# trungnt13/odin-ai

Measured on AMD Instinct MI355X. Metric: VAE train images/sec, higher is better.
Workload: dtype f32; 1 GPU; dsprites_betavae_b256; global_batch=256, per_gpu_batch=256, parallelism=dp1, graph=True

## Files before the change

### include/odin_hip.h

```cpp
#ifndef ODIN_HIP_H
#define ODIN_HIP_H

#include <stddef.h>
#include <stdint.h>

#ifdef __cplusplus
extern "C" {
#endif

enum { ODIN_LINEAR = 0, ODIN_ELU = 1, ODIN_RELU = 2 };

typedef struct odin_conv_desc {
  int B, H, W, Cin;
  int OH, OW, Cout;
  int KH, KW, stride;
  int pad_t, pad_l;
  int act;
  int center;
  uint32_t* dy_amax;
  uint32_t* dx_amax;
  const uint32_t* x_amax;
  uint32_t* y_amax;
} odin_conv_desc;

int odin_version(void);
const char* odin_debug_last_path(void);
uint32_t odin_crc32c(uint32_t crc, const void* data, size_t n);
const char* odin_last_error(void);
int odin_max_slab_rows(void);
int odin_conv2d_dgrad_keeps_range(const odin_conv_desc* d, int aux_act);
int odin_deconv2d_dgrad_keeps_range(const odin_conv_desc* d, int aux_act);
int odin_bernoulli_tail_keeps_range(int is_deconv, const odin_conv_desc* d, int C1);
#define ODIN_RANGE_WORDS 2048
int odin_range_reset(uint32_t* words, int n, void* stream);
int odin_absmax(const float* t, size_t n, uint32_t* word, void* stream);
int odin_debug_stream_probe(const float* a, const float* b, float* out, size_t n, int variant, int blocks,
                            void* stream);
int odin_debug_absmax_fallbacks(void);

int odin_conv2d_fwd(const float* x, const float* w, const float* bias, float* y,
                    const odin_conv_desc* d, void* stream);
int odin_conv2d_dgrad(const float* dy, const float* w, const float* aux, int aux_act, float* dx,
                      float* colsum_slab, int* slab_rows_out, const odin_conv_desc* d,
                      void* stream);
int odin_conv2d_wgrad(const float* x, const float* dy, float* slab, int* slab_rows_out,
                      const odin_conv_desc* d, void* stream);

int odin_deconv2d_fwd(const float* x, const float* w, const float* bias, float* y,
                      const odin_conv_desc* d, void* stream);
int odin_deconv2d_dgrad(const float* dy, const float* w, const float* aux, int aux_act,
                        float* dx, float* colsum_slab, int* slab_rows_out,
                        const odin_conv_desc* d, void* stream);
int odin_deconv2d_wgrad(const float* x, const float* dy, float* slab, int* slab_rows_out,
                        const odin_conv_desc* d, void* stream);

int odin_conv2d_bwd(const float* x, const float* dy, const float* w, const float* aux, int aux_act, float* dx,
                    float* colsum_slab, int* colsum_rows_out, float* wslab, int* wslab_rows_out,
                    const odin_conv_desc* d, void* stream);
int odin_deconv2d_bwd(const float* x, const float* dy, const float* w, const float* aux, int aux_act, float* dx,
                      float* colsum_slab, int* colsum_rows_out, float* wslab, int* wslab_rows_out,
                      const odin_conv_desc* d, void* stream);
int odin_conv2d_dgrad_first(const float* dy, const float* w, const float* aux, int aux_act, float* dx,
                            float* colsum_slab, int* colsum_rows_out, const odin_conv_desc* d, const float* x0,
                            float* wslab0, int* wslab0_rows_out, const odin_conv_desc* d0, void* stream);
int odin_dense_bwd(const float* x, const float* dy, const float* w, const float* aux, int aux_act, float* dx,
                   float* colsum_slab, int* colsum_rows_out, float* wslab, int* wslab_rows_out, int B, int K,
                   int N, int want_wgrad, int want_dgrad, const uint32_t* dy_amax, uint32_t* dx_amax, void* stream);
int odin_conv2d_reads_x_range(const odin_conv_desc* d);
int odin_deconv2d_reads_x_range(const odin_conv_desc* d);
int odin_dense_reads_x_range(int B, int K, int N);
int odin_dense_fwd_ranged(const float* x, const float* w, const float* bias, float* y, int B, int K, int N, int act,
                          const uint32_t* x_amax, uint32_t* y_amax, void* stream);
int odin_dense_bwd_ranged(const float* x, const float* dy, const float* w, const float* aux, int aux_act, float* dx,
                          float* colsum_slab, int* colsum_rows_out, float* wslab, int* wslab_rows_out, int B, int K,
                          int N, int want_wgrad, int want_dgrad, const uint32_t* dy_amax, uint32_t* dx_amax,
                          const uint32_t* x_amax, void* stream);
int odin_dense_dgrad_keeps_range(int B, int K, int N);

int odin_bernoulli_tail_fwd_bwd(int is_deconv, const float* x, const float* w, const float* bias,
                                const float* w1, const float* b1, const float* target,
                                float* logits, float* g_out, float* llk_part, int* n_part_out,
                                float* tail_slab, int* slab_rows_out, const float* scale,
                                const odin_conv_desc* d, int C1, void* stream);

int odin_dense_fwd(const float* x, const float* w, const float* bias, float* y, int B, int K,
                   int N, int act, void* stream);
int odin_dense_dgrad(const float* dy, const float* w, const float* aux, int aux_act, float* dx,
                     float* colsum_slab, int* slab_rows_out, int B, int K, int N, void* stream);
int odin_dense_wgrad(const float* x, const float* dy, float* slab, int* slab_rows_out, int B,
                     int K, int N, void* stream);

typedef struct odin_reduce_job {
  const float* src;
  float* dst;
  int n;
  int rows;
  int stride;
  int pad_;
} odin_reduce_job;
int odin_slab_reduce(const odin_reduce_job* jobs, int n_jobs, void* stream);

int odin_latent_fwd(const float* p, const float* eps, float* z, float* kl, float* fbmask, int B,
                    int D, int analytic, float free_bits, const float* capacity, void* stream);
int odin_latent_bwd(const float* p, const float* eps, const float* z, const float* dz,
                    const float* dz_extra, const float* fbmask, const float* klw,
                    const float* dloc_x, const float* dscale_x, float* dp, int B, int D,
                    int analytic, void* stream);

int odin_latent_block_rows(int B, int P, int D, int N0);
int odin_latent_block_fwd(const float* h, const float* wl, const float* bl, const float* eps_in,
                          float* eps_out, uint64_t seed, const int32_t* step_dev, float* p, float* z,
                          float* kl, float* fbmask, const float* w0, const float* b0, float* y0, int B,
                          int P, int D, int N0, int act0, int analytic, float free_bits,
                          const float* capacity, void* stream);
int odin_latent_block_bwd(const float* g0, const float* w0, const float* z, const float* p,
                          const float* eps, const float* fbmask, const float* klw, const float* dz_extra,
                          const float* dloc_x, const float* dscale_x, const float* wl, const float* h,
                          int h_act, float* dz, float* dp, float* dh, float* slab0, float* slabl, int B,
                          int P, int D, int N0, int analytic, uint32_t* dh_amax, void* stream);

typedef struct odin_neck_args {
  int B, P, D, C0;
  int act2, act3, act4, act0, act1;
  int analytic;
  float free_bits;
  uint64_t seed;
  const int32_t* step_dev;
  const float* x;
  const uint32_t* x_amax;
  const float *w3, *b3;
  float* y3;
  const float *w4, *b4;
  float* y4;
  const float *wl, *bl;
  const float* eps_in;
  float* eps;
  float *p, *z, *kl, *fbmask;
  const float* capacity;
  const float *w0, *b0;
  float* y0;
  const float *w1, *b1;
  float* y1;
  uint32_t* y1_amax;
  const float* dy1;
  const float* klw;
  const float *dz_extra, *dloc_x, *dscale_x;
  float *dz, *dp;
  float* dh4;
  float* dy3;
  float* dx;
  uint32_t *dh4_amax, *dy3_amax, *dx_amax;
  float* slab1;
  float* slab0;
  float* slabl;
} odin_neck_args;
void odin_wgrad_pair_begin(void);
int odin_wgrad_pair_end(void);
int odin_neck_rows(int B, int P, int D, int C0);
int odin_neck_fwd(const odin_neck_args* a, void* stream);
int odin_neck_bwd(const odin_neck_args* a, void* stream);

int odin_disc_head_rows(int B, int K);
int odin_disc_head_fwd_bwd(const float* h, const float* w, const float* bias, float* logit, int mode,
                           const float* dlogit_in, float* dlogit_out, float* out, int aux_act, float* dh,
                           uint32_t* dh_amax, float* wslab, int* rows_out, void* workspace, int B, int K, void* stream);

int odin_elbo_bernoulli_fwd_bwd(const float* logits, const float* x, float* llk_part,
                                float* dlogits, const float* scale, int B, int n_per_sample,
                                int* n_part_out, void* stream);
int odin_elbo_bernoulli_fwd_bwd_ranged(const float* logits, const float* x, float* llk_part,
                                       float* dlogits, const float* scale, int B, int n_per_sample,
                                       int* n_part_out, uint32_t* dlogits_amax, void* stream);
int odin_elbo_gaussian_fwd_bwd(const float* h, const float* x, float* llk_part, float* dh,
                               const float* scale, int B, int n_pix, int C, int softplus1,
                               int* n_part_out, void* stream);
void odin_wgrad_planes_defer_begin(void);
int odin_wgrad_planes_defer_end(void* stream);
double odin_debug_igemm_h_min_flop(double flop);
double odin_debug_blk_min_flop(double flop);
int odin_debug_blk_planes(int enable);
int odin_debug_blk_first(int on);
int odin_debug_dense_hw_min_tiles(int tiles);

int odin_gaussian_tail_applicable(const odin_conv_desc* d, int C);
int odin_gaussian_tail_fwd_bwd(const float* x, const float* w, const float* bias, const float* w1, const float* b1,
                               const float* target, float* logits, float* g_out, float* llk_part, int* n_part_out,
                               float* tail_slab, int* slab_rows_out, const float* scale, const odin_conv_desc* d, int C,
                               int softplus1, void* stream);
int odin_gaussian_head_fwd_bwd(const float* h, const float* w1, const float* b1, const float* target,
                               float* logits, float* dlogits, float* dh, float* llk_part, int* n_part_out,
                               float* wslab, int* rows_out, float* colsum_slab, const float* scale, int B,
                               int n_pix, int Cin, int C, int softplus1, int h_act, uint32_t* dh_amax,
                               void* stream);
int odin_elbo_mixqlogistic_fwd_bwd(const float* h, const float* x, float* llk_part, float* dh,
                                   const float* scale, int B, int n_pix, int C, int K,
                                   int* n_part_out, void* stream);
int odin_elbo_finalize(const float* llk_part, int n_part, const float* kl, const float* hyper,
                       const float* tc, float* llk, float* out4, int B, void* stream);
int odin_mean(const float* x, int n, float* out, void* stream);

int odin_total_correlation_workspace(int B_local, int B_global, int D);
int odin_total_correlation_fwd_bwd(const float* z, const float* p, float* tc_out, float* dz,
                                   float* dloc, float* dscale, const float* coef, int B, int D,
                                   void* stream);
int odin_total_correlation_shard(const float* z_local, const float* p_global, float* tc_out,
                                 float* dz_local, float* dloc_part, float* dscale_part,
                                 const float* coef, int B_local, int B_global, int D, void* stream);
int odin_mmd_workspace(int B_local, int B_global, int M, int D);
int odin_mmd_fwd_bwd(const float* x, const float* y, float* ws, float* dz, const float* coef,
                     const float* coef_grad, int N, int M, int D, int kernel, uint64_t prior_seed,
                     const int32_t* step_dev, void* stream);
int odin_mmd_shard(const float* x_local, const float* x_all, const float* y, float* ws, float* dz_local,
                   const float* coef, const float* coef_grad, int B_local, int B_global, int M, int D,
                   int kernel, int include_yy, uint64_t prior_seed, const int32_t* step_dev, void* stream);
int odin_dip_workspace(int world, int D);
int odin_dip_fwd_bwd(const float* p, float* ws, float* dloc, float* dscale, const float* coef,
                     const float* coef_grad, int N, int D, int type2, float lambda_diag, float lambda_offdiag,
                     void* stream);
int odin_dip_moments(const float* p_local, float* block, int B_local, int D, void* stream);
int odin_dip_finish(const float* blocks, int world, const float* p_local, float* ws, float* dloc,
                    float* dscale, const float* coef, const float* coef_grad, int B_local, int D, int type2,
                    float lambda_diag, float lambda_offdiag, void* stream);
int odin_vamprior_workspace(int B, int K, int D);
int odin_vamprior_fwd_bwd(const float* z, const float* pu, float* ws, float* c, float* dz, float* dpu,
                          const float* coef, const float* coef_grad, int B, int K, int D, void* stream);
int odin_clip_range_fwd(const float* w, float* u, size_t n, float lo, float hi, void* stream);
int odin_clip_range_bwd(const float* w, float* g, size_t n, float lo, float hi, float scale, void* stream);
int odin_vq_workspace(int N);
int odin_vq_assign(const float* codes, const float* codebook, int32_t* idx, float* z_q, float* ws, float* m_out,
                   int32_t* cnt, uint32_t* zq_amax, int N, int K, int Cs, void* stream);
int odin_vq_bwd(const float* codes, const float* z_q, const int32_t* idx, const float* dz_q, float* codebook,
                float* dcodes, float* dcodebook, float* ema_counts, float* ema_means, float commitment, double decay,
                double epsilon, int act, uint32_t* dcodes_amax, int N, int K, int Cs, void* stream);
int odin_permute_dims(const float* z, const int32_t* perm, float* out, int B, int D, void* stream);
int odin_random_perm(int32_t* perm, int B, int D, uint64_t seed, const int32_t* step_dev,
                     void* stream);
int odin_random_permute_dims(int32_t* perm, const float* z, float* out, int B, int D, uint64_t seed,
                             const int32_t* step_dev, void* stream);
int odin_dtc_loss_fwd_bwd(const float* logit_z, const float* logit_perm, float* out,
                          float* dlogit_z, float* dlogit_perm, int n, void* stream);

int odin_adam_step_flat(float* theta, const float* g, float* m, float* v, size_t n,
                        const float* hyper, const float* gnorm2, float clip, int32_t* flag,
                        void* stream);
typedef struct odin_adam_fold {
  const float* x; const float* dy; int B, K, N; size_t w_off;
  const float* slab; int slab_rows; size_t slab_stride, slab_n, slab_off;
  void* zero; int zero_n;
} odin_adam_fold;
int odin_adam_step_fold(float* theta, float* g, float* m, float* v, size_t n, const float* hyper,
                        const odin_adam_fold* fold, void* stream);
int odin_latent_sample_logprob(const float* p, const float* eps, float* z, float* logq,
                               float* logp, int n, int B, int D, void* stream);
int odin_logmeanexp_rows(const float* in, float* out, int n, int B, void* stream);
int odin_sum_parts(const float* llk_part, int n_part, float* out, int B, void* stream);

int odin_grad_skip_threshold(float* g, size_t n, float threshold, const int32_t* enable,
                             int32_t* hit, int32_t* skipped_count, void* stream);
int odin_clip_by_norm_segments(float* g, const int64_t* seg_offsets, int n_segments, float clipnorm,
                               void* stream);
int odin_clip_by_value(float* g, size_t n, float clipvalue, const float* gnorm2,
                       float global_clipnorm, void* stream);

int odin_sumsq_flat(const float* g, size_t n, float* workspace, float* out, void* stream);
int odin_sumsq_adam_flat(float* theta, const float* g, float* m, float* v, size_t n,
                         const float* hyper, float* workspace, float* gnorm2_out, float clip,
                         int32_t* flag, void* stream);

int odin_sumsq_adam_ring(float* theta, const float* g, float* m, float* v, size_t n, const float* hyper,
                         float* workspace, float* gnorm2_out, float clip, int32_t* flag, const float* llk_part,
                         int n_part, const float* kl, const float* elbo_hyper, const float* tc, float* llk,
                         float* out4, int B, const float* ring, float* cur, float* staged, int rows, int row_floats,
                         int t_word, void* stream);

int odin_slab_reduce_sumsq(const odin_reduce_job* jobs, int n_jobs, const float* g, size_t g_n, float* part,
                           int* n_parts_out, const float* stage_src, float* stage_dst, int stage_n, void* stream);
int odin_adam_ring_parts(float* theta, const float* g, float* m, float* v, size_t n, const float* staged,
                         int alpha_off, int elbo_off, const float* parts, int n_parts, float* gnorm2_out, float clip,
                         int32_t* flag, const float* llk_part, int n_part, const float* kl, const float* tc, float* llk,
                         float* out4, int B, const float* ring, float* cur, int rows, int row_floats, int t_word,
                         void* stream);

int odin_sumsq_adam_finalize_flat(float* theta, const float* g, float* m, float* v, size_t n,
                                  const float* hyper, float* workspace, float* gnorm2_out, float clip,
                                  int32_t* flag, const float* llk_part, int n_part, const float* kl,
                                  const float* elbo_hyper, const float* tc, float* llk, float* out4, int B,
                                  void* stream);

int odin_rng_normal(float* out, size_t n, uint64_t seed, const int32_t* step_dev, void* stream);

int odin_gather_normalize_u8(const uint8_t* data, const int32_t* idx, float* out, int B, int n_per,
                             float premul, int mode, void* stream);
int odin_gather_rows_f32(const float* data, const int32_t* idx, float* out, int B, int n_per, void* stream);

int odin_stft_mel_db(const float* y, const double* window, const double* twiddles,
                     const double* fb_vals, const int32_t* fb_band, float* out, int B,
                     int n_samples, int frame_length, int step_length, int n_fft, int n_mels,
                     double preemph, double top_db, int log_output, void* stream);
int odin_stft_mel_db_frames(const float* y, const double* window, const double* twiddles,
                            const double* fb_vals, const int32_t* fb_band, float* out, int B, int n_samples,
                            int frame_length, int step_length, int n_fft, int n_mels, double preemph,
                            double top_db, int log_output, int n_out_frames, float* workspace, void* stream);

int odin_comm_unique_id(void* id128);
int odin_comm_init(void** comm_out, const void* id128, int rank, int world_size);
int odin_comm_destroy(void* comm);
const char* odin_comm_library(void);
int odin_allreduce_flat(void* comm, float* buf, size_t n, void* stream);
int odin_allgather_flat(void* comm, const float* send, float* recv, size_t n_per_rank, void* stream);
int odin_reduce_scatter_flat(void* comm, const float* send, float* recv, size_t n_per_rank, void* stream);

int odin_debug_set_stamps(void* buf);
int odin_debug_set_wgrad_stamps(void* buf);
int odin_debug_set_neck_stamps(void* buf);
int odin_debug_elbo_shape(int blocks, int U, int pipelined);
int odin_debug_set_mel_stamps(void* buf);
int odin_debug_mel_r16(int enable);
int odin_debug_smallc_planes(int enable);
int odin_debug_igemm_h_ldsw_steps(int steps);

int odin_graph_begin(void* stream);
int odin_graph_end(void* stream, void** graph_exec_out);
int odin_graph_launch(void* graph_exec, void* stream);
int odin_graph_destroy(void* graph_exec);

#ifdef __cplusplus
}
#endif
#endif
```

### odin_ai_amd/_lib.py

```python
from __future__ import annotations

import ctypes as C
import os
from typing import Optional

_HERE = os.path.dirname(os.path.abspath(__file__))
DEFAULT_LIB = os.path.join(_HERE, 'libodin_hip.so')

ACT = {'linear': 0, 'elu': 1, 'relu': 2, None: 0}


class ConvDesc(C.Structure):
  _fields_ = [(n, C.c_int) for n in ('B', 'H', 'W', 'Cin', 'OH', 'OW', 'Cout', 'KH', 'KW',
                                     'stride', 'pad_t', 'pad_l', 'act', 'center')] + \
             [('dy_amax', C.c_void_p), ('dx_amax', C.c_void_p),
              ('x_amax', C.c_void_p), ('y_amax', C.c_void_p)]


class ReduceJob(C.Structure):
  _fields_ = [('src', C.c_void_p), ('dst', C.c_void_p), ('n', C.c_int), ('rows', C.c_int),
              ('stride', C.c_int), ('pad_', C.c_int)]


class AdamFold(C.Structure):
  _fields_ = [('x', C.c_void_p), ('dy', C.c_void_p), ('B', C.c_int), ('K', C.c_int), ('N', C.c_int), ('w_off', C.c_size_t),
              ('slab', C.c_void_p), ('slab_rows', C.c_int), ('slab_stride', C.c_size_t), ('slab_n', C.c_size_t),
              ('slab_off', C.c_size_t), ('zero', C.c_void_p), ('zero_n', C.c_int)]


class NeckArgs(C.Structure):
  _fields_ = [(n, C.c_int) for n in ('B', 'P', 'D', 'C0', 'act2', 'act3', 'act4', 'act0', 'act1', 'analytic')] + \
             [('free_bits', C.c_float), ('seed', C.c_uint64)] + \
             [(n, C.c_void_p) for n in (
                 'step_dev', 'x', 'x_amax', 'w3', 'b3', 'y3', 'w4', 'b4', 'y4', 'wl', 'bl', 'eps_in', 'eps', 'p', 'z',
                 'kl', 'fbmask', 'capacity', 'w0', 'b0', 'y0', 'w1', 'b1', 'y1', 'y1_amax',
                 'dy1', 'klw', 'dz_extra', 'dloc_x', 'dscale_x', 'dz', 'dp', 'dh4', 'dy3', 'dx',
                 'dh4_amax', 'dy3_amax', 'dx_amax', 'slab1', 'slab0', 'slabl')]


P = C.c_void_p
I = C.c_int
F = C.c_float
IP = C.POINTER(C.c_int)
DP = C.POINTER(ConvDesc)

SIGNATURES = {
    'odin_version': [],
    'odin_debug_last_path': [],
    'odin_crc32c': [C.c_uint32, P, C.c_size_t],
    'odin_max_slab_rows': [],
    'odin_range_reset': [P, I, P],
    'odin_conv2d_dgrad_keeps_range': [DP, I],
    'odin_deconv2d_dgrad_keeps_range': [DP, I],
    'odin_bernoulli_tail_keeps_range': [I, DP, I],
    'odin_conv2d_bwd': [P, P, P, P, I, P, P, IP, P, IP, DP, P],
    'odin_deconv2d_bwd': [P, P, P, P, I, P, P, IP, P, IP, DP, P],
    'odin_conv2d_dgrad_first': [P, P, P, I, P, P, IP, DP, P, P, IP, DP, P],
    'odin_dense_bwd': [P, P, P, P, I, P, P, IP, P, IP, I, I, I, I, I, P, P, P],
    'odin_dense_bwd_ranged': [P, P, P, P, I, P, P, IP, P, IP, I, I, I, I, I, P, P, P, P],
    'odin_dense_dgrad_keeps_range': [I, I, I],
    'odin_conv2d_reads_x_range': [DP],
    'odin_deconv2d_reads_x_range': [DP],
    'odin_dense_reads_x_range': [I, I, I],
    'odin_absmax': [P, C.c_size_t, P, P],
    'odin_debug_absmax_fallbacks': [],
    'odin_debug_stream_probe': [P, P, P, C.c_size_t, I, I, P],
    'odin_comm_unique_id': [P],
    'odin_comm_init': [C.POINTER(C.c_void_p), P, I, I],
    'odin_comm_destroy': [P],
    'odin_comm_library': [],
    'odin_allreduce_flat': [P, P, C.c_size_t, P],
    'odin_allgather_flat': [P, P, P, C.c_size_t, P],
    'odin_reduce_scatter_flat': [P, P, P, C.c_size_t, P],
    'odin_conv2d_fwd': [P, P, P, P, DP, P],
    'odin_conv2d_dgrad': [P, P, P, I, P, P, IP, DP, P],
    'odin_conv2d_wgrad': [P, P, P, IP, DP, P],
    'odin_deconv2d_fwd': [P, P, P, P, DP, P],
    'odin_deconv2d_dgrad': [P, P, P, I, P, P, IP, DP, P],
    'odin_deconv2d_wgrad': [P, P, P, IP, DP, P],
    'odin_bernoulli_tail_fwd_bwd': [I, P, P, P, P, P, P, P, P, P, IP, P, IP, P, DP, I, P],
    'odin_dense_fwd': [P, P, P, P, I, I, I, I, P],
    'odin_dense_fwd_ranged': [P, P, P, P, I, I, I, I, P, P, P],
    'odin_dense_dgrad': [P, P, P, I, P, P, IP, I, I, I, P],
    'odin_dense_wgrad': [P, P, P, IP, I, I, I, P],
    'odin_slab_reduce': [C.POINTER(ReduceJob), I, P],
    'odin_latent_fwd': [P, P, P, P, P, I, I, I, F, P, P],
    'odin_latent_bwd': [P, P, P, P, P, P, P, P, P, P, I, I, I, P],
    'odin_latent_block_rows': [I, I, I, I],
    'odin_latent_block_fwd': [P, P, P, P, P, C.c_uint64, P, P, P, P, P, P, P, P, I, I, I, I, I, I, F, P, P],
    'odin_latent_block_bwd': [P, P, P, P, P, P, P, P, P, P, P, P, I, P, P, P, P, P, I, I, I, I, I, P, P],
    'odin_wgrad_pair_begin': [],
    'odin_wgrad_pair_end': [],
    'odin_neck_rows': [I, I, I, I],
    'odin_neck_fwd': [C.POINTER(NeckArgs), P],
    'odin_neck_bwd': [C.POINTER(NeckArgs), P],
    'odin_elbo_bernoulli_fwd_bwd': [P, P, P, P, P, I, I, IP, P],
    'odin_elbo_bernoulli_fwd_bwd_ranged': [P, P, P, P, P, I, I, IP, P, P],
    'odin_elbo_gaussian_fwd_bwd': [P, P, P, P, P, I, I, I, I, IP, P],
    'odin_gaussian_tail_applicable': [DP, I],
    'odin_gaussian_tail_fwd_bwd': [P, P, P, P, P, P, P, P, P, IP, P, IP, P, DP, I, I, P],
    'odin_gaussian_head_fwd_bwd': [P, P, P, P, P, P, P, P, IP, P, IP, P, P, I, I, I, I, I, I, P, P],
    'odin_disc_head_rows': [I, I],
    'odin_disc_head_fwd_bwd': [P, P, P, P, I, P, P, P, I, P, P, P, IP, P, I, I, P],
    'odin_debug_igemm_h_min_flop': [C.c_double],
    'odin_debug_blk_min_flop': [C.c_double],
    'odin_debug_blk_planes': [C.c_int],
    'odin_debug_blk_first': [C.c_int],
    'odin_debug_dense_hw_min_tiles': [C.c_int],
    'odin_debug_mel_r16': [C.c_int],
    'odin_debug_smallc_planes': [C.c_int],
    'odin_wgrad_planes_defer_begin': [],
    'odin_wgrad_planes_defer_end': [P],
    'odin_elbo_mixqlogistic_fwd_bwd': [P, P, P, P, P, I, I, I, I, IP, P],
    'odin_elbo_finalize': [P, I, P, P, P, P, P, I, P],
    'odin_mean': [P, I, P, P],
    'odin_total_correlation_workspace': [I, I, I],
    'odin_total_correlation_fwd_bwd': [P, P, P, P, P, P, P, I, I, P],
    'odin_total_correlation_shard': [P, P, P, P, P, P, P, I, I, I, P],
    'odin_mmd_workspace': [I, I, I, I],
    'odin_mmd_fwd_bwd': [P, P, P, P, P, P, I, I, I, I, C.c_uint64, P, P],
    'odin_mmd_shard': [P, P, P, P, P, P, P, I, I, I, I, I, I, C.c_uint64, P, P],
    'odin_dip_workspace': [I, I],
    'odin_dip_fwd_bwd': [P, P, P, P, P, P, I, I, I, F, F, P],
    'odin_dip_moments': [P, P, I, I, P],
    'odin_dip_finish': [P, I, P, P, P, P, P, P, I, I, I, F, F, P],
    'odin_vamprior_workspace': [I, I, I],
    'odin_vamprior_fwd_bwd': [P, P, P, P, P, P, P, P, I, I, I, P],
    'odin_clip_range_fwd': [P, P, C.c_size_t, F, F, P],
    'odin_clip_range_bwd': [P, P, C.c_size_t, F, F, F, P],
    'odin_vq_workspace': [I],
    'odin_vq_assign': [P, P, P, P, P, P, P, P, I, I, I, P],
    'odin_vq_bwd': [P, P, P, P, P, P, P, P, P, F, C.c_double, C.c_double, I, P, I, I, I, P],
    'odin_permute_dims': [P, P, P, I, I, P],
    'odin_random_perm': [P, I, I, C.c_uint64, P, P],
    'odin_random_permute_dims': [P, P, P, I, I, C.c_uint64, P, P],
    'odin_dtc_loss_fwd_bwd': [P, P, P, P, P, I, P],
    'odin_adam_step_flat': [P, P, P, P, C.c_size_t, P, P, F, P, P],
    'odin_adam_step_fold': [P, P, P, P, C.c_size_t, P, C.POINTER(AdamFold), P],
    'odin_sumsq_flat': [P, C.c_size_t, P, P, P],
    'odin_latent_sample_logprob': [P, P, P, P, P, I, I, I, P],
    'odin_logmeanexp_rows': [P, P, I, I, P],
    'odin_sum_parts': [P, I, P, I, P],
    'odin_grad_skip_threshold': [P, C.c_size_t, F, P, P, P, P],
    'odin_clip_by_norm_segments': [P, P, I, F, P],
    'odin_clip_by_value': [P, C.c_size_t, F, P, F, P],
    'odin_sumsq_adam_flat': [P, P, P, P, C.c_size_t, P, P, P, F, P, P],
    'odin_sumsq_adam_finalize_flat': [P, P, P, P, C.c_size_t, P, P, P, F, P, P, I, P, P, P, P, P, I, P],
    'odin_sumsq_adam_ring': [P, P, P, P, C.c_size_t, P, P, P, F, P, P, I, P, P, P, P, P, I, P, P, P, I, I, I, P],
    'odin_slab_reduce_sumsq': [P, I, P, C.c_size_t, P, IP, P, P, I, P],
    'odin_adam_ring_parts': [P, P, P, P, C.c_size_t, P, I, I, P, I, P, F, P, P, I, P, P, P, P, I, P, P, I, I, I, P],
    'odin_rng_normal': [P, C.c_size_t, C.c_uint64, P, P],
    'odin_gather_normalize_u8': [P, P, P, I, I, F, I, P],
    'odin_gather_rows_f32': [P, P, P, I, I, P],
    'odin_stft_mel_db': [P, P, P, P, P, P, I, I, I, I, I, I, C.c_double, C.c_double, I, P],
    'odin_stft_mel_db_frames': [P, P, P, P, P, P, I, I, I, I, I, I, C.c_double, C.c_double, I, I, P, P],
    'odin_debug_set_stamps': [P],
    'odin_debug_set_wgrad_stamps': [P],
    'odin_debug_set_neck_stamps': [P],
    'odin_debug_elbo_shape': [I, I, I],
    'odin_debug_set_mel_stamps': [P],
    'odin_debug_igemm_h_ldsw_steps': [I],
    'odin_graph_begin': [P],
    'odin_graph_end': [P, C.POINTER(C.c_void_p)],
    'odin_graph_launch': [P, P],
    'odin_graph_destroy': [P],
}


VALUE_RETURNING = ('odin_version', 'odin_comm_library', 'odin_conv2d_dgrad_keeps_range',
                   'odin_deconv2d_dgrad_keeps_range', 'odin_bernoulli_tail_keeps_range', 'odin_dense_dgrad_keeps_range', 'odin_conv2d_reads_x_range',
                   'odin_deconv2d_reads_x_range', 'odin_dense_reads_x_range', 'odin_max_slab_rows', 'odin_debug_absmax_fallbacks', 'odin_crc32c', 'odin_debug_last_path',
                   'odin_latent_block_rows', 'odin_neck_rows', 'odin_debug_igemm_h_ldsw_steps', 'odin_total_correlation_workspace', 'odin_mmd_workspace', 'odin_dip_workspace', 'odin_vamprior_workspace', 'odin_vq_workspace', 'odin_debug_igemm_h_min_flop', 'odin_debug_blk_min_flop',
                   'odin_debug_blk_planes', 'odin_debug_blk_first', 'odin_debug_dense_hw_min_tiles', 'odin_gaussian_tail_applicable', 'odin_disc_head_rows', 'odin_debug_mel_r16', 'odin_debug_smallc_planes')
VOID_RETURNING = ('odin_wgrad_planes_defer_begin', 'odin_wgrad_pair_begin')


class OdinError(RuntimeError):
  pass


class Lib:

  def __init__(self, path: str):
    if not os.path.exists(path):
      raise OdinError(
          f"HIP extension not found: {path}. Build it with `python -c 'import "
          f"__graft_entry__ as g; g.build()'` (hipcc --offload-arch=gfx950). There is no "
          f"CPU fallback.")
    self.path = path
    self.c = C.CDLL(path)
    self.c.odin_last_error.restype = C.c_char_p
    self.c.odin_last_error.argtypes = []
    for name, args in SIGNATURES.items():
      fn = getattr(self.c, name)
      fn.argtypes = args
      fn.restype = (C.c_char_p if name in ('odin_debug_last_path', 'odin_comm_library') else
                    C.c_double if name in ('odin_debug_igemm_h_min_flop', 'odin_debug_blk_min_flop') else
                    None if name in VOID_RETURNING else
                    C.c_uint32 if name in VALUE_RETURNING else C.c_int)

  def check(self, rc: int, what: str = ''):
    if rc != 0:
      raise OdinError(f"{what} failed: {self.c.odin_last_error().decode()} (rc={rc})")

  def __getattr__(self, name):
    if name.startswith('odin_'):
      fn = getattr(self.c, name)

      trace = os.environ.get('ODIN_TRACE', '0') == '1'

      def call(*a):
        if trace:
          import sys
          import torch
          print('odin>', name, [x if isinstance(x, int) else '.' for x in a][-6:], flush=True,
                file=sys.stderr)
        rc = fn(*a)
        if trace:
          import torch
          if torch.cuda.is_available():
            torch.cuda.synchronize()
        if name in VOID_RETURNING:
          return None
        if rc != 0 and name not in VALUE_RETURNING:
          raise OdinError(f"{name} failed: {self.c.odin_last_error().decode()} (rc={rc})")
        return rc

      self.__dict__[name] = call
      return call
    raise AttributeError(name)


_lib: Optional[Lib] = None


def load(path: Optional[str] = None) -> Lib:
  global _lib
  if path is not None:
    _lib = Lib(path)
  elif _lib is None:
    _lib = Lib(os.environ.get('ODIN_HIP_LIB') or DEFAULT_LIB)
  return _lib


def ptr(t) -> Optional[int]:
  if t is None:
    return None
  assert t.is_contiguous(), 'odin kernels need contiguous buffers'
  return t.data_ptr()


def conv_desc(B, H, W, Cin, OH, OW, Cout, K, stride, pad_t, pad_l, act='linear',
              center=False) -> ConvDesc:
  return ConvDesc(B, H, W, Cin, OH, OW, Cout, K, K, stride, pad_t, pad_l, ACT[act], int(center))
```

### odin_ai_amd/csrc/dispatch.hip

```cpp
#include "odin_device.h"
#include "odin_internal.h"

namespace {

enum Family {
  GENERIC,
  SMALLC, PW1X1, SMALLDECONV, SMALLDECONV_GEN,
  FCONV_PLANES, FCONV_RING, FCONV_BLK, CONV5_BLK, TCONV_PLANES, TCONV_RING, TCONV_BLK, IGEMM_H, IGEMM,
  WGRAD_PLANES, WGRAD5_BLK, WGRAD_BLK, IGEMM_H_WGRAD, IGEMM_WGRAD,
  BWD_PLANES, BWD_BLK,
  TCONV_PLANES_FIRST,
  NOT_SERVED,
  BWD_PAIR,
  TINY_DENSE, THIN_DENSE, DENSE_H, DENSE_GEMM
};

enum { FOLDS_Y = 1, FOLDS_DX = 2, READS_X = 4 };
int traits(Family f) {
  switch (f) {
    case SMALLC: case SMALLDECONV_GEN: return FOLDS_Y;
    case SMALLDECONV: case IGEMM: case THIN_DENSE: return FOLDS_Y | FOLDS_DX;
    case FCONV_PLANES: case FCONV_BLK: case CONV5_BLK: case TCONV_PLANES: case TCONV_BLK: case IGEMM_H: case DENSE_H:
      return FOLDS_Y | FOLDS_DX | READS_X;
    case WGRAD_PLANES: case WGRAD5_BLK: case WGRAD_BLK: case IGEMM_H_WGRAD: return READS_X;
    case BWD_PLANES: case BWD_BLK: case DENSE_GEMM: case TCONV_PLANES_FIRST: return FOLDS_DX;
    default: return 0;
  }
}

int keep_range(int rc, Family f, int fold_bit, const float* t, size_t n, uint32_t* word, void* stream) {
  if (rc != 0 || t == nullptr || word == nullptr || (traits(f) & fold_bit)) return rc;
  return odin_absmax_fold(t, n, word, stream);
}

bool doubles(const odin_geom& g) { return g.OH == 2 * g.H && g.OW == 2 * g.W; }
bool same_size(const odin_geom& g) { return g.H == g.OH && g.W == g.OW; }
bool aligned16(const void* a, const void* b, const void* c, const void* d) {
  return ((((size_t)a | (size_t)b | (size_t)c | (size_t)d)) & 15) == 0;
}


Family select_conv2d_fwd(const odin_geom& g, bool bias, int act) {
  if (odin_smallc_applicable(g)) return SMALLC;
  if (odin_pw1x1_applicable(g)) return PW1X1;
  if (act == ODIN_ACT_ELU && bias && odin_fconv_planes_applicable(g)) return FCONV_PLANES;
  if (act == ODIN_ACT_ELU && bias && odin_fconv_ring_applicable(g)) return FCONV_RING;
  if (bias && same_size(g) && odin_conv5_blk_applicable(g)) return CONV5_BLK;
  if (bias && odin_fconv_blk_applicable(g)) return FCONV_BLK;
  if (odin_igemm_h_applicable(0, g)) return IGEMM_H;
  if (odin_igemm_applicable(0, g)) return IGEMM;
  return GENERIC;
}

bool igemm_dgrad(int tmode, const odin_geom& g, bool slab, bool dry) {
  return odin_igemm_applicable(tmode, g) && (odin_igemm_tiles(tmode, g) <= ODIN_MAX_COLSUM_BLOCKS || (!slab && !dry));
}

Family select_conv2d_dgrad(const odin_geom& l, const odin_geom& g, int aux_act, bool aux_ok, bool slab, bool dry) {
  if (odin_pw1x1_applicable(l)) return PW1X1;
  if (aux_act == ODIN_ACT_ELU && aux_ok && doubles(g) && odin_tconv_planes_applicable(g, 2, 1)) return TCONV_PLANES;
  if (aux_act == ODIN_ACT_ELU && aux_ok && doubles(g) && odin_tconv_ring_applicable(g)) return TCONV_RING;
  if (same_size(g) && odin_conv5_blk_applicable(g)) return CONV5_BLK;
  if (doubles(g) && odin_tconv_blk_applicable(g)) return TCONV_BLK;
  if (odin_igemm_h_applicable(1, g)) return IGEMM_H;
  if (igemm_dgrad(1, g, slab, dry)) return IGEMM;
  return GENERIC;
}

Family select_conv2d_dgrad_first(const odin_geom& l, const odin_geom& g, const odin_geom& l0, int aux_act, bool aux_ok) {
  if (select_conv2d_dgrad(l, g, aux_act, aux_ok, false, false) != TCONV_PLANES) return NOT_SERVED;
  return odin_tconv_planes_first_applicable(g, l0) ? TCONV_PLANES_FIRST : NOT_SERVED;
}

Family select_deconv2d_fwd(const odin_geom& g, bool bias, int act) {
  if (bias && odin_smalldeconv_applicable(g)) return SMALLDECONV;
  if (act == ODIN_ACT_ELU && bias && doubles(g) && odin_tconv_planes_applicable(g, 1, 1)) return TCONV_PLANES;
  if (act == ODIN_ACT_ELU && bias && doubles(g) && odin_tconv_ring_applicable(g)) return TCONV_RING;
  if (bias && (g.CI & 7) != 0 && odin_smalldeconv_gen_applicable(g)) return SMALLDECONV_GEN;
  if (bias && doubles(g) && odin_tconv_blk_applicable(g)) return TCONV_BLK;
  if (odin_igemm_h_applicable(1, g)) return IGEMM_H;
  if (odin_igemm_applicable(1, g)) return IGEMM;
  return GENERIC;
}

Family select_deconv2d_dgrad(const odin_geom& l, const odin_geom& g, int aux_act, bool aux_ok, bool slab, bool dry) {
  if (!slab && odin_smalldeconv_applicable(l)) return SMALLDECONV;
  if (aux_act == ODIN_ACT_ELU && aux_ok && odin_fconv_planes_applicable(g)) return FCONV_PLANES;
  if (odin_fconv_blk_applicable(g)) return FCONV_BLK;
  if (odin_igemm_h_applicable(0, g)) return IGEMM_H;
  const bool ring_two_pass_vs_igemm =
      g.CI == 64 && odin_igemm_applicable(0, g) && odin_igemm_tiles(0, g) <= ODIN_MAX_COLSUM_BLOCKS;
  if (!ring_two_pass_vs_igemm && aux_act == ODIN_ACT_ELU && aux_ok && odin_fconv_ring_applicable(g)) return FCONV_RING;
  if (igemm_dgrad(0, g, slab, dry)) return IGEMM;
  return GENERIC;
}

Family select_bernoulli_tail(int is_deconv, const odin_geom& g, int act, int C1) {
  if (is_deconv && act == ODIN_ACT_ELU && doubles(g) && odin_tconv_planes_applicable(g, 3, C1)) return TCONV_PLANES;
  if (is_deconv && act == ODIN_ACT_ELU && g.CO == 32 && (C1 == 1 || C1 == 3) && doubles(g) &&
      odin_tconv_ring_applicable(g))
    return TCONV_RING;
  return GENERIC;
}

Family select_wgrad_shared(const odin_geom& g, bool want_bias) {
  if (odin_wgrad_planes_applicable(g)) return WGRAD_PLANES;
  if (same_size(g) && want_bias && odin_wgrad5_blk_applicable(g)) return WGRAD5_BLK;
  if (odin_wgrad_blk_applicable(g)) return WGRAD_BLK;
  if (odin_igemm_h_wgrad_applicable(g)) return IGEMM_H_WGRAD;
  if (odin_igemm_wgrad_applicable(g)) return IGEMM_WGRAD;
  return GENERIC;
}
Family select_conv2d_wgrad(const odin_geom& g) {
  if (odin_smallc_applicable(g)) return SMALLC;
  if (odin_pw1x1_applicable(g)) return PW1X1;
  return select_wgrad_shared(g, true);
}
Family select_deconv2d_wgrad(const odin_geom& l, const odin_geom& g) {
  if (odin_smalldeconv_applicable(l)) return SMALLDECONV;
  return select_wgrad_shared(g, false);
}

Family select_deconv2d_bwd(const odin_geom& l, const odin_geom& g, int aux_act, bool aux, bool both, bool dry,
                           bool slab) {
  if (!slab && both && odin_smalldeconv_applicable(l)) return SMALLDECONV;
  const bool k4s2 = l.KH == 4 && l.KW == 4 && l.S == 2 && l.pt == 1 && l.pl == 1 && doubles(l);
  if (((both && aux) || dry) && aux_act == ODIN_ACT_ELU && k4s2 && odin_bwd_planes_applicable(l) &&
      odin_wgrad_planes_applicable(g) && odin_fconv_planes_applicable(g))
    return BWD_PLANES;
  if ((both || dry) && k4s2 && !l.center && odin_bwd_blk_applicable(l)) return BWD_BLK;
  return BWD_PAIR;
}

bool dense_via_igemm() { return ODIN_DIAG_ENV("ODIN_NODENSEIGEMM") == nullptr; }

Family select_dense_fwd(int B, int K, int N, bool aligned) {
  if (odin_tiny_dense_ok(B, K, N)) return TINY_DENSE;
  if (odin_thin_dense_kind(B, K, N) != 0 && aligned) return THIN_DENSE;
  if (odin_dense_h_ok(B, K, N)) return DENSE_H;
  if (dense_via_igemm() && odin_igemm_applicable(0, odin_geom_dense(B, K, N))) return IGEMM;
  if (odin_dense_gemm_ok(B, K, N)) return DENSE_GEMM;
  return GENERIC;
}
Family select_dense_dgrad(int B, int K, int N, bool slab, bool aligned) {
  if (odin_tiny_dense_ok(B, K, N)) return TINY_DENSE;
  if (slab) return GENERIC;
  if (odin_thin_dense_kind(B, K, N) != 0 && aligned) return THIN_DENSE;
  if (odin_dense_h_ok(B, K, N)) return DENSE_H;
  if (dense_via_igemm() && odin_igemm_applicable(1, odin_geom_dense(B, N, K))) return IGEMM;
  if (odin_dense_gemm_ok(B, K, N)) return DENSE_GEMM;
  return GENERIC;
}
Family select_dense_wgrad(int B, int K, int N, bool aligned) {
  if (odin_dense_h_ok(B, K, N)) return DENSE_H;
  if (odin_thin_dense_wgrad_rows(B, K, N) > 0 && aligned) return THIN_DENSE;
  if (dense_via_igemm() && !odin_tiny_dense_ok(B, K, N) && odin_igemm_wgrad_applicable(odin_geom_dense(B, K, N)))
    return IGEMM_WGRAD;
  if (odin_dense_gemm_ok(B, K, N) && !ODIN_DIAG_ENV("ODIN_NOTINYWGRADGEMM")) return DENSE_GEMM;
  return select_wgrad_shared(odin_geom_dense(B, K, N), true);
}
Family select_dense_bwd(int B, int K, int N, bool slab) {
  return odin_dense_h_ok(B, K, N) && !slab ? DENSE_H : BWD_PAIR;
}


int launch_gather(Family f, int tmode, int wmode, const odin_geom& g, const float* in, const float* w, const float* bias,
                  const float* aux, int aux_act, float* out, float* colsum, int* rows_out, int epi, int act,
                  const uint32_t* in_amax, uint32_t* out_amax, void* stream) {
  const float* blk_aux = aux_act != 0 ? aux : nullptr;
  const int blk_act = epi == 1 ? act : aux_act;
  switch (f) {
    case FCONV_PLANES:
      return odin_fconv_planes_launch(in, w, bias, aux, out, colsum, rows_out, g.B, g.OH, g.OW, g.CI, g.CO, epi, in_amax,
                                      out_amax, stream);
    case FCONV_RING:
      return odin_fconv_ring_launch(in, w, bias, aux, out, colsum, rows_out, g.B, g.H, g.W, g.CI, g.OH, g.OW, g.CO, epi,
                                    stream);
    case FCONV_BLK:
      return odin_fconv_blk_launch(in, w, bias, blk_aux, out, colsum, rows_out, g.B, g.OH, g.OW, g.CI, g.CO, epi, blk_act,
                                   in_amax, out_amax, stream);
    case CONV5_BLK:
      return odin_conv5_blk_launch(in, w, bias, blk_aux, out, colsum, rows_out, g.B, g.H, g.W, g.CI, g.CO, g.KH, epi,
                                   blk_act, in_amax, out_amax, stream);
    case TCONV_PLANES:
      return odin_tconv_planes_launch(in, w, bias, aux, out, colsum, rows_out, nullptr, nullptr, nullptr, nullptr, nullptr,
                                      nullptr, nullptr, nullptr, 1, g.B, g.H, g.W, g.CI, g.CO, epi, in_amax, out_amax, stream);
    case TCONV_RING:
      return odin_tconv_ring_launch(in, w, bias, aux, out, colsum, rows_out, nullptr, nullptr, nullptr, nullptr, nullptr,
                                    nullptr, nullptr, nullptr, 1, g.B, g.H, g.W, g.CO, epi, stream);
    case TCONV_BLK:
      return odin_tconv_blk_launch(in, w, bias, blk_aux, out, colsum, rows_out, g.B, g.H, g.W, g.CI, g.CO, epi, blk_act,
                                   in_amax, out_amax, stream);
    case IGEMM_H:
      return odin_igemm_h_launch(tmode, in, w, bias, aux, aux_act, out, colsum, g.B, g.H, g.W, g.CI, g.OH, g.OW, g.CO, g.KH,
                                 g.KW, g.S, g.pt, g.pl, act, in_amax, epi == 2, out_amax, stream);
    case IGEMM:
      return odin_igemm_launch(tmode, in, w, bias, aux, aux_act, out, colsum, g.B, g.H, g.W, g.CI, g.OH, g.OW, g.CO, g.KH,
                               g.KW, g.S, g.pt, g.pl, act, out_amax, stream);
    default:
      return odin_gather_generic(tmode, wmode, g, in, w, bias, act, aux, aux_act, out, colsum,
                                 colsum ? -ODIN_MAX_COLSUM_BLOCKS : odin_num_cus(), rows_out, nullptr, nullptr, stream);
  }
}

int dgrad_rows(Family f, int tmode, const odin_geom& g) {
  switch (f) {
    case SMALLDECONV: return 0;
    case IGEMM_H: return odin_igemm_h_rows(tmode, g);
    case IGEMM: return odin_igemm_tiles(tmode, g);
    default: return -1;
  }
}

int conv_dgrad(Family f, int tmode, int wmode, const odin_geom& g, const float* dy, const float* w, const float* aux,
               int aux_act, float* dx, float* colsum_slab, int* slab_rows_out, const odin_conv_desc* d, void* stream) {
  const int rows = dgrad_rows(f, tmode, g);
  if (rows >= 0) {
    if (slab_rows_out) *slab_rows_out = rows;
    if (dx == nullptr) return 0;
  }
  int rc;
  if (f == PW1X1) rc = odin_pw1x1_dgrad(dy, w, aux, aux_act, dx, colsum_slab, slab_rows_out, d, stream);
  else if (f == SMALLDECONV) rc = odin_smalldeconv_bwd(nullptr, dy, w, aux, aux_act, dx, nullptr, nullptr, d, stream);
  else
    rc = launch_gather(f, tmode, wmode, g, dy, w, nullptr, aux, aux_act, dx, colsum_slab, slab_rows_out, 2, 0, d->dy_amax,
                       d->dx_amax, stream);
  return keep_range(rc, f, FOLDS_DX, dx, (size_t)d->B * d->H * d->W * d->Cin, d->dx_amax, stream);
}

int conv_fwd(Family f, int tmode, int wmode, const odin_geom& g, const float* x, const float* w, const float* bias,
             float* y, const odin_conv_desc* d, void* stream) {
  int rc;
  switch (f) {
    case SMALLC: rc = odin_smallc_fwd(x, w, bias, y, d, stream); break;
    case PW1X1: rc = odin_pw1x1_fwd(x, w, bias, y, d, stream); break;
    case SMALLDECONV: rc = odin_smalldeconv_fwd(x, w, bias, y, d, stream); break;
    case SMALLDECONV_GEN: rc = odin_smalldeconv_gen_fwd(x, w, bias, y, d, stream); break;
    default:
      rc = launch_gather(f, tmode, wmode, g, x, w, bias, nullptr, 0, y, nullptr, nullptr, 1, d->act, d->x_amax, d->y_amax,
                         stream);
  }
  return keep_range(rc, f, FOLDS_Y, y, (size_t)d->B * d->OH * d->OW * d->Cout, d->y_amax, stream);
}

int launch_wgrad(Family f, const odin_geom& g, const float* in, const float* dy, float* slab, int want_bias,
                 const uint32_t* g_amax, const uint32_t* a_amax, int* rows_out, void* stream) {
  const int grad_u = want_bias ? 0 : 1;
  const int slab_stride = g.KH * g.KW * g.CI * g.CO + (want_bias ? g.CO : 0);
  if (f == IGEMM_H_WGRAD || f == IGEMM_WGRAD) {
    if (rows_out) *rows_out = f == IGEMM_H_WGRAD ? odin_igemm_h_wgrad_rows(g) : odin_igemm_wgrad_rows(g);
    if (slab == nullptr) return 0;
  }
  switch (f) {
    case WGRAD_PLANES:
      return odin_wgrad_planes_launch(in, dy, slab, rows_out, g.B, g.OH, g.OW, g.CI, g.CO, want_bias, grad_u, g_amax, a_amax,
                                      stream);
    case WGRAD5_BLK:
      return odin_wgrad5_blk_launch(in, dy, slab, rows_out, g.B, g.H, g.W, g.CI, g.CO, g.KH, want_bias, g_amax, a_amax,
                                    stream);
    case WGRAD_BLK:
      return odin_wgrad_blk_launch(in, dy, slab, rows_out, g.B, g.OH, g.OW, g.CI, g.CO, want_bias, grad_u, g_amax, a_amax,
                                   stream);
    case IGEMM_H_WGRAD:
      return odin_igemm_h_wgrad_launch(in, dy, slab, slab_stride, g.B, g.H, g.W, g.CI, g.OH, g.OW, g.CO, g.KH, g.KW, g.S,
                                       g.pt, g.pl, want_bias, grad_u, g_amax, a_amax, stream);
    case IGEMM_WGRAD:
      return odin_igemm_wgrad_launch(in, dy, slab, slab_stride, g.B, g.H, g.W, g.CI, g.OH, g.OW, g.CO, g.KH, g.KW, g.S, g.pt,
                                     g.pl, want_bias, stream);
    default:
      return odin_wgrad_generic(g, in, dy, slab, want_bias, rows_out, stream);
  }
}

int pair_end(int rc) {
  const int rc2 = odin_igemm_pair_end();
  return rc != 0 ? rc : rc2;
}

}

extern "C" int odin_conv2d_fwd(const float* x, const float* w, const float* bias, float* y, const odin_conv_desc* d,
                               void* stream) {
  const odin_geom g = odin_geom_fwd(d);
  return conv_fwd(select_conv2d_fwd(g, bias != nullptr, d->act), 0, 0, g, x, w, bias, y, d, stream);
}

extern "C" int odin_conv2d_dgrad(const float* dy, const float* w, const float* aux, int aux_act, float* dx,
                                 float* colsum_slab, int* slab_rows_out, const odin_conv_desc* d, void* stream) {
  const odin_geom g = odin_geom_dgrad(d);
  const Family f = select_conv2d_dgrad(odin_geom_fwd(d), g, aux_act, aux != nullptr || dx == nullptr,
                                       colsum_slab != nullptr, dx == nullptr);
  return conv_dgrad(f, 1, 1, g, dy, w, aux, aux_act, dx, colsum_slab, slab_rows_out, d, stream);
}

extern "C" int odin_conv2d_wgrad(const float* x, const float* dy, float* slab, int* slab_rows_out,
                                 const odin_conv_desc* d, void* stream) {
  const odin_geom g = odin_geom_fwd(d);
  const Family f = select_conv2d_wgrad(g);
  if (f == SMALLC) return odin_smallc_wgrad(x, dy, slab, slab_rows_out, d, stream);
  if (f == PW1X1) return odin_pw1x1_wgrad(x, dy, slab, slab_rows_out, d, stream);
  return launch_wgrad(f, g, x, dy, slab, 1, d->dy_amax, d->x_amax, slab_rows_out, stream);
}

extern "C" int odin_conv2d_bwd(const float* x, const float* dy, const float* w, const float* aux, int aux_act, float* dx,
                               float* colsum_slab, int* colsum_rows_out, float* wslab, int* wslab_rows_out,
                               const odin_conv_desc* d, void* stream) {
  odin_igemm_pair_begin();
  int rc = odin_conv2d_wgrad(x, dy, wslab, wslab_rows_out, d, stream);
  if (rc == 0) rc = odin_conv2d_dgrad(dy, w, aux, aux_act, dx, colsum_slab, colsum_rows_out, d, stream);
  return pair_end(rc);
}

extern "C" int odin_conv2d_dgrad_first(const float* dy, const float* w, const float* aux, int aux_act, float* dx,
                                       float* colsum_slab, int* colsum_rows_out, const odin_conv_desc* d, const float* x0,
                                       float* wslab0, int* wslab0_rows_out, const odin_conv_desc* d0, void* stream) {
  const bool dry = wslab0 == nullptr;
  const Family f = select_conv2d_dgrad_first(odin_geom_fwd(d), odin_geom_dgrad(d), odin_geom_fwd(d0), aux_act,
                                             aux != nullptr || dry);
  if (f != TCONV_PLANES_FIRST) return odin_fail(-2, "conv2d_dgrad_first: shapes outside the kernel");
  if (!dry && (dy == nullptr || w == nullptr || x0 == nullptr))
    return odin_fail(-2, "conv2d_dgrad_first: null argument");
  int rows = 0;
  const int rc = odin_tconv_planes_first_launch(dy, w, aux, dx, colsum_slab, x0, d0->center, wslab0, &rows, d->B, d->dy_amax,
                                                d->dx_amax, stream);
  if (rc == 0 && wslab0_rows_out) *wslab0_rows_out = rows;
  if (rc == 0 && colsum_rows_out) *colsum_rows_out = rows;
  return keep_range(rc, f, FOLDS_DX, dx, (size_t)d->B * d->H * d->W * d->Cin, d->dx_amax, stream);
}

extern "C" int odin_conv2d_dgrad_keeps_range(const odin_conv_desc* d, int aux_act) {
  const Family f = select_conv2d_dgrad(odin_geom_fwd(d), odin_geom_dgrad(d), aux_act, true, false, false);
  return (traits(f) & FOLDS_DX) ? 1 : 0;
}

extern "C" int odin_conv2d_reads_x_range(const odin_conv_desc* d) {
  const odin_geom g = odin_geom_fwd(d);
  return ((traits(select_conv2d_fwd(g, true, d->act)) | traits(select_conv2d_wgrad(g))) & READS_X) ? 1 : 0;
}

extern "C" int odin_deconv2d_fwd(const float* x, const float* w, const float* bias, float* y, const odin_conv_desc* d,
                                 void* stream) {
  const odin_geom g = odin_geom_fwd(d);
  return conv_fwd(select_deconv2d_fwd(g, bias != nullptr, d->act), 1, 1, g, x, w, bias, y, d, stream);
}

extern "C" int odin_deconv2d_dgrad(const float* dy, const float* w, const float* aux, int aux_act, float* dx,
                                   float* colsum_slab, int* slab_rows_out, const odin_conv_desc* d, void* stream) {
  const odin_geom g = odin_geom_dgrad(d);
  const Family f = select_deconv2d_dgrad(odin_geom_fwd(d), g, aux_act, aux != nullptr || dx == nullptr,
                                         colsum_slab != nullptr, dx == nullptr);
  return conv_dgrad(f, 0, 0, g, dy, w, aux, aux_act, dx, colsum_slab, slab_rows_out, d, stream);
}

extern "C" int odin_deconv2d_wgrad(const float* x, const float* dy, float* slab, int* slab_rows_out,
                                   const odin_conv_desc* d, void* stream) {
  const odin_geom g = odin_geom_dgrad(d);
  const Family f = select_deconv2d_wgrad(odin_geom_fwd(d), g);
  if (f == SMALLDECONV)
    return odin_smalldeconv_bwd(x, dy, nullptr, nullptr, 0, nullptr, slab, slab_rows_out, d, stream);
  return launch_wgrad(f, g, dy, x, slab, 0, d->dy_amax, d->x_amax, slab_rows_out, stream);
}

extern "C" int odin_deconv2d_bwd(const float* x, const float* dy, const float* w, const float* aux, int aux_act, float* dx,
                                 float* colsum_slab, int* colsum_rows_out, float* wslab, int* wslab_rows_out,
                                 const odin_conv_desc* d, void* stream) {
  const odin_geom l = odin_geom_fwd(d);
  const bool dry = dx == nullptr && wslab == nullptr;
  const Family f = select_deconv2d_bwd(l, odin_geom_dgrad(d), aux_act, aux != nullptr, dx != nullptr && wslab != nullptr,
                                       dry, colsum_slab != nullptr);
  if (f == SMALLDECONV) {
    if (colsum_rows_out) *colsum_rows_out = 0;
    return odin_smalldeconv_bwd(x, dy, w, aux, aux_act, dx, wslab, wslab_rows_out, d, stream);
  }
  if (f == BWD_PLANES || f == BWD_BLK) {
    const int rows = f == BWD_PLANES ? odin_bwd_planes_rows(l) : odin_bwd_blk_rows(l);
    if (colsum_rows_out) *colsum_rows_out = rows;
    if (wslab_rows_out) *wslab_rows_out = rows;
    if (dry) return 0;
    if (f == BWD_PLANES)
      return odin_bwd_planes_launch(x, dy, w, aux, dx, colsum_slab, wslab, d->B, d->H, d->W, d->Cin, d->Cout, d->dy_amax,
                                    d->x_amax, d->dx_amax, stream);
    return odin_bwd_blk_launch(x, dy, w, aux, aux_act, dx, colsum_slab, wslab, d->B, d->H, d->W, d->Cin, d->Cout,
                               d->dy_amax, d->x_amax, d->dx_amax, stream);
  }
  odin_igemm_pair_begin();
  int rc = odin_deconv2d_wgrad(x, dy, wslab, wslab_rows_out, d, stream);
  if (rc == 0) rc = odin_deconv2d_dgrad(dy, w, aux, aux_act, dx, colsum_slab, colsum_rows_out, d, stream);
  return pair_end(rc);
}

extern "C" int odin_deconv2d_dgrad_keeps_range(const odin_conv_desc* d, int aux_act) {
  const Family f = select_deconv2d_dgrad(odin_geom_fwd(d), odin_geom_dgrad(d), aux_act, true, false, false);
  return (traits(f) & FOLDS_DX) ? 1 : 0;
}
extern "C" int odin_deconv2d_reads_x_range(const odin_conv_desc* d) {
  const odin_geom l = odin_geom_fwd(d);
  return ((traits(select_deconv2d_fwd(l, true, d->act)) | traits(select_deconv2d_wgrad(l, odin_geom_dgrad(d)))) & READS_X)
             ? 1 : 0;
}

extern "C" int odin_bernoulli_tail_fwd_bwd(int is_deconv, const float* x, const float* w, const float* bias, const float* w1,
                                           const float* b1, const float* target, float* logits, float* g_out,
                                           float* llk_part, int* n_part_out, float* tail_slab, int* slab_rows_out,
                                           const float* scale, const odin_conv_desc* d, int C1, void* stream) {
  const odin_geom g = odin_geom_fwd(d);
  const Family f = select_bernoulli_tail(is_deconv, g, d->act, C1);
  const odin_tail_args tail = {w1, b1, target, scale, logits, llk_part, tail_slab, C1};
  int rc;
  if (f == TCONV_PLANES)
    rc = odin_tconv_planes_launch(x, w, bias, nullptr, g_out, nullptr, slab_rows_out, w1, b1, target, logits, llk_part,
                                  n_part_out, tail_slab, scale, C1, d->B, d->H, d->W, d->Cin, d->Cout, 3, d->x_amax,
                                  d->dy_amax, stream);
  else if (f == TCONV_RING)
    rc = odin_tconv_ring_launch(x, w, bias, nullptr, g_out, nullptr, slab_rows_out, w1, b1, target, logits, llk_part,
                                n_part_out, tail_slab, scale, C1, d->B, d->H, d->W, d->Cout, 3, stream);
  else
    rc = odin_gather_generic(is_deconv, is_deconv ? 1 : 0, g, x, w, bias, d->act, nullptr, 0, g_out, nullptr,
                             -ODIN_MAX_COLSUM_BLOCKS, slab_rows_out, &tail, n_part_out, stream);
  return keep_range(rc, f, FOLDS_Y, g_out, (size_t)d->B * d->OH * d->OW * d->Cout, d->dy_amax, stream);
}
extern "C" int odin_bernoulli_tail_keeps_range(int is_deconv, const odin_conv_desc* d, int C1) {
  return (traits(select_bernoulli_tail(is_deconv, odin_geom_fwd(d), d->act, C1)) & FOLDS_Y) ? 1 : 0;
}

extern "C" int odin_dense_fwd(const float* x, const float* w, const float* bias, float* y, int B, int K, int N, int act,
                              void* stream) {
  return odin_dense_fwd_ranged(x, w, bias, y, B, K, N, act, nullptr, nullptr, stream);
}

extern "C" int odin_dense_fwd_ranged(const float* x, const float* w, const float* bias, float* y, int B, int K, int N,
                                     int act, const uint32_t* x_amax, uint32_t* y_amax, void* stream) {
  const Family f = select_dense_fwd(B, K, N, aligned16(x, w, y, bias));
  int rc;
  switch (f) {
    case TINY_DENSE: rc = odin_tiny_dense_fwd(x, w, bias, y, B, K, N, act, stream); break;
    case THIN_DENSE: rc = odin_thin_dense_fwd(x, w, bias, y, B, K, N, act, y_amax, stream); break;
    case DENSE_H: rc = odin_dense_h_fwd(x, w, bias, y, B, K, N, act, x_amax, y_amax, stream); break;
    case DENSE_GEMM: rc = odin_dense_gemm_fwd(x, w, bias, y, B, K, N, act, stream); break;
    default:
      rc = launch_gather(f, 0, 0, odin_geom_dense(B, K, N), x, w, bias, nullptr, 0, y, nullptr, nullptr, 1, act, nullptr,
                         y_amax, stream);
  }
  return keep_range(rc, f, FOLDS_Y, y, (size_t)B * N, y_amax, stream);
}

static int dense_dgrad(const float* dy, const float* w, const float* aux, int aux_act, float* dx, float* colsum_slab,
                       int* slab_rows_out, int B, int K, int N, const uint32_t* dy_amax, uint32_t* dx_amax,
                       void* stream) {
  const Family f = select_dense_dgrad(B, K, N, colsum_slab != nullptr, aligned16(dy, w, dx, aux));
  if (f != TINY_DENSE && f != GENERIC) {
    if (slab_rows_out) *slab_rows_out = 0;
    if (dx == nullptr) return 0;
  }
  int rc;
  switch (f) {
    case TINY_DENSE:
      rc = odin_tiny_dense_dgrad(dy, w, aux, aux_act, dx, colsum_slab, slab_rows_out, B, K, N, stream);
      break;
    case THIN_DENSE: rc = odin_thin_dense_dgrad(dy, w, aux, aux_act, dx, B, K, N, dx_amax, stream); break;
    case DENSE_H: rc = odin_dense_h_dgrad(dy, w, aux, aux_act, dx, B, K, N, dy_amax, dx_amax, stream); break;
    case DENSE_GEMM: rc = odin_dense_gemm_dgrad(dy, w, aux, aux_act, dx, B, K, N, dx_amax, stream); break;
    default:
      rc = launch_gather(f, f == IGEMM, 1, odin_geom_dense(B, N, K), dy, w, nullptr, aux, aux_act, dx, colsum_slab,
                         slab_rows_out, 2, 0, nullptr, dx_amax, stream);
  }
  return keep_range(rc, f, FOLDS_DX, dx, (size_t)B * K, dx_amax, stream);
}

extern "C" int odin_dense_dgrad(const float* dy, const float* w, const float* aux, int aux_act, float* dx,
                                float* colsum_slab, int* slab_rows_out, int B, int K, int N, void* stream) {
  return dense_dgrad(dy, w, aux, aux_act, dx, colsum_slab, slab_rows_out, B, K, N, nullptr, nullptr, stream);
}

extern "C" int odin_dense_wgrad(const float* x, const float* dy, float* slab, int* slab_rows_out, int B, int K, int N,
                                void* stream) {
  const Family f = select_dense_wgrad(B, K, N, slab == nullptr || aligned16(x, dy, slab, nullptr));
  if (f == DENSE_H || f == THIN_DENSE || f == DENSE_GEMM) {
    if (slab_rows_out) *slab_rows_out = f == THIN_DENSE ? odin_thin_dense_wgrad_rows(B, K, N) : 1;
    if (slab == nullptr) return 0;
    if (f == DENSE_H) return odin_dense_h_wgrad(x, dy, slab, B, K, N, nullptr, nullptr, stream);
    if (f == THIN_DENSE) return odin_thin_dense_wgrad(x, dy, slab, B, K, N, stream);
    return odin_dense_gemm_wgrad(x, dy, slab, B, K, N, stream);
  }
  return launch_wgrad(f, odin_geom_dense(B, K, N), x, dy, slab, 1, nullptr, nullptr, slab_rows_out, stream);
}

extern "C" int odin_dense_bwd(const float* x, const float* dy, const float* w, const float* aux, int aux_act, float* dx,
                              float* colsum_slab, int* colsum_rows_out, float* wslab, int* wslab_rows_out, int B, int K,
                              int N, int want_wgrad, int want_dgrad, const uint32_t* dy_amax, uint32_t* dx_amax, void* stream) {
  return odin_dense_bwd_ranged(x, dy, w, aux, aux_act, dx, colsum_slab, colsum_rows_out, wslab, wslab_rows_out, B, K, N,
                               want_wgrad, want_dgrad, dy_amax, dx_amax, nullptr, stream);
}

extern "C" int odin_dense_bwd_ranged(const float* x, const float* dy, const float* w, const float* aux, int aux_act,
                                     float* dx, float* colsum_slab, int* colsum_rows_out, float* wslab, int* wslab_rows_out,
                                     int B, int K, int N, int want_wgrad, int want_dgrad, const uint32_t* dy_amax,
                                     uint32_t* dx_amax, const uint32_t* x_amax, void* stream) {
  if (select_dense_bwd(B, K, N, colsum_slab != nullptr) == DENSE_H) {
    int rc = 0;
    if (dy_amax == nullptr && ((want_wgrad && wslab != nullptr) || (want_dgrad && dx != nullptr))) {
      dy_amax = odin_range_word_of(dy, (size_t)B * N, nullptr, stream);
      if (dy_amax == nullptr) return odin_fail(-3, "dense_bwd: no range word for dy");
    }
    if (want_wgrad && want_dgrad && wslab != nullptr && dx != nullptr) {
      if (wslab_rows_out) *wslab_rows_out = 1;
      if (colsum_rows_out) *colsum_rows_out = 0;
      return odin_dense_h_bwd_pair(x, dy, w, aux, aux_act, dx, wslab, B, K, N, dy_amax, dx_amax, x_amax, stream);
    }
    if (want_wgrad) {
      if (wslab_rows_out) *wslab_rows_out = 1;
      if (wslab != nullptr) rc = odin_dense_h_wgrad(x, dy, wslab, B, K, N, dy_amax, x_amax, stream);
    }
    if (rc == 0 && want_dgrad) {
      if (colsum_rows_out) *colsum_rows_out = 0;
      if (dx != nullptr) rc = odin_dense_h_dgrad(dy, w, aux, aux_act, dx, B, K, N, dy_amax, dx_amax, stream);
    }
    return rc;
  }
  odin_igemm_pair_begin();
  int rc = 0;
  if (want_wgrad) rc = odin_dense_wgrad(x, dy, wslab, wslab_rows_out, B, K, N, stream);
  if (rc == 0 && want_dgrad)
    rc = dense_dgrad(dy, w, aux, aux_act, dx, colsum_slab, colsum_rows_out, B, K, N, dy_amax, dx_amax, stream);
  return pair_end(rc);
}

extern "C" int odin_dense_dgrad_keeps_range(int B, int K, int N) {
  return (traits(select_dense_dgrad(B, K, N, false, true)) & FOLDS_DX) ? 1 : 0;
}
extern "C" int odin_dense_reads_x_range(int B, int K, int N) {
  return (traits(select_dense_fwd(B, K, N, true)) & READS_X) ? 1 : 0;
}
```

### odin_ai_amd/csrc/fconv_planes.hip

```cpp
#include "odin_device.h"
#include "odin_internal.h"
#include <cstdlib>

namespace {

struct FPParams {
  const float* in;
  const float* w;
  const float* bias;
  const float* aux;
  float* out;
  float* colsum;
  int B, OH, CO;
  int CS, ci_off;
  int tiles_per_img, n_tiles, tiles_per_wg;
  const unsigned* in_amax;
  unsigned* out_amax;
  long long* stamps;
};

#if defined(ODIN_SIM) || !defined(ODIN_DIAG)
#define FP_STAMP(k) ((void)0)
#else
#define FP_STAMP(k)                                                                               \
  do {                                                                                            \
    if (p.stamps != nullptr && blockIdx.x == 0 && blockIdx.y == 0 && lane == 0 && stamp_i < 32)        \
      p.stamps[32 * wave + stamp_i++] = ((long long)(k) << 56) | (long long)(clock64() & 0xFFFFFFFFFFFFFFll); \
  } while (0)
#endif

struct alignas(8) FpEnt {
  int x, y;
};

struct FpItem {
  float4 v;
  int dst;
};

constexpr int FP_MAXU = 4;

template <int EPI, int OW, bool ACC, int SCM>
__device__ __forceinline__ void fp_body(const FPParams& p) {
  constexpr int NPL = 2;
  constexpr int TC = 32 / OW;
  constexpr int WU = 2 * OW;
  constexpr int SU = OW + 1;
  constexpr int PARB = (SU + 1) * 64;
  constexpr int PBU = 2 * PARB;
  constexpr int RBU = NPL * PBU;
  constexpr int NSU = 4 * TC + 3;
  constexpr int IPU = WU / 8;
  constexpr int RJ = 8 / IPU > 0 ? 8 / IPU : 1;
  constexpr int RED = 8 * 8 * 64 * 8;
  ODIN_DYN_SMEM(char, smem);
  char* ring = smem;
  char* red = smem + NSU * RBU;
  const int tid = threadIdx.x, lane = tid & 63;
#ifdef ODIN_SIM
  const int wave = tid >> 6;
#else
  const int wave = __builtin_amdgcn_readfirstlane(tid >> 6);
#endif
  const int l31 = lane & 31, half = lane >> 5;
  const int n0 = blockIdx.y * 32;
  const int HU = 2 * p.OH, HPU = HU + 1;
  const int T0 = blockIdx.x * p.tiles_per_wg;
  int T1 = T0 + p.tiles_per_wg;
  if (T1 > p.n_tiles) T1 = p.n_tiles;
  if (T0 >= T1) return;
  int stamp_i = 0;
  (void)stamp_i;
  FP_STAMP(1);

  const OdinRangeReq in_rq = odin_range_issue(SCM != 0 ? p.in_amax : nullptr, lane);
  const int kh = wave >> 1, kw0 = 2 * (wave & 1);
  float wv[2][2][8];
#pragma unroll
  for (int t = 0; t < 2; ++t)
#pragma unroll
    for (int kk = 0; kk < 2; ++kk) {
      const int tap = kh * 4 + kw0 + t;
#pragma unroll
      for (int e = 0; e < 8; ++e)
        wv[t][kk][e] = p.w[((size_t)(tap * p.CS + p.ci_off + 16 * kk + 8 * half + e)) * p.CO + n0 + l31];
    }
  const OdinRun RU = odin_run(p.in, (unsigned)((size_t)p.B * HU * WU * p.CS * 4));
  float amx = 0.f;
  constexpr int RPF = FP_MAXU * RJ;
  constexpr int DST_NONE = -(1 << 24);
  constexpr unsigned OFF_NONE = 0x7FFF0000u;
  const unsigned u_rowbytes = (unsigned)(WU * p.CS * 4);
  const int ch4 = lane & 7, pxl = lane >> 3;
  const int r0w = wave / IPU, cblk = wave - r0w * IPU;
  const int pcw = 8 * cblk + pxl + 1;
  const int u_lds = (pcw & 1) * PARB + (pcw >> 1) * 64 + (((ch4 >> 1) ^ (((pcw >> 1) >> 2) & 3)) << 4) + (ch4 & 1) * 8;
  const unsigned u_g = (unsigned)(((8 * cblk + pxl) * p.CS + p.ci_off + 4 * ch4) * 4);
  FpItem iuA[FP_MAXU], iuB[FP_MAXU], iuC[FP_MAXU];
  {
    const int tpi = p.tiles_per_img;
    const int b0 = odin_div_small(T0, tpi), t0 = T0 - b0 * tpi;
    const int start = HPU * b0 + 2 * TC * t0;
#pragma unroll
    for (int j = 0; j < FP_MAXU; ++j) {
      const int r = r0w + RJ * j, G = start + r;
      const bool valid = r < 2 * TC + 2;
      const int b = b0 + (2 * TC * t0 + r >= HPU ? 1 : 0), gi = G - b * HPU;
      const bool real = valid && gi != 0 && b < p.B;
      const int slot = G - odin_div_small(G, NSU) * NSU;
      iuA[j].dst = valid ? slot * RBU + u_lds : -1;
      iuA[j].v = odin_run_load4(RU, real ? (unsigned)(G - b - 1) * u_rowbytes + u_g : ODIN_OOB);
    }
  }
  ODIN_SCHED_FENCE();
  bool sc = SCM == 1;
  float in_s = 1.f, in_s2k = ODIN_LO_SCALE, out_s = 1.f;

  for (int e = tid; e < NSU * 8 * NPL; e += 512) {
    const int sl = e / (8 * NPL), rem = e - sl * (8 * NPL);
    const int pl = rem >> 3, side = (rem >> 2) & 1, piece = rem & 3;
    *reinterpret_cast<float4*>(ring + sl * RBU + pl * PBU + (side ? PARB + OW * 64 : 0) + piece * 16) =
        make_float4(0.f, 0.f, 0.f, 0.f);
  }

  for (int e = tid; e < RED / 16; e += 512)
    *reinterpret_cast<float4*>(red + ((T0 - 1) & 1) * RED + e * 16) = make_float4(0.f, 0.f, 0.f, 0.f);

  const int NF = p.tiles_per_wg + 4;
  FpEnt* tt = reinterpret_cast<FpEnt*>(red + 2 * RED);
  FpEnt* tr = tt + NF;
  {
    const int tpi = p.tiles_per_img;
    for (int e = tid; e < NF; e += 512) {
      const int T = T0 + e, b = odin_div_small(T, tpi), t = T - b * tpi;
      const int g0 = HPU * b + 2 * TC * t;
      tt[e] = FpEnt{g0 - odin_div_small(g0, NSU) * NSU, (int)(((size_t)(b * p.OH + TC * t) * OW) * p.CO * 4)};
    }
    for (int e = tid; e < NF * RPF; e += 512) {
      const int f = e / RPF, r = e - f * RPF;
      const int T = T0 + f, b1 = odin_div_small(T, tpi), t1 = T - b1 * tpi;
      const int end = HPU * b1 + 2 * TC * t1 + 2 * TC + 2;
      int start = end - (2 * TC + 2);
      if (f > 0) {
        const int b0 = t1 > 0 ? b1 : b1 - 1, t0 = t1 > 0 ? t1 - 1 : tpi - 1;
        start = HPU * b0 + 2 * TC * t0 + 2 * TC + 2;
      }
      const int G = start + r;
      const bool valid = T < T1 && G < end;
      const int b = odin_div_small(G, HPU), gi = G - b * HPU;
      const bool real = valid && gi != 0 && b < p.B;
      tr[e] = FpEnt{valid ? (G - odin_div_small(G, NSU) * NSU) * RBU : DST_NONE,
                        real ? (int)((unsigned)(G - b - 1) * u_rowbytes) : (int)OFF_NONE};
    }
  }
  auto fill_entries = [&](FpEnt (&en)[FP_MAXU], int f) {
#pragma unroll
    for (int j = 0; j < FP_MAXU; ++j) en[j] = tr[f * RPF + r0w + RJ * j];
  };
  auto fill_loads = [&](FpItem (&iu)[FP_MAXU], const FpEnt (&en)[FP_MAXU]) {
#pragma unroll
    for (int j = 0; j < FP_MAXU; ++j) {
      iu[j].dst = en[j].x + u_lds;
      iu[j].v = odin_run_load4(RU, (unsigned)en[j].y + u_g);
    }
  };
  auto store_item = [&](const FpItem& it) {
#ifdef ODIN_SIM
    if (it.dst < 0) return;
#else
    if (__builtin_amdgcn_readfirstlane(it.dst) < 0) return;
#endif
    u32x2 h, l;
    if (SCM == 1 || (SCM == 2 && sc)) odin_split_h4<true>(it.v, in_s, in_s2k, h, l);
    else odin_split_h4<false>(it.v, 1.f, ODIN_LO_SCALE, h, l);
    char* d = ring + it.dst;
    *reinterpret_cast<u32x2*>(d) = h;
    *reinterpret_cast<u32x2*>(d + PBU) = l;
  };

  const int orow = (OW == 32) ? 0 : (OW == 16) ? (l31 >> 4) : (l31 >> 3);
  const int ocol = (OW == 32) ? l31 : (OW == 16) ? (l31 & 15) : (l31 & 7);
  int boff[2][2];
#pragma unroll
  for (int t = 0; t < 2; ++t)
#pragma unroll
    for (int kk = 0; kk < 2; ++kk) {
      const int kw = kw0 + t, slot = ocol + (kw >> 1);
      boff[t][kk] = (kw & 1) * PARB + slot * 64 + (((2 * kk + half) ^ ((slot >> 2) & 3)) << 4);
    }
  const int c0 = n0 + ((2 * wave) & 3) + 8 * ((2 * wave) >> 2) + 4 * half;
  float bias2[2] = {0.f, 0.f};
  if (EPI == 1) { bias2[0] = p.bias[c0]; bias2[1] = p.bias[c0 + 1]; }
  float csum[2] = {0.f, 0.f};

  FpEnt en[FP_MAXU];
  FP_STAMP(6);
  u32x4 wf[2][2][NPL];
#pragma unroll
  for (int t = 0; t < 2; ++t)
#pragma unroll
    for (int kk = 0; kk < 2; ++kk) {
      const float(&v)[8] = wv[t][kk];
      u32x2 h0, l0, h1, l1;
      odin_split_h4<false>(make_float4(v[0], v[1], v[2], v[3]), 1.f, ODIN_LO_SCALE, h0, l0);
      odin_split_h4<false>(make_float4(v[4], v[5], v[6], v[7]), 1.f, ODIN_LO_SCALE, h1, l1);
      wf[t][kk][0][0] = h0.x; wf[t][kk][0][1] = h0.y; wf[t][kk][0][2] = h1.x; wf[t][kk][0][3] = h1.y;
      wf[t][kk][1][0] = l0.x; wf[t][kk][1][1] = l0.y; wf[t][kk][1][2] = l1.x; wf[t][kk][1][3] = l1.y;
    }

  if (SCM != 0) {
    const unsigned in_mb = odin_range_finish(in_rq);
    sc = SCM == 1 || odin_act_needs_scale(in_mb);
    const int gk = sc ? odin_range_shift(in_mb) : 0;
    in_s = odin_pow2(gk); in_s2k = odin_pow2(gk + 11); out_s = odin_pow2(-gk);
  }
  FP_STAMP(8);
#pragma unroll
  for (int j = 0; j < FP_MAXU; ++j) store_item(iuA[j]);
  FP_STAMP(9);
  __syncthreads();
  FP_STAMP(7);
  FpEnt en1[FP_MAXU], en2[FP_MAXU];
  fill_entries(en1, 1);
  fill_entries(en2, 2);
  fill_entries(en, 3);
  FpEnt thN = tt[0];
  fill_loads(iuA, en1);
  fill_loads(iuB, en2);
  const unsigned o_lane = (unsigned)(((orow * OW + ocol) * p.CO + c0) * 4);

  const unsigned out_bytes = (unsigned)((size_t)p.B * p.OH * OW * p.CO * 4);
  const OdinRun RO = odin_run(p.out, out_bytes);
  const OdinRun RX = odin_run(EPI == 2 ? p.aux : p.out, out_bytes);
  unsigned ooffP = ODIN_OOB;
  float2 auxP = make_float2(0.f, 0.f), pvP = make_float2(0.f, 0.f);

  auto finish_load = [&](int buf, float2 (&q8)[8]) {
    const char* q = red + buf * RED + ((wave * 8 * 64 + lane) << 3);
#pragma unroll
    for (int wv = 0; wv < 8; ++wv) q8[wv] = *reinterpret_cast<const float2*>(q + wv * (64 * 8));
  };
  auto finish_done = [&](const float2 (&q8)[8]) {
    float2 s = q8[0];
#pragma unroll
    for (int wv = 1; wv < 8; ++wv) { s.x += q8[wv].x; s.y += q8[wv].y; }
    float v[2] = {s.x, s.y};
    if (SCM == 1 || (SCM == 2 && sc)) { v[0] *= out_s; v[1] *= out_s; }
    if (ACC) { v[0] += pvP.x; v[1] += pvP.y; }
    if (EPI == 1) {
#pragma unroll
      for (int k = 0; k < 2; ++k) {
        const float tt = v[k] + bias2[k];
        v[k] = fmaxf(tt, 0.f) + (odin_exp2(fminf(tt, 0.f) * 1.44269504088896341f) - 1.f);
      }
      amx = odin_amax3(amx, v[0], v[1]);
    } else if (EPI == 2) {
      v[0] = fmaf(v[0], fminf(auxP.x, 0.f), v[0]);
      v[1] = fmaf(v[1], fminf(auxP.y, 0.f), v[1]);
      csum[0] += v[0];
      csum[1] += v[1];
      amx = odin_amax3(amx, v[0], v[1]);
    }
    odin_run_store2(RO, ooffP, make_float2(v[0], v[1]));
  };

  auto run_tile = [&](int T, FpItem (&ldu)[FP_MAXU], const FpItem (&stu)[FP_MAXU]) {
    const FpEnt th = thN;
    int su = th.x + 2 * orow + kh;
    su -= su >= NSU ? NSU : 0;
    const char* rowp = ring + su * RBU;
    u32x4 fb[2][2][NPL];
    FP_STAMP(2);
#pragma unroll
    for (int pl = NPL - 1; pl >= 0; --pl)
#pragma unroll
      for (int t = 0; t < 2; ++t)
#pragma unroll
        for (int kk = 0; kk < 2; ++kk) fb[t][kk][pl] = *reinterpret_cast<const u32x4*>(rowp + boff[t][kk] + pl * PBU);
    ODIN_SCHED_FENCE();
    const unsigned ooff = (unsigned)th.y + o_lane;
    float2 auxN = make_float2(0.f, 0.f), pvN = make_float2(0.f, 0.f);
    float2 q8[8];
    f32x16 acc = f32x16_zero(), acx = f32x16_zero();
#pragma unroll
    for (int m = 0; m < 12; ++m) {
      const int t = (m >> 1) & 1, kk = m & 1, pp = m >> 2;
      if (pp == 0) acx = mfma32_f16(wf[t][kk][0], fb[t][kk][1], acx);
      if (pp == 1) acx = mfma32_f16(wf[t][kk][1], fb[t][kk][0], acx);
      if (pp == 2) acc = mfma32_f16(wf[t][kk][0], fb[t][kk][0], acc);
      if (m == 0) FP_STAMP(3);
      if (m == 11) FP_STAMP(4);
      if (m == 0) {
        fill_loads(ldu, en);
        if (EPI == 2) auxN = odin_run_load2(RX, ooff);
        if (ACC) pvN = odin_run_load2(RO, ooff);
      }
      if (m == 10) {
        fill_entries(en, T - T0 + 4);
        thN = tt[T - T0 + 1];
      }
      if ((m & 1) == 1 && (m >> 1) < FP_MAXU) store_item(stu[m >> 1]);
      if (m == 8) finish_load((T - 1) & 1, q8);
      if (m == 9) finish_done(q8);
      ODIN_SCHED_FENCE();
    }
#pragma unroll
    for (int r = 0; r < 16; ++r) acc[r] = fmaf(acx[r], ODIN_LO_UNSCALE, acc[r]);
    char* d = red + (T & 1) * RED + ((wave * 64 + lane) << 3);
#pragma unroll
    for (int pr = 0; pr < 8; ++pr)
      *reinterpret_cast<float2*>(d + pr * (8 * 64 * 8)) = make_float2(acc[2 * pr], acc[2 * pr + 1]);
    FP_STAMP(5);
    ooffP = ooff;
    auxP = auxN;
    pvP = pvN;
    __syncthreads();
  };
#pragma unroll 1
  for (int T = T0; T < T1; T += 3) {
    run_tile(T, iuC, iuA);
    if (T + 1 < T1) run_tile(T + 1, iuA, iuB);
    if (T + 2 < T1) run_tile(T + 2, iuB, iuC);
  }
  {
    float2 q8[8];
    finish_load((T1 - 1) & 1, q8);
    finish_done(q8);
  }

  if (EPI == 2 || EPI == 1) {
    __syncthreads();
    odin_amax_commit_wg(p.out_amax, amx, tid, 512, reinterpret_cast<float*>(red), blockIdx.x + gridDim.x * blockIdx.y);
  }
  if (EPI == 2 && p.colsum != nullptr) {
#pragma unroll
    for (int k = 0; k < 2; ++k) {
      float v = csum[k];
#pragma unroll
      for (int m = 16; m >= 1; m >>= 1) v += __shfl_xor(v, m);
      if (l31 == 0) p.colsum[(size_t)blockIdx.x * p.CO + c0 + k] = v;
    }
  }
}

template <int EPI, int OW, bool ACC, int SCM>
__global__ __launch_bounds__(512) void fconv_planes_kernel(FPParams p) {
  fp_body<EPI, OW, ACC, SCM>(p);
}

template <int EPI, int OW, int SCM>
__global__ __launch_bounds__(512) void fconv_planes2_kernel(FPParams p) {
  {
    FPParams q = p;
    q.colsum = nullptr;
    q.out_amax = nullptr;
    q.ci_off = 0;
    fp_body<0, OW, false, SCM>(q);
  }
  odin_wait_vmem();
#ifndef ODIN_SIM
  __builtin_amdgcn_fence(__ATOMIC_SEQ_CST, "workgroup");
#endif
  __syncthreads();
  p.ci_off = 32;
  fp_body<EPI, OW, true, SCM>(p);
}

constexpr int FP_LDS_MAX = 160 * 1024;
int fp_ring_bytes(int OW) { return (4 * (32 / OW) + 3) * 2 * 2 * (OW + 2) * 64 + 2 * (8 * 4 * 64 * 16); }
int fp_fill_bytes(int OW) {
  const int ipu = 2 * OW / 8, rj = 8 / ipu > 0 ? 8 / ipu : 1;
  return 8 * (1 + FP_MAXU * rj);
}
int fp_tiles_per_wg(int OW, int n_tiles, int gy) {
  int cap = odin_num_cus() / gy;
  if (cap < 1) cap = 1;
  if (cap > ODIN_MAX_COLSUM_BLOCKS) cap = ODIN_MAX_COLSUM_BLOCKS;
  int tpw = (n_tiles + cap - 1) / cap;
  const int limit = (FP_LDS_MAX - fp_ring_bytes(OW)) / fp_fill_bytes(OW) - 4;
  if (tpw > limit) tpw = limit;
  if ((n_tiles + tpw - 1) / tpw > ODIN_MAX_COLSUM_BLOCKS) return -1;
  return tpw;
}

template <int EPI, int OW, bool ACC, int SC>
int fp_launch(const FPParams& p, dim3 grid, void* stream) {
  const size_t lds = (size_t)fp_ring_bytes(OW) + (size_t)(p.tiles_per_wg + 4) * fp_fill_bytes(OW);
#ifndef ODIN_SIM
  static bool attr_done = false;
  if (!attr_done) {
    if (hipFuncSetAttribute(reinterpret_cast<const void*>(&fconv_planes_kernel<EPI, OW, ACC, SC>),
                            hipFuncAttributeMaxDynamicSharedMemorySize, FP_LDS_MAX) != hipSuccess)
      (void)hipGetLastError();
    attr_done = true;
  }
#endif
  ODIN_LAUNCH((fconv_planes_kernel<EPI, OW, ACC, SC>), grid, dim3(512), lds, stream, p);
  return odin_check_launch("fconv_planes(f16x2)");
}

template <int EPI, int SC>
int fp_launch2_w(const FPParams& p, int OW, dim3 grid, void* stream) {
  const size_t lds = (size_t)fp_ring_bytes(OW) + (size_t)(p.tiles_per_wg + 4) * fp_fill_bytes(OW);
#ifndef ODIN_SIM
  static bool attr_done = false;
  if (!attr_done) {
    const void* fns[3] = {reinterpret_cast<const void*>(&fconv_planes2_kernel<EPI, 32, SC>),
                          reinterpret_cast<const void*>(&fconv_planes2_kernel<EPI, 16, SC>),
                          reinterpret_cast<const void*>(&fconv_planes2_kernel<EPI, 8, SC>)};
    for (int i = 0; i < 3; ++i)
      if (hipFuncSetAttribute(fns[i], hipFuncAttributeMaxDynamicSharedMemorySize, FP_LDS_MAX) != hipSuccess)
        (void)hipGetLastError();
    attr_done = true;
  }
#endif
  if (OW == 32) ODIN_LAUNCH((fconv_planes2_kernel<EPI, 32, SC>), grid, dim3(512), lds, stream, p);
  else if (OW == 16) ODIN_LAUNCH((fconv_planes2_kernel<EPI, 16, SC>), grid, dim3(512), lds, stream, p);
  else ODIN_LAUNCH((fconv_planes2_kernel<EPI, 8, SC>), grid, dim3(512), lds, stream, p);
  return odin_check_launch("fconv_planes(f16x2)");
}

}

static long long* g_fp_stamps = nullptr;
void odin_fconv_planes_set_stamps(void* buf) { g_fp_stamps = (long long*)buf; }

bool odin_fconv_planes_applicable(const odin_geom& g) {
  const int B = g.B, H = g.H, W = g.W, CI = g.CI, OH = g.OH, OW = g.OW, CO = g.CO, KH = g.KH, KW = g.KW, S = g.S;
  if (odin_blk_first()) return false;
  if (odin_exact_fp32() || ODIN_DIAG_ENV("ODIN_NOPLANES") || ODIN_DIAG_ENV("ODIN_SPLIT") || ODIN_DIAG_ENV("ODIN_NOFPLANES")) return false;
  return KH == 4 && KW == 4 && S == 2 && g.pt == 1 && g.pl == 1 && (CI == 32 || (CI == 64 && !ODIN_DIAG_ENV("ODIN_FP_NO64"))) && (CO % 32) == 0 && !g.center &&
         H == 2 * OH && W == 2 * OW && (OW == 8 || OW == 16 || OW == 32) && (OH % (32 / OW)) == 0 &&
         (size_t)B * H * W * CI * 4 < 0x7FFF0000ull && (size_t)B * OH * OW * CO * 4 < (1ull << 31) &&
         fp_tiles_per_wg(OW, B * (OH / (32 / OW)), CO / 32) > 0;
}

template <int EPI, bool ACC, int SC>
int fp_launch_w(const FPParams& p, int OW, dim3 grid, void* stream) {
  if (OW == 32) return fp_launch<EPI, 32, ACC, SC>(p, grid, stream);
  if (OW == 16) return fp_launch<EPI, 16, ACC, SC>(p, grid, stream);
  return fp_launch<EPI, 8, ACC, SC>(p, grid, stream);
}

int odin_fconv_planes_launch(const float* in, const float* w, const float* bias, const float* aux,
                             float* out, float* colsum, int* rows_out, int B, int OH, int OW, int CI, int CO,
                             int epi, const uint32_t* in_amax, uint32_t* out_amax, void* stream) {
  FPParams p;
  memset(&p, 0, sizeof(p));
  p.in = in; p.w = w; p.bias = bias; p.aux = aux; p.out = out; p.colsum = colsum;
  p.B = B; p.OH = OH; p.CO = CO;
  p.CS = CI; p.ci_off = 0;
  p.stamps = g_fp_stamps;
  const int TC = 32 / OW;
  p.tiles_per_img = OH / TC;
  p.n_tiles = B * p.tiles_per_img;
  const int gy = CO / 32;
  p.tiles_per_wg = fp_tiles_per_wg(OW, p.n_tiles, gy);
  if (p.tiles_per_wg <= 0) return odin_fail(-2, "fconv_planes: too many tiles for the fill tables");
  const int gx = (p.n_tiles + p.tiles_per_wg - 1) / p.tiles_per_wg;
  if (rows_out) *rows_out = gx;
  if (out == nullptr) return 0;
  if (epi == 2) {
    p.in_amax = odin_range_word_of(in, (size_t)B * 2 * OH * 2 * OW * CI, in_amax, stream);
    if (p.in_amax == nullptr) return odin_fail(-3, "fconv_planes: no range word for the gradient input");
    p.out_amax = out_amax;
  } else {
    p.in_amax = in_amax;
    p.out_amax = out_amax;
  }
  const bool aw = epi == 1 && in_amax != nullptr;
  dim3 grid(gx, gy, 1);
  if (CI == 64) {
#ifdef ODIN_DIAG
    if (ODIN_DIAG_ENV("ODIN_FP_2LAUNCH")) {
      FPParams q = p;
      q.colsum = nullptr;
      q.out_amax = nullptr;
      const int rc = epi == 1 ? fp_launch_w<0, false, 0>(q, OW, grid, stream) : fp_launch_w<0, false, 1>(q, OW, grid, stream);
      if (rc != 0) return rc;
      p.ci_off = 32;
      return epi == 1 ? fp_launch_w<1, true, 0>(p, OW, grid, stream) : fp_launch_w<2, true, 1>(p, OW, grid, stream);
    }
#endif
    if (epi == 1) return aw ? fp_launch2_w<1, 2>(p, OW, grid, stream) : fp_launch2_w<1, 0>(p, OW, grid, stream);
    return fp_launch2_w<2, 1>(p, OW, grid, stream);
  }
  if (epi == 1) return aw ? fp_launch_w<1, false, 2>(p, OW, grid, stream) : fp_launch_w<1, false, 0>(p, OW, grid, stream);
  return fp_launch_w<2, false, 1>(p, OW, grid, stream);
}
```

### odin_ai_amd/csrc/odin_internal.h

```cpp
#pragma once
#include <cstdio>
#include <cstring>
#include "../../include/odin_hip.h"

#define ODIN_MAX_SLAB_BLOCKS 256
#define ODIN_MAX_COLSUM_BLOCKS 512

#include <cstdlib>
#ifdef ODIN_DIAG
#define ODIN_DIAG_ENV(name) getenv(name)
#else
#define ODIN_DIAG_ENV(name) ((const char*)nullptr)
#endif
static inline bool odin_exact_fp32() { return getenv("ODIN_EXACT_FP32") != nullptr; }

struct odin_geom {
  int B, H, W, CI, OH, OW, CO, KH, KW, S, pt, pl, center;
};
static inline odin_geom odin_geom_fwd(const odin_conv_desc* d) {
  return {d->B, d->H, d->W, d->Cin, d->OH, d->OW, d->Cout, d->KH, d->KW, d->stride, d->pad_t, d->pad_l, d->center};
}
static inline odin_geom odin_geom_dgrad(const odin_conv_desc* d) {
  return {d->B, d->OH, d->OW, d->Cout, d->H, d->W, d->Cin, d->KH, d->KW, d->stride, d->pad_t, d->pad_l, 0};
}
static inline odin_geom odin_geom_dense(int B, int K, int N) { return {B, 1, 1, K, 1, 1, N, 1, 1, 1, 0, 0, 0}; }

int odin_fail(int code, const char* msg);
int odin_check_launch(const char* what);
int odin_wgrad_planes_flush(void* stream);
int odin_num_cus();
const uint32_t* odin_range_word_of(const float* t, size_t n, const uint32_t* given, void* stream);
int odin_absmax_fold(const float* t, size_t n, uint32_t* word, void* stream);

bool odin_smallc_applicable(const odin_geom& g);
int odin_smallc_fwd(const float* x, const float* w, const float* bias, float* y,
                    const odin_conv_desc* d, void* stream);
int odin_smallc_wgrad(const float* x, const float* dy, float* slab, int* rows_out,
                      const odin_conv_desc* d, void* stream);

bool odin_tiny_dense_ok(int B, int K, int N);
int odin_tiny_dense_fwd(const float* x, const float* w, const float* bias, float* y, int B, int K,
                        int N, int act, void* stream);
int odin_tiny_dense_dgrad(const float* dy, const float* w, const float* aux, int aux_act, float* dx,
                          float* colsum_slab, int* slab_rows_out, int B, int K, int N, void* stream);

bool odin_pw1x1_applicable(const odin_geom& g);
int odin_pw1x1_fwd(const float* x, const float* w, const float* bias, float* y,
                   const odin_conv_desc* d, void* stream);
int odin_pw1x1_dgrad(const float* dy, const float* w, const float* aux, int aux_act, float* dx,
                     float* colsum_slab, int* slab_rows_out, const odin_conv_desc* d, void* stream);
int odin_pw1x1_wgrad(const float* x, const float* dy, float* slab, int* slab_rows_out,
                     const odin_conv_desc* d, void* stream);

bool odin_dense_gemm_ok(int B, int K, int N);
int odin_dense_gemm_fwd(const float* x, const float* w, const float* bias, float* y, int B, int K,
                        int N, int act, void* stream);
int odin_dense_gemm_dgrad(const float* dy, const float* w, const float* aux, int aux_act, float* dx,
                          int B, int K, int N, uint32_t* dx_amax, void* stream);
int odin_zero_u32(uint32_t* p, size_t n, void* stream);
int odin_dense_gemm_wgrad(const float* x, const float* dy, float* slab, int B, int K, int N,
                          void* stream);

int odin_thin_dense_kind(int B, int K, int N);
int odin_thin_dense_wgrad_rows(int B, int K, int N);
int odin_thin_dense_fwd(const float* x, const float* w, const float* bias, float* y, int B, int K, int N, int act,
                        uint32_t* y_amax, void* stream);
int odin_thin_dense_dgrad(const float* dy, const float* w, const float* aux, int aux_act, float* dx, int B, int K, int N,
                          uint32_t* dx_amax, void* stream);
int odin_thin_dense_wgrad(const float* x, const float* dy, float* slab, int B, int K, int N, void* stream);

bool odin_dense_h_ok(int B, int K, int N);
int odin_dense_h_fwd(const float* x, const float* w, const float* bias, float* y, int B, int K, int N, int act,
                     const uint32_t* x_amax, uint32_t* y_amax, void* stream);
int odin_dense_h_dgrad(const float* dy, const float* w, const float* aux, int aux_act, float* dx, int B, int K, int N,
                       const uint32_t* dy_amax, uint32_t* dx_amax, void* stream);
int odin_dense_h_wgrad(const float* x, const float* dy, float* slab, int B, int K, int N, const uint32_t* dy_amax,
                       const uint32_t* x_amax, void* stream);
int odin_dense_h_bwd_pair(const float* x, const float* dy, const float* w, const float* aux, int aux_act, float* dx,
                          float* slab, int B, int K, int N, const uint32_t* dy_amax, uint32_t* dx_amax,
                          const uint32_t* x_amax, void* stream);

bool odin_bwd_planes_applicable(const odin_geom& g);
int odin_bwd_planes_rows(const odin_geom& g);
int odin_bwd_planes_launch(const float* x, const float* dy, const float* w, const float* aux, float* dx, float* colsum,
                           float* wslab, int B, int H, int W, int Cin, int Cout, const uint32_t* dy_amax,
                           const uint32_t* x_amax, uint32_t* dx_amax, void* stream);
bool odin_smalldeconv_applicable(const odin_geom& g);
bool odin_smalldeconv_gen_applicable(const odin_geom& g);
int odin_smalldeconv_gen_fwd(const float* x, const float* w, const float* bias, float* y, const odin_conv_desc* d,
                             void* stream);
int odin_smalldeconv_fwd(const float* x, const float* w, const float* bias, float* y, const odin_conv_desc* d,
                         void* stream);
int odin_smalldeconv_bwd(const float* x, const float* dy, const float* w, const float* aux, int aux_act, float* dx,
                         float* slab, int* rows_out, const odin_conv_desc* d, void* stream);

bool odin_fconv_ring_applicable(const odin_geom& g);
int odin_fconv_ring_launch(const float* in, const float* w, const float* bias, const float* aux,
                           float* out, float* colsum, int* rows_out, int B, int H, int W, int CI,
                           int OH, int OW, int CO, int epi, void* stream);
void odin_fconv_ring_set_stamps(void* buf);

void odin_tconv_ring_set_stamps(void* buf);
bool odin_tconv_ring_applicable(const odin_geom& g);
int odin_tconv_ring_launch(const float* in, const float* w, const float* bias, const float* aux,
                           float* out, float* colsum, int* rows_out, const float* w1, const float* b1,
                           const float* target, float* logits, float* llk_part, int* n_part_out,
                           float* slab, const float* scale, int C1, int B, int H, int W, int CO,
                           int epi, void* stream);

bool odin_tconv_blk_applicable(const odin_geom& g);
int odin_tconv_blk_launch(const float* in, const float* w, const float* bias, const float* aux, float* out,
                          float* colsum, int* rows_out, int B, int H, int W, int CI, int CO, int epi, int act,
                          const uint32_t* in_amax, uint32_t* out_amax, void* stream);
bool odin_fconv_blk_applicable(const odin_geom& g);
int odin_fconv_blk_launch(const float* in, const float* w, const float* bias, const float* aux, float* out,
                          float* colsum, int* rows_out, int B, int OH, int OW, int CI, int CO, int epi, int act,
                          const uint32_t* in_amax, uint32_t* out_amax, void* stream);
bool odin_wgrad_blk_applicable(const odin_geom& g);
int odin_wgrad_blk_launch(const float* U, const float* V, float* slab, int* rows_out, int B, int OH, int OW, int CI,
                          int CO, int want_bias, int grad_u, const uint32_t* g_amax, const uint32_t* a_amax,
                          void* stream);
bool odin_conv5_blk_applicable(const odin_geom& g);
int odin_conv5_blk_launch(const float* in, const float* w, const float* bias, const float* aux, float* out,
                          float* colsum, int* rows_out, int B, int H, int W, int CI, int CO, int K, int epi, int act,
                          const uint32_t* in_amax, uint32_t* out_amax, void* stream);
bool odin_wgrad5_blk_applicable(const odin_geom& g);
int odin_wgrad5_blk_launch(const float* x, const float* dy, float* slab, int* rows_out, int B, int H, int W, int CI,
                           int CO, int K, int want_bias, const uint32_t* g_amax, const uint32_t* a_amax, void* stream);
bool odin_blk_enabled(double flop);
bool odin_blk_first();
bool odin_bwd_blk_applicable(const odin_geom& g);
int odin_bwd_blk_rows(const odin_geom& g);
int odin_bwd_blk_launch(const float* x, const float* dy, const float* w, const float* aux, int aux_act, float* dx,
                        float* colsum, float* wslab, int B, int H, int W, int Cin, int Cout, const uint32_t* dy_amax,
                        const uint32_t* x_amax, uint32_t* dx_amax, void* stream);
void odin_tconv_planes_set_stamps(void* buf);
bool odin_tconv_planes_applicable(const odin_geom& g, int epi, int C1);
int odin_tconv_planes_launch(const float* in, const float* w, const float* bias, const float* aux,
                             float* out, float* colsum, int* rows_out, const float* w1, const float* b1,
                             const float* target, float* logits, float* llk_part, int* n_part_out,
                             float* slab, const float* scale, int C1, int B, int H, int W, int CI,
                             int CO, int epi, const uint32_t* in_amax, uint32_t* out_amax, void* stream);
bool odin_tconv_planes_first_applicable(const odin_geom& g, const odin_geom& l0);
int odin_tconv_planes_first_launch(const float* in, const float* w, const float* aux, float* out, float* colsum, const float* img,
                                   int center0, float* wslab0, int* rows_out, int B, const uint32_t* in_amax,
                                   uint32_t* out_amax, void* stream);

bool odin_wgrad_planes_applicable(const odin_geom& g);
int odin_wgrad_planes_launch(const float* U, const float* V, float* slab, int* rows_out, int B, int OH,
                             int OW, int CI, int CO, int want_bias, int grad_u, const uint32_t* g_amax,
                             const uint32_t* a_amax, void* stream);

bool odin_fconv_planes_applicable(const odin_geom& g);
void odin_fconv_planes_set_stamps(void* buf);
int odin_fconv_planes_launch(const float* in, const float* w, const float* bias, const float* aux,
                             float* out, float* colsum, int* rows_out, int B, int OH, int OW, int CI, int CO,
                             int epi, const uint32_t* in_amax, uint32_t* out_amax, void* stream);

bool odin_igemm_applicable(int tmode, const odin_geom& g);
void odin_igemm_set_stamps(void* buf);
int odin_igemm_tiles(int tmode, const odin_geom& g);
int odin_igemm_launch(int tmode, const float* in, const float* w, const float* bias, const float* aux,
                      int aux_act, float* out, float* colsum, int B, int H, int W, int CI, int OH, int OW,
                      int CO, int KH, int KW, int S, int pt, int pl, int act, uint32_t* out_amax, void* stream);
void odin_igemm_pair_begin();
int odin_igemm_pair_end();
bool odin_igemm_h_applicable(int tmode, const odin_geom& g);
int odin_igemm_h_rows(int tmode, const odin_geom& g);
int odin_igemm_h_launch(int tmode, const float* in, const float* w, const float* bias, const float* aux, int aux_act,
                        float* out, float* colsum, int B, int H, int W, int CI, int OH, int OW, int CO, int KH, int KW,
                        int S, int pt, int pl, int act, const uint32_t* in_amax, int in_is_grad, uint32_t* out_amax,
                        void* stream);
bool odin_igemm_h_wgrad_applicable(const odin_geom& g);
int odin_igemm_h_wgrad_rows(const odin_geom& g);
int odin_igemm_h_wgrad_launch(const float* u, const float* v, float* slab, int slab_stride, int B, int FH, int FW,
                              int CU, int h, int w, int CV, int KH, int KW, int S, int pt, int pl, int want_bias,
                              int grad_u, const uint32_t* g_amax, const uint32_t* a_amax, void* stream);
bool odin_igemm_wgrad_applicable(const odin_geom& g);
int odin_igemm_wgrad_rows(const odin_geom& g);
int odin_igemm_wgrad_launch(const float* u, const float* v, float* slab, int slab_stride, int B, int FH,
                            int FW, int CU, int h, int w, int CV, int KH, int KW, int S, int pt, int pl,
                            int want_bias, void* stream);

struct odin_tail_args {
  const float *w1, *b1, *target, *scale;
  float *logits, *llk_part, *slab;
  int C1;
};
int odin_gather_generic(int mode_t, int wmode, const odin_geom& g, const float* in, const float* w, const float* bias,
                        int act, const float* aux, int aux_act, float* out, float* colsum_slab, int max_blocks,
                        int* rows_out, const odin_tail_args* tail, int* n_part_out, void* stream);
int odin_wgrad_generic(const odin_geom& g, const float* in, const float* dy, float* slab, int want_bias, int* rows_out,
                       void* stream);
```

### odin_ai_amd/engine.py

```python
from __future__ import annotations

import ctypes as C
import math
from typing import Callable, Dict, List, NamedTuple, Optional, Sequence, Tuple

import numpy as np
import torch

from . import _lib
from ._lib import ACT, ConvDesc, ReduceJob


def same_pads(n: int, k: int, s: int) -> Tuple[int, int, int]:
  out = -(-n // s)
  total = max((out - 1) * s + k - n, 0)
  return out, total // 2, total - total // 2


class ParamLayout:

  def __init__(self):
    self.entries: List[Tuple[tuple, Tuple[int, ...], int]] = []
    self.size = 0

  def add(self, key, shape) -> int:
    off = self.size
    self.entries.append((key, tuple(shape), off))
    self.size += int(np.prod(shape))
    return off

  def pad_to(self, mult=4):
    self.size = (self.size + mult - 1) // mult * mult

  def views(self, flat: torch.Tensor) -> Dict[tuple, torch.Tensor]:
    return {k: flat[o:o + int(np.prod(s))].view(s) for k, s, o in self.entries}


class LayerRec:
  __slots__ = ('kind', 'act', 'key', 'w_off', 'b_off', 'w_n', 'b_n', 'in_shape', 'out_shape',
               'desc', 'K', 'N', 'center')


def build_layers(net: str, layers: Sequence[tuple], in_shape: Tuple[int, ...],
                 layout: ParamLayout) -> Tuple[List[LayerRec], Tuple[int, ...]]:
  recs: List[LayerRec] = []
  shp = tuple(in_shape)
  center = False
  for li, L in enumerate(layers):
    kind = L[0]
    if kind == 'center':
      center = True
      continue
    if kind == 'flatten':
      shp = (int(np.prod(shp)),)
      continue
    if kind == 'reshape':
      assert int(np.prod(L[1])) == int(np.prod(shp))
      shp = tuple(L[1])
      continue
    r = LayerRec()
    r.kind, r.key, r.center = kind, (net, li), center
    r.in_shape = shp
    r.desc = None
    r.K = r.N = 0
    if kind == 'conv':
      _, co, k, s, act = L
      H, W, Ci = shp
      OH, pt, _ = same_pads(H, k, s)
      OW, pl, _ = same_pads(W, k, s)
      r.act = act
      r.out_shape = (OH, OW, co)
      r.desc = dict(H=H, W=W, Cin=Ci, OH=OH, OW=OW, Cout=co, K=k, stride=s, pad_t=pt, pad_l=pl)
      wshape = (k, k, Ci, co)
    elif kind == 'deconv':
      _, co, k, s, act = L
      H, W, Ci = shp
      OH, OW = H * s, W * s
      _, pt, _ = same_pads(OH, k, s)
      _, pl, _ = same_pads(OW, k, s)
      r.act = act
      r.out_shape = (OH, OW, co)
      r.desc = dict(H=H, W=W, Cin=Ci, OH=OH, OW=OW, Cout=co, K=k, stride=s, pad_t=pt, pad_l=pl)
      wshape = (k, k, co, Ci)
      assert not center
    elif kind == 'dense':
      _, u, act = L
      assert len(shp) == 1, 'dense needs a flat input (add a flatten layer)'
      r.act, r.K, r.N = act, shp[0], u
      r.out_shape = (u,)
      wshape = (shp[0], u)
      assert not center
    else:
      raise ValueError(f'unknown layer kind {kind!r}')
    r.w_n = int(np.prod(wshape))
    r.b_n = wshape[-1] if kind != 'deconv' else wshape[2]
    r.w_off = layout.add((net, li, 'w'), wshape)
    r.b_off = layout.add((net, li, 'b'), (r.b_n,))
    center = False
    shp = r.out_shape
    recs.append(r)
  return recs, shp


RANGE_WORDS = 2048


class NetProgram:

  def __init__(self, lib, recs: List[LayerRec], B: int, device, params: torch.Tensor,
               grads: torch.Tensor, max_rows: int, range_words: Optional[torch.Tensor] = None,
               act_words: Optional[torch.Tensor] = None, use_act_words: bool = True, small_wgrad_gf: float = 0.8,
               direct_wgrad: bool = False, fuse_first_wgrad: bool = False):
    self.lib, self.recs, self.B, self.device = lib, recs, B, device
    self.fuse_first = bool(fuse_first_wgrad) and self._first_pair_qualifies()
    self.params, self.grads = params, grads
    f32 = dict(dtype=torch.float32, device=device)
    self.act_words = (torch.zeros(len(recs) * RANGE_WORDS, dtype=torch.int32, device=device)
                      if act_words is None else act_words)
    assert self.act_words.numel() == len(recs) * RANGE_WORDS and self.act_words.is_contiguous()
    self.range_words = (torch.zeros(len(recs) * RANGE_WORDS, dtype=torch.int32, device=device)
                        if range_words is None else range_words)
    assert self.range_words.numel() == len(recs) * RANGE_WORDS and self.range_words.is_contiguous()
    self.outs = [torch.empty((B,) + r.out_shape, **f32) for r in recs]
    self.gouts = [torch.empty((B,) + r.out_shape, **f32) for r in recs]
    self.descs = []
    for r in recs:
      if r.desc is not None:
        d = r.desc
        cd = _lib.conv_desc(B, d['H'], d['W'], d['Cin'], d['OH'], d['OW'], d['Cout'],
                            d['K'], d['stride'], d['pad_t'], d['pad_l'], r.act, r.center)
        i = len(self.descs)
        cd.dx_amax = (self.range_words.data_ptr() + 4 * RANGE_WORDS * (i - 1)) if i > 0 else None
        self.descs.append(cd)
      else:
        self.descs.append(None)
    self.dy_word = [self.word(i) if i + 1 < len(recs) else None for i in range(len(recs))]
    self.dx_word = [self.word(i - 1) if i > 0 else None for i in range(len(recs))]
    for i, cd in enumerate(self.descs):
      if cd is not None:
        cd.dy_amax = self.dy_word[i]
    self.reads_x = [bool(use_act_words) and self._reads_x(i) for i in range(len(recs))]
    self.x_word: List[Optional[int]] = [None] * len(recs)
    self.y_word: List[Optional[int]] = [None] * len(recs)
    for i in range(1, len(recs)):
      if self.reads_x[i]:
        self.x_word[i] = self.y_word[i - 1] = self.aword(i - 1)
    for i, cd in enumerate(self.descs):
      if cd is not None:
        cd.x_amax, cd.y_amax = self.x_word[i], self.y_word[i]
    self.wslabs: List[Optional[torch.Tensor]] = [None] * len(recs)
    self.direct_wgrad = bool(direct_wgrad)
    self.wdirect = [False] * len(recs)
    self.wrows = [0] * len(recs)
    self.bslabs: List[Optional[torch.Tensor]] = [None] * len(recs)
    self.brows = [0] * len(recs)
    self.small_wgrad = []
    for r in recs:
      if r.desc is not None:
        d = r.desc
        mac = B * (d['OH'] * d['OW'] if r.kind == 'conv' else d['H'] * d['W']) * d['K'] ** 2 * \
            d['Cin'] * d['Cout']
      else:
        mac = B * r.K * r.N
      self.small_wgrad.append(2 * mac < float(small_wgrad_gf) * 1e9)
    self._plan_slabs()

  def word(self, i: int) -> int:
    return self.range_words.data_ptr() + 4 * RANGE_WORDS * i

  def aword(self, i: int) -> int:
    return self.act_words.data_ptr() + 4 * RANGE_WORDS * i

  def _reads_x(self, i: int) -> bool:
    r = self.recs[i]
    if self.descs[i] is None:
      return bool(self.lib.odin_dense_reads_x_range(self.B, r.K, r.N))
    fn = self.lib.odin_conv2d_reads_x_range if r.kind == 'conv' else self.lib.odin_deconv2d_reads_x_range
    return bool(fn(C.byref(self.descs[i])))

  def set_x_word(self, i: int, valid: bool) -> None:
    w = self.aword(i - 1) if (valid and self.reads_x[i]) else None
    self.x_word[i] = w
    if self.descs[i] is not None:
      self.descs[i].x_amax = w

  def set_top_word(self, kept: bool, n: Optional[int] = None) -> Optional[int]:
    n = len(self.recs) - 1 if n is None else n
    self.dy_word[n] = self.word(n) if kept else None
    if self.descs[n] is not None:
      self.descs[n].dy_amax = self.dy_word[n]
    return self.dy_word[n]

  def check_range_words(self, upto: Optional[int] = None, first: int = 0) -> None:
    n = len(self.recs) if upto is None else upto
    for i in range(first, n):
      if self.dy_word[i] is None or self.dy_word[i] != self.word(i):
        continue
      blk = self.range_words[RANGE_WORDS * i:RANGE_WORDS * (i + 1)]
      bound = float(blk.view(torch.float32).max().item())
      t = self.gouts[i]
      m = float(torch.nan_to_num(t, nan=0.0, posinf=0.0, neginf=0.0).abs().max().item())
      assert bound >= m, f'range word of gouts[{i}] ({self.recs[i].kind}): {bound} < max|t| = {m}'

  def dgrad_keeps_range(self, j: int) -> bool:
    if j <= 0 or j >= len(self.recs):
      return False
    if self.descs[j] is None:
      return self.bslabs_wanted(j - 1) is False and bool(
          self.lib.odin_dense_dgrad_keeps_range(self.B, self.recs[j].K, self.recs[j].N))
    fn = (self.lib.odin_conv2d_dgrad_keeps_range if self.recs[j].kind == 'conv'
          else self.lib.odin_deconv2d_dgrad_keeps_range)
    return bool(fn(C.byref(self.descs[j]), ACT[self.recs[j - 1].act]))

  def _first_pair_qualifies(self) -> bool:
    if len(self.recs) < 2 or any(r.kind != 'conv' for r in self.recs[:2]):
      return False
    r0, r1 = self.recs[0], self.recs[1]
    k4s2 = dict(K=4, stride=2, pad_t=1, pad_l=1)
    return (r0.act == 'elu' and r0.desc == dict(H=64, W=64, Cin=1, OH=32, OW=32, Cout=32, **k4s2) and
            r1.desc == dict(H=32, W=32, Cin=32, OH=16, OW=16, Cout=32, **k4s2) and not r1.center)

  def bslabs_wanted(self, i: int) -> bool:
    return self.recs[i].kind == 'deconv'

  def _plan_slabs(self):
    lib, B = self.lib, self.B
    f32 = dict(dtype=torch.float32, device=self.device)
    rows = C.c_int(0)
    for i, r in enumerate(self.recs):
      d = self.descs[i]
      if r.kind == 'conv':
        lib.odin_conv2d_wgrad(None, None, None, C.byref(rows), C.byref(d), None)
        n = r.w_n + r.b_n
        if i == 0 and self.fuse_first:
          r1 = C.c_int(0)
          try:
            lib.odin_conv2d_dgrad_first(None, None, None, ACT[r.act], None, None, None, C.byref(self.descs[1]), None, None,
                                        C.byref(r1), C.byref(d), None)
            rows.value = max(rows.value, r1.value)
          except _lib.OdinError:
            self.fuse_first = False
      elif r.kind == 'deconv':
        lib.odin_deconv2d_wgrad(None, None, None, C.byref(rows), C.byref(d), None)
        r1, r2 = C.c_int(0), C.c_int(0)
        lib.odin_deconv2d_bwd(None, None, None, None, ACT[self.recs[i - 1].act] if i > 0 else 0, None, None, C.byref(r2),
                              None, C.byref(r1), C.byref(d), None)
        rows.value = max(rows.value, r1.value)
        n = r.w_n
      else:
        lib.odin_dense_wgrad(None, None, None, C.byref(rows), B, r.K, r.N, None)
        n = r.w_n + r.b_n
      self.wrows[i] = rows.value
      if (self.direct_wgrad and r.kind == 'dense' and rows.value == 1 and r.b_off == r.w_off + r.w_n and
          self.grads[r.w_off:].data_ptr() % 16 == 0):
        self.wslabs[i] = self.grads[r.w_off:r.w_off + n].view(1, n)
        self.wdirect[i] = True
        continue
      self.wslabs[i] = torch.empty((rows.value, n), **f32)
      if r.kind == 'deconv':
        assert i + 1 < len(self.recs), 'a network may not END with a Conv2DTranspose'
        self.bslabs[i] = torch.empty((lib.odin_max_slab_rows(), r.b_n), **f32)

  def w(self, i):
    r = self.recs[i]
    return self.params[r.w_off:r.w_off + r.w_n]

  def b(self, i):
    r = self.recs[i]
    return self.params[r.b_off:r.b_off + r.b_n]

  def forward(self, x: torch.Tensor, st, upto: Optional[int] = None, start: int = 0):
    lib, B = self.lib, self.B
    h = x
    for i in range(start, len(self.recs) if upto is None else upto):
      r = self.recs[i]
      y = self.outs[i]
      if r.kind == 'conv':
        lib.odin_conv2d_fwd(h.data_ptr(), self.w(i).data_ptr(), self.b(i).data_ptr(),
                            y.data_ptr(), C.byref(self.descs[i]), st)
      elif r.kind == 'deconv':
        lib.odin_deconv2d_fwd(h.data_ptr(), self.w(i).data_ptr(), self.b(i).data_ptr(),
                              y.data_ptr(), C.byref(self.descs[i]), st)
      else:
        lib.odin_dense_fwd_ranged(h.data_ptr(), self.w(i).data_ptr(), self.b(i).data_ptr(),
                                  y.data_ptr(), B, r.K, r.N, ACT[r.act], self.x_word[i], self.y_word[i], st)
      h = y
    return h

  def backward(self, x: torch.Tensor, gout_last: torch.Tensor, st,
               dx_out: Optional[torch.Tensor] = None, last: Optional[int] = None,
               skip_bias_of_last: bool = False, data_only: bool = False,
               fork=None, side_jobs: Optional[list] = None, first: int = 0,
               fuse_first: bool = False) -> List[ReduceJob]:
    fuse_first = (fuse_first and self.fuse_first and first == 0 and dx_out is None and not data_only and
                  (fork is None or not (fork.wants(self.small_wgrad[0]) or fork.wants(self.small_wgrad[1]))))
    lib, B = self.lib, self.B
    n = len(self.recs) if last is None else last + 1
    jobs: List[ReduceJob] = []
    g = gout_last
    rows = C.c_int(0)
    for i in range(n - 1, first - 1, -1):
      r, d = self.recs[i], self.descs[i]
      xin = x if i == 0 else self.outs[i - 1]
      slab = self.wslabs[i]
      wst = st if (fork is None or not fork.wants(self.small_wgrad[i])) else fork(i)
      if i > 0:
        prev = self.recs[i - 1]
        dst, aux, aux_act = self.gouts[i - 1], self.outs[i - 1], ACT[prev.act]
        bslab = self.bslabs[i - 1]
      elif dx_out is not None:
        dst, aux, aux_act, bslab = dx_out, None, 0, None
      else:
        dst = None
      auxp = aux.data_ptr() if (dst is not None and aux is not None and aux_act != 0) else None
      bsp = bslab.data_ptr() if (dst is not None and bslab is not None) else None
      both = (not data_only) and dst is not None and wst is st
      wrows = C.c_int(0)
      if fuse_first and i == 1:
        r0, slab0, rows0 = self.recs[0], self.wslabs[0], C.c_int(0)
        lib.odin_conv2d_wgrad(xin.data_ptr(), g.data_ptr(), slab.data_ptr(), C.byref(wrows), C.byref(d), st)
        lib.odin_conv2d_dgrad_first(g.data_ptr(), self.w(1).data_ptr(), auxp, aux_act, None, None, None, C.byref(d),
                                    x.data_ptr(),
                                    slab0.data_ptr(), C.byref(rows0), C.byref(self.descs[0]), st)
        assert 0 < wrows.value <= self.wrows[1] and 0 < rows0.value <= self.wrows[0]
        jobs.append(ReduceJob(slab.data_ptr(), self.grads[r.w_off:].data_ptr(), slab.shape[1], wrows.value,
                              slab.shape[1], 0))
        jobs.append(ReduceJob(slab0.data_ptr(), self.grads[r0.w_off:].data_ptr(), slab0.shape[1], rows0.value,
                              slab0.shape[1], 0))
        break
      if both:
        if r.kind == 'conv':
          lib.odin_conv2d_bwd(xin.data_ptr(), g.data_ptr(), self.w(i).data_ptr(), auxp, aux_act, dst.data_ptr(),
                              bsp, C.byref(rows), slab.data_ptr(), C.byref(wrows), C.byref(d), st)
        elif r.kind == 'deconv':
          lib.odin_deconv2d_bwd(xin.data_ptr(), g.data_ptr(), self.w(i).data_ptr(), auxp, aux_act, dst.data_ptr(),
                                bsp, C.byref(rows), slab.data_ptr(), C.byref(wrows), C.byref(d), st)
        else:
          lib.odin_dense_bwd_ranged(xin.data_ptr(), g.data_ptr(), self.w(i).data_ptr(), auxp, aux_act, dst.data_ptr(),
                                    bsp, C.byref(rows), slab.data_ptr(), C.byref(wrows), B, r.K, r.N, 1, 1,
                                    self.dy_word[i], self.dx_word[i], self.x_word[i], st)
      elif data_only:
        pass
      elif r.kind == 'conv':
        lib.odin_conv2d_wgrad(xin.data_ptr(), g.data_ptr(), slab.data_ptr(), C.byref(wrows),
                              C.byref(d), wst)
      elif r.kind == 'deconv':
        lib.odin_deconv2d_wgrad(xin.data_ptr(), g.data_ptr(), slab.data_ptr(), C.byref(wrows),
                                C.byref(d), wst)
      else:
        lib.odin_dense_bwd_ranged(xin.data_ptr(), g.data_ptr(), None, None, 0, None, None, None, slab.data_ptr(),
                                  C.byref(wrows), B, r.K, r.N, 1, 0, self.dy_word[i], None, self.x_word[i], wst)
      if not data_only:
        assert 0 < wrows.value <= self.wrows[i]
        n_red = slab.shape[1]
        if skip_bias_of_last and i == n - 1 and r.kind != 'deconv':
          n_red = r.w_n
        tgt = side_jobs if (side_jobs is not None and wst is not st) else jobs
        if self.wdirect[i]:
          assert wrows.value == 1
        else:
          tgt.append(ReduceJob(slab.data_ptr(), self.grads[r.w_off:].data_ptr(), n_red, wrows.value,
                               slab.shape[1], 0))
      if dst is None:
        break
      if not both:
        if r.kind == 'conv':
          lib.odin_conv2d_dgrad(g.data_ptr(), self.w(i).data_ptr(), auxp, aux_act, dst.data_ptr(),
                                bsp, C.byref(rows), C.byref(d), st)
        elif r.kind == 'deconv':
          lib.odin_deconv2d_dgrad(g.data_ptr(), self.w(i).data_ptr(), auxp, aux_act,
                                  dst.data_ptr(), bsp, C.byref(rows), C.byref(d), st)
        else:
          lib.odin_dense_bwd(None, g.data_ptr(), self.w(i).data_ptr(), auxp, aux_act, dst.data_ptr(), bsp,
                             C.byref(rows), None, None, B, r.K, r.N, 0, 1, self.dy_word[i], self.dx_word[i], st)
      if bslab is not None and not data_only:
        pr = self.recs[i - 1]
        jobs.append(ReduceJob(bslab.data_ptr(), self.grads[pr.b_off:].data_ptr(), pr.b_n,
                              rows.value, pr.b_n, 0))
      g = dst
    return jobs


OBS_MODE = {'gaussian': 0, 'gaussian_softplus1': 1, 'qlogistic': 2}
MIXQL_K = 10


def observation_maps(observation: str, C: int) -> int:
  if observation == 'bernoulli':
    return C
  if observation == 'mixqlogistic':
    return MIXQL_K * (2 * C + C * (C - 1) // 2 + 1)
  return 2 * C
H_ALPHA, H_B1, H_B2, H_EPS, H_GSCALE, H_INVB, H_KLW, H_BETA, H_TCCOEF, H_TCGRAD = range(10)
H_CAP = 15
N_HYPER = 16
MMD_KERNELS = {'gaussian': 0, 'linear': 1}
PRIOR_KEY_SALT = 0x6D6D6470 << 32


class LatentTerm(NamedTuple):
  value: Optional[torch.Tensor] = None
  dz: Optional[torch.Tensor] = None
  dloc: Optional[torch.Tensor] = None
  dscale: Optional[torch.Tensor] = None
  launch: Optional[Callable] = None

  def ptr(self) -> Optional[int]:
    return None if self.value is None else self.value.data_ptr()


class VAEEngine:

  def __init__(self, enc_layers, dec_layers, in_shape, zdim, batch_size, device,
               observation='bernoulli', analytic=False, free_bits=None, tc=None, lib=None,
               params: Optional[torch.Tensor] = None, world_size: int = 1, seed: int = 1,
               optim_state: Optional[Tuple[torch.Tensor, torch.Tensor]] = None,
               force_dp: bool = False, reverse: bool = True, capacity: bool = False,
               range_words: Optional[torch.Tensor] = None, *,
               act_words: bool = True, hyper_ring: bool = True, hyper_ring_rows: int = 128, fuse_norm: bool = True,
               overlap_wgrad: Optional[str] = None, early_reduce: bool = False, defer_wgrad: bool = False,
               fuse_first_wgrad: bool = True, side_streams: int = 2, small_wgrad_gf: float = 0.8, dp_buckets: Optional[int] = None,
               neck: bool = True, neck_bwd: Optional[bool] = None, static_top_word: bool = True,
               latent_reg: Optional[str] = None, reg_coef: float = 1.0, mmd_kernel: str = 'gaussian',
               mmd_prior_samples: int = 100, dip_lambda: Tuple[float, float] = (1.0, 2.0), prior_seed: int = 0,
               vamprior_components: Optional[int] = None, pseudoinputs_mean: float = -0.05,
               pseudoinputs_std: float = 0.01, pseudoinputs=None,
               vq_codes: Optional[int] = None, vq_code_size: Optional[int] = None, vq_commitment: float = 0.25,
               vq_ema: bool = False, vq_ema_decay: float = 0.99, vq_epsilon: float = 1e-5, vq_state=None):
    self.lib = lib if lib is not None else _lib.load()
    self.device = torch.device(device)
    self.B, self.D = int(batch_size), int(zdim)
    self.capacity_on = bool(capacity)
    self.in_shape = tuple(in_shape)
    self.observation = observation
    self.set_kl_form(analytic, reverse)
    self.free_bits = -1.0 if free_bits is None else float(free_bits)
    self.tc_mode, self.world_size, self.seed = tc, int(world_size), int(seed)
    self.is_dp = self.world_size > 1 or bool(force_dp)
    self.tc_sharded = tc == 'betatc' and self.is_dp
    if latent_reg not in (None, 'mmd', 'dip_i', 'dip_ii'):
      raise ValueError(f"latent_reg={latent_reg!r}: expected None, 'mmd', 'dip_i' or 'dip_ii'")
    if latent_reg is not None and tc is not None:
      raise ValueError(f'latent_reg={latent_reg!r} cannot be combined with tc={tc!r}')
    if latent_reg == 'mmd' and mmd_kernel not in MMD_KERNELS:
      raise NotImplementedError(f'mmd_kernel={mmd_kernel!r}: the HIP path offers {sorted(MMD_KERNELS)}')
    self.reg_mode, self.reg_coef = latent_reg, float(reg_coef)
    self.reg_sharded = latent_reg is not None and self.is_dp
    self.vamp_K = None if vamprior_components is None else int(vamprior_components)
    if self.vamp_K is not None:
      self._check_vamprior(analytic, reverse, free_bits, tc, latent_reg, capacity, range_words)
    self.vq_K = None if vq_codes is None else int(vq_codes)
    if self.vq_K is not None:
      self._check_vq(free_bits, tc, latent_reg, capacity, range_words, neck_bwd)
      self.vq_cw, self.vq_ema = float(vq_commitment), bool(vq_ema)
      self.vq_decay, self.vq_eps = float(vq_ema_decay), float(vq_epsilon)
    f32 = dict(dtype=torch.float32, device=self.device)
    self.layout = ParamLayout()
    self.enc_recs, eo = build_layers('enc', enc_layers, self.in_shape, self.layout)
    assert len(eo) == 1, 'encoder must end with a flat output'
    self.hdim = eo[0]
    if self.vq_K is None:
      self.lat_w_off = self.layout.add(('lat', 'w'), (self.hdim, 2 * self.D))
      self.lat_b_off = self.layout.add(('lat', 'b'), (2 * self.D,))
    else:
      self.lat_w_off = self.lat_b_off = 0
      self.D = self.hdim
      self._resolve_vq_code_size(vq_code_size)
    self.dec_recs, do = build_layers('dec', dec_layers, (self.D,), self.layout)
    if self.vq_K is not None and not self.vq_ema:
      self.vq_cb_off = self.layout.add(('vq', 'codebook'), (self.vq_K, self.vq_Cs))
    if self.vamp_K is not None:
      self.vamp_u_off = self.layout.add(('vamp', 'u'), (self.vamp_K, int(np.prod(self.in_shape))))
    self.layout.pad_to(4)
    self.out_shape = do
    C_in = self.in_shape[-1]
    assert tuple(do) == self.in_shape[:-1] + (observation_maps(observation, C_in),), (do, self.in_shape)
    n = self.layout.size
    own_params = params is None
    self.params = params if params is not None else torch.zeros(n, **f32)
    assert self.params.numel() == n
    if self.vamp_K is not None and (own_params or pseudoinputs is not None):
      self._init_pseudoinputs(pseudoinputs, pseudoinputs_mean, pseudoinputs_std)
    self.grads = torch.zeros(n, **f32)
    if optim_state is not None:
      self.m, self.v = optim_state
    else:
      self.m = torch.zeros(n, **f32)
      self.v = torch.zeros(n, **f32)
    self.n_params = sum(int(np.prod(s)) for _, s, _ in self.layout.entries)
    B, D = self.B, self.D
    mr = self.lib.odin_max_slab_rows()
    ne = len(self.enc_recs)
    nl = ne + len(self.dec_recs)
    self._shared_ranges = range_words is not None
    npw = 2 * ne if self.vamp_K is not None else 0
    if self.vq_K is not None:
      npw = 1
    self.range_words = (range_words if range_words is not None else
                        torch.zeros((2 * nl + npw) * RANGE_WORDS, dtype=torch.int32, device=self.device))
    assert self.range_words.numel() == (2 * nl + npw) * RANGE_WORDS
    gw, aw = self.range_words[:nl * RANGE_WORDS], self.range_words[nl * RANGE_WORDS:2 * nl * RANGE_WORDS]
    self.enc = NetProgram(self.lib, self.enc_recs, B, self.device, self.params, self.grads, mr,
                          range_words=gw[:ne * RANGE_WORDS], act_words=aw[:ne * RANGE_WORDS],
                          use_act_words=act_words, small_wgrad_gf=small_wgrad_gf, fuse_first_wgrad=fuse_first_wgrad)
    self.dec = NetProgram(self.lib, self.dec_recs, B, self.device, self.params, self.grads, mr,
                          range_words=gw[ne * RANGE_WORDS:], act_words=aw[ne * RANGE_WORDS:],
                          use_act_words=act_words, small_wgrad_gf=small_wgrad_gf)
    self._act_words_dirty = False
    self._bern_keeps_top = observation == 'bernoulli' and bool(static_top_word)
    if self._bern_keeps_top:
      self.dec.set_top_word(True)
    self.p = torch.empty(B, 2 * D, **f32)
    self.dp = torch.empty(B, 2 * D, **f32)
    self.eps = torch.zeros(B, D, **f32)
    self.z = torch.empty(B, D, **f32)
    self.dz = torch.empty(B, D, **f32)
    self.kl = torch.empty(B, **f32)
    self.fbmask = torch.empty(B, **f32)
    self.dh_e = torch.empty(B, self.hdim, **f32)
    n_per = int(np.prod(self.in_shape))
    self.n_per = n_per
    npart = self._observation_fwd_bwd(None, None, None, None, None, None)
    self.llk_part = torch.empty(B * max(npart, (n_per + 1023) // 1024), **f32)
    self.llk = torch.empty(B, **f32)
    self.out8 = torch.zeros(8, **f32)
    self.out4 = self.out8[:4]
    self.n_part = 0
    if self.vq_K is None:
      rows = C.c_int(0)
      self.lib.odin_dense_wgrad(None, None, None, C.byref(rows), B, self.hdim, 2 * D, None)
      self.lat_slab = torch.empty(rows.value, self.hdim * 2 * D + 2 * D, **f32)
      self.lat_rows = rows.value
    if tc == 'betatc':
      self.tc_ws = torch.zeros(self.lib.odin_total_correlation_workspace(
          B, B * self.world_size if self.tc_sharded else B, D), **f32)
      self.tc_dz = torch.empty(B, D, **f32)
      self.tc_dloc = torch.empty(B, D, **f32)
      self.tc_dscale = torch.empty(B, D, **f32)
      if self.tc_sharded:
        Bg = B * self.world_size
        self.tc_pz_local = torch.empty(B, 3 * D, **f32)
        self.tc_pz_all = torch.empty(Bg, 3 * D, **f32)
        self.tc_p_all = torch.empty(Bg, 2 * D, **f32)
        self.tc_part_all = torch.empty(2, Bg, D, **f32)
    if latent_reg is not None:
      self._plan_latent_reg(f32, mmd_kernel, mmd_prior_samples, dip_lambda, prior_seed)
    if self.vq_K is None:
      self._plan_fused_tail(f32)
      self._plan_gauss_head(f32)
      self._plan_latent_block(f32)
      self._neck_bwd_opt = neck_bwd
      self._plan_neck(f32, bool(neck))
    else:
      self._plan_vq(f32, own_params, vq_state)
    if self.vamp_K is not None:
      self._plan_vamprior(f32, mr, act_words, small_wgrad_gf)
    self._term = self._plan_term()
    self.ws = torch.empty(4096, **f32)
    self.gnorm2 = torch.zeros(1, **f32)
    self.flag = torch.zeros(1, dtype=torch.int32, device=self.device)
    self.skip_hit = torch.zeros(1, dtype=torch.int32, device=self.device)
    self.skipped_update = torch.zeros(1, dtype=torch.int32, device=self.device)
    offs = [o for _, _, o in self.layout.entries] + [self.n_params_end()]
    self.seg_offsets = torch.tensor(offs, dtype=torch.int64, device=self.device)
    self._ring = [torch.zeros(N_HYPER + 4, dtype=torch.float32) for _ in range(8)]
    self._ring_ev = [None] * 8
    if self.device.type == 'cuda':
      self._ring = [t.pin_memory() for t in self._ring]
    self._ring_i = 0
    self.hyper = torch.zeros(N_HYPER + 4, **f32)
    self.ring_rows = int(hyper_ring_rows)
    assert self.ring_rows >= 8 and self.ring_rows & (self.ring_rows - 1) == 0
    self.hyper_ring = torch.zeros(self.ring_rows, N_HYPER + 4, **f32)
    self.fuse_norm = bool(fuse_norm)
    self.hyper_staged = torch.zeros(32, **f32)
    self._ring_host = torch.zeros(self.ring_rows, N_HYPER + 4, dtype=torch.float32)
    if self.device.type == 'cuda':
      self._ring_host = self._ring_host.pin_memory()
    self._ring_filled_to = -1
    self._ring_last_t = None
    self._ring_live = False
    self._ring_args = None
    self._ring_copy_ev = [None, None]
    self.use_hyper_ring = bool(hyper_ring)
    self.step_count = 0
    self.side_stream = torch.cuda.Stream(self.device) if self.device.type == 'cuda' else None
    n_side = int(side_streams)
    self.side_streams = ([self.side_stream] + [torch.cuda.Stream(self.device) for _ in range(n_side - 1)]
                         if self.side_stream is not None else [])
    assert overlap_wgrad in (None, 'small'), overlap_wgrad
    self.overlap_wgrad = overlap_wgrad
    self.early_reduce = bool(early_reduce)
    self.defer_wgrad = bool(defer_wgrad)
    self.graph = None
    self.debug_check_ranges = False
    self._jobs_keepalive = None
    self._jobs_cover_ok: Dict[tuple, bool] = {}
    self.comm = None
    big = self.grads.numel() * 4 >= (8 << 20)
    self.dp_buckets = int(dp_buckets or 0) or (2 if (self.world_size >= 4 and big) else 1)
    self.dec_start = min(o for k, _, o in self.layout.entries if k[0] == 'dec')

  def _plan_latent_reg(self, f32, mmd_kernel, M, dip_lambda, prior_seed):
    B, D, W = self.B, self.D, self.world_size
    if self.reg_mode == 'mmd':
      self.mmd_kernel, self.mmd_M = MMD_KERNELS[mmd_kernel], int(M)
      self.prior_key = (int(prior_seed) ^ PRIOR_KEY_SALT) & 0xFFFFFFFFFFFFFFFF
      self.reg_ws = torch.zeros(self.lib.odin_mmd_workspace(B, B * W, self.mmd_M, D), **f32)
      self.reg_dz = torch.empty(B, D, **f32)
      self.reg_y = torch.zeros(self.mmd_M, D, **f32)
      if self.reg_sharded:
        self.reg_z_all = torch.empty(B * W, D, **f32)
    else:
      self.dip_type2 = int(self.reg_mode == 'dip_ii')
      self.dip_lambda = (float(dip_lambda[0]), float(dip_lambda[1]))
      self.reg_ws = torch.zeros(self.lib.odin_dip_workspace(W, D), **f32)
      self.reg_dloc = torch.empty(B, D, **f32)
      self.reg_dscale = torch.empty(B, D, **f32)
      bs = 1 + 2 * D + D * D
      self.dip_block_local = self.reg_ws[4:4 + bs]
      self.dip_blocks = self.reg_ws[4 + bs:4 + bs + W * bs]
    self._prior_explicit = False

  def _plan_term(self) -> LatentTerm:
    if self.tc_mode == 'betatc':
      return LatentTerm(self.tc_ws, self.tc_dz, self.tc_dloc, self.tc_dscale,
                        self._tc_global if self.tc_sharded else self._tc_local)
    if self.reg_mode == 'mmd':
      return LatentTerm(self.reg_ws, dz=self.reg_dz, launch=self._reg_global if self.reg_sharded else self._mmd_local)
    if self.reg_mode is not None:
      return LatentTerm(self.reg_ws, dloc=self.reg_dloc, dscale=self.reg_dscale if self.dip_type2 else None,
                        launch=self._reg_global if self.reg_sharded else self._dip_local)
    if self.vamp_K is not None:
      return LatentTerm(self.vamp_ws, dz=self.vamp_dz, launch=self._vamp_term)
    if self.vq_K is not None:
      return LatentTerm(self.out8[4:])
    return LatentTerm()

  def _tc_local(self, st):
    self.lib.odin_total_correlation_fwd_bwd(self.z.data_ptr(), self.p.data_ptr(), self.tc_ws.data_ptr(),
                                            self.tc_dz.data_ptr(), self.tc_dloc.data_ptr(), self.tc_dscale.data_ptr(),
                                            self.hp(H_TCGRAD), self.B, self.D, st)

  def _tc_global(self, st):
    self._tc_pack()
    self._tc_gather()
    self._tc_shard(st)
    self._tc_scatter()

  def _mmd_local(self, st):
    self.lib.odin_mmd_fwd_bwd(self.z.data_ptr(), self._prior_ptr(), self.reg_ws.data_ptr(), self.reg_dz.data_ptr(),
                              None, self.hp(H_TCGRAD), self.B, self.mmd_M, self.D, self.mmd_kernel, self.prior_key,
                              self.hp(N_HYPER), st)

  def _dip_local(self, st):
    self.lib.odin_dip_fwd_bwd(self.p.data_ptr(), self.reg_ws.data_ptr(), self.reg_dloc.data_ptr(),
                              self.reg_dscale.data_ptr() if self.dip_type2 else None, None, self.hp(H_TCGRAD), self.B,
                              self.D, self.dip_type2, self.dip_lambda[0], self.dip_lambda[1], st)

  def _reg_global(self, st):
    if self.reg_mode != 'mmd':
      self._dip_moments(st)
    for _, fn in self._reg_segments():
      fn()

  def _vamp_term(self, st):
    self.lib.odin_vamprior_fwd_bwd(self.z.data_ptr(), self.vamp_pu.data_ptr(), self.vamp_ws.data_ptr(),
                                   self.vamp_c.data_ptr(), self.vamp_dz.data_ptr(), self.vamp_dpu.data_ptr(), None,
                                   self.hp(H_TCGRAD), self.B, self.vamp_K, self.D, st)

  VAMP_CLIP = (1e-6, 1.0 - 1e-6)

  def _check_vamprior(self, analytic, reverse, free_bits, tc, latent_reg, capacity, range_words):
    K = self.vamp_K
    if not 1 <= K <= 1024:
      raise ValueError(f'vamprior_components={K}: the mixture kernel takes 1 .. 1024 components')
    if not 1 <= self.B <= 4096 or not 1 <= self.D <= 64:
      raise ValueError(f'vamprior_components: batch_size={self.B}, zdim={self.D} outside the kernel (4096, 64)')
    self._check_no_term('vamprior_components', 'the same step scalars', tc, latent_reg)
    if not reverse:
      raise NotImplementedError('vamprior_components with reverse=False: KL(p || q) needs samples of the mixture')
    if analytic:
      raise NotImplementedError('vamprior_components with analytic=True: the KL to a mixture has no closed form')
    self._check_plain_kl('vamprior_components', 'the clamp acts on the standard-normal KL only', free_bits, capacity,
                         range_words)

  def _check_no_term(self, what, why, tc, latent_reg):
    if tc is not None:
      raise ValueError(f'{what} cannot be combined with tc={tc!r} ({why})')
    if latent_reg is not None:
      raise ValueError(f'{what} cannot be combined with latent_reg={latent_reg!r} ({why})')

  def _check_plain_kl(self, what, why_free_bits, free_bits, capacity, range_words):
    if free_bits is not None:
      raise NotImplementedError(f'{what} with free_bits: {why_free_bits}')
    if capacity:
      raise NotImplementedError(f'{what} with capacity=True (BetaCapacityVAE) is not offered')
    if self.is_dp:
      raise NotImplementedError(f'{what} under data parallelism (world_size > 1 / force_dp) is not offered')
    if range_words is not None:
      raise NotImplementedError(f'{what} with shared range_words is not offered')

  def _init_pseudoinputs(self, pseudoinputs, mean, std):
    K, n = self.vamp_K, int(np.prod(self.in_shape))
    dst = self.params[self.vamp_u_off:self.vamp_u_off + K * n]
    if pseudoinputs is not None:
      a = torch.as_tensor(np.asarray(pseudoinputs, dtype=np.float32)).reshape(-1)
      if a.numel() != K * n:
        raise ValueError(f'pseudoinputs: expected [{K}, {n}], got {tuple(np.shape(pseudoinputs))}')
      dst.copy_(a.to(self.device))
      return
    g = torch.Generator(device='cpu').manual_seed(self.seed + 0x76616D70)
    dst.copy_((torch.randn(K * n, generator=g) * float(std) + float(mean)).to(self.device))

  def _plan_vamprior(self, f32, max_rows, act_words, small_wgrad_gf):
    K, D, ne = self.vamp_K, self.D, len(self.enc_recs)
    if any(r.kind == 'deconv' for r in self.enc_recs):
      raise NotImplementedError('vamprior_components: an encoder with Conv2DTranspose layers is not offered')
    nl = ne + len(self.dec_recs)
    pw = self.range_words[2 * nl * RANGE_WORDS:]
    self.penc = NetProgram(self.lib, self.enc_recs, K, self.device, self.params, self.grads, max_rows,
                           range_words=pw[:ne * RANGE_WORDS], act_words=pw[ne * RANGE_WORDS:],
                           use_act_words=act_words, small_wgrad_gf=small_wgrad_gf)
    self._penc_words_dirty = False
    self._enc_tall: List[torch.Tensor] = []
    for i in range(ne):
      n = self.enc.wslabs[i].shape[1]
      tall = torch.empty(self.enc.wrows[i] + self.penc.wrows[i], n, **f32)
      self._enc_tall.append(tall)
      self.enc.wslabs[i] = tall[:self.enc.wrows[i]]
      self.penc.wslabs[i] = tall[self.enc.wrows[i]:]
    rows = C.c_int(0)
    self.lib.odin_dense_wgrad(None, None, None, C.byref(rows), K, self.hdim, 2 * D, None)
    self.plat_rows = rows.value
    self.lat_slab = torch.empty(self.lat_rows + rows.value, self.lat_slab.shape[1], **f32)
    if self.lat_block:
      self.lb_slabl = torch.empty(self.lb_rows + rows.value, self.lb_slabl.shape[1], **f32)
    if self.neck:
      self.nk_slabl = torch.empty(self.nk_rows + rows.value, self.nk_slabl.shape[1], **f32)
    n_u = K * self.n_per
    self.vamp_u = torch.empty((K,) + self.in_shape, **f32)
    self.vamp_du = torch.empty(1, n_u, **f32)
    self.vamp_pu = torch.empty(K, 2 * D, **f32)
    self.vamp_dpu = torch.empty(K, 2 * D, **f32)
    self.vamp_c = torch.empty(self.B, **f32)
    self.vamp_dz = torch.empty(self.B, D, **f32)
    self.vamp_ws = torch.zeros(self.lib.odin_vamprior_workspace(self.B, K, D), **f32)

  def pseudo_forward(self, st=None):
    lib, K, D = self.lib, self.vamp_K, self.D
    st = self.stream() if st is None else st
    lo, hi = self.VAMP_CLIP
    lib.odin_clip_range_fwd(self.params[self.vamp_u_off:].data_ptr(), self.vamp_u.data_ptr(), self.vamp_u.numel(),
                            lo, hi, st)
    if self._penc_words_dirty:
      ne = len(self.enc_recs)
      lib.odin_range_reset(self.penc.act_words.data_ptr(), ne, st)
    self._penc_words_dirty = True
    h = self.penc.forward(self.vamp_u, st)
    lib.odin_dense_fwd(h.data_ptr(), self.params[self.lat_w_off:].data_ptr(), self.params[self.lat_b_off:].data_ptr(),
                       self.vamp_pu.data_ptr(), K, self.hdim, 2 * D, 0, st)
    return self.vamp_pu

  def vamprior_log_prob(self, z: torch.Tensor, out: torch.Tensor, st=None):
    st = self.stream() if st is None else st
    N, D, K = z.shape[0], self.D, self.vamp_K
    assert z.shape == (N, D) and z.is_contiguous() and out.is_contiguous() and out.numel() == N
    step = min(N, 4096)
    ws = torch.zeros(self.lib.odin_vamprior_workspace(step, K, D), dtype=torch.float32, device=self.device)
    for i0 in range(0, N, step):
      n = min(step, N - i0)
      self.lib.odin_vamprior_fwd_bwd(z[i0:].data_ptr(), self.vamp_pu.data_ptr(), ws.data_ptr(), out[i0:].data_ptr(),
                                     None, None, None, None, n, K, D, st)
    out.copy_(-0.5 * (z * z).sum(1) - 0.5 * D * math.log(2.0 * math.pi) - out)
    return out

  def _backward_pseudo(self, st, jobs, late_jobs):
    lib, K, D, ne = self.lib, self.vamp_K, self.D, len(self.enc_recs)
    g0 = self.grads.data_ptr()
    by_dst = {jb.dst: jb for jb in list(jobs) + list(late_jobs)}

    def data_job(off):
      jb = by_dst.get(g0 + 4 * off)
      assert jb is not None, f'no data-pass reduction job for the parameter at offset {off}'
      return jb
    h = self.penc.outs[-1]
    last = self.enc_recs[-1]
    jb = data_job(self.lat_w_off)
    slab = next(t for t in (self.lat_slab, getattr(self, 'lb_slabl', None), getattr(self, 'nk_slabl', None))
                if t is not None and t.data_ptr() == jb.src)
    assert jb.rows + self.plat_rows <= slab.shape[0] and jb.stride == slab.shape[1] and jb.n == slab.shape[1]
    rows = C.c_int(0)
    lib.odin_dense_wgrad(h.data_ptr(), self.vamp_dpu.data_ptr(), slab[jb.rows:].data_ptr(), C.byref(rows), K, self.hdim,
                         2 * D, st)
    assert 0 < rows.value <= self.plat_rows
    jb.rows += rows.value
    aux_act = ACT[last.act]
    top = self.penc.set_top_word(True)
    lib.odin_dense_bwd(None, self.vamp_dpu.data_ptr(), self.params[self.lat_w_off:].data_ptr(),
                       h.data_ptr() if aux_act != 0 else None, aux_act, self.penc.gouts[-1].data_ptr(), None,
                       C.byref(rows), None, None, K, self.hdim, 2 * D, 0, 1, None, top, st)
    for i, r in enumerate(self.enc_recs):
      jb = data_job(r.w_off)
      tall = self._enc_tall[i]
      assert jb.src == tall.data_ptr() and jb.rows + self.penc.wrows[i] <= tall.shape[0]
      self.penc.wslabs[i] = tall[jb.rows:]
    pjobs = self.penc.backward(self.vamp_u, self.penc.gouts[-1], st, dx_out=self.vamp_du)
# ... 143 lines not shown
    self.tail_keeps_range = bool(self.lib.odin_bernoulli_tail_keeps_range(
        int(a.kind == 'deconv'), C.byref(self.dec.descs[-2]), b.desc['Cout']))
    self.tail_rows, self.tail_npart = rows.value, npart.value
    co, c1 = a.desc['Cout'], b.desc['Cout']
    self.tail_slab = torch.empty(rows.value, co * c1 + c1 + co, **f32)
    self.tail_llk_part = torch.empty(self.B * npart.value, **f32)

  def _plan_gauss_tail(self, f32):
    a, b = self.dec_recs[-2], self.dec_recs[-1]
    Cc = self.in_shape[-1]
    if not (b.kind == 'conv' and b.desc['K'] == 1 and b.desc['stride'] == 1 and b.act == 'linear'
            and b.desc['Cout'] == 2 * Cc and a.kind == 'deconv'):
      return
    d = self.dec.descs[-2]
    if not self.lib.odin_gaussian_tail_applicable(C.byref(d), Cc):
      return
    rows, npart = C.c_int(0), C.c_int(0)
    self.lib.odin_gaussian_tail_fwd_bwd(None, None, None, None, None, None, None, None, None, C.byref(npart), None,
                                        C.byref(rows), None, C.byref(d), Cc, OBS_MODE[self.observation], None)
    self.fused_tail = True
    self.tail_mode = OBS_MODE[self.observation]
    self.tail_keeps_range = True
    self.tail_rows, self.tail_npart = rows.value, npart.value
    co, c1 = a.desc['Cout'], b.desc['Cout']
    self.tail_slab = torch.empty(rows.value, co * c1 + c1 + co, **f32)
    self.tail_llk_part = torch.empty(self.B * npart.value, **f32)

  def _plan_gauss_head(self, f32):
    self.gauss_head = self._used_head = False
    recs = self.dec_recs
    if self.observation not in ('gaussian', 'gaussian_softplus1', 'bernoulli') or len(recs) < 2:
      return
    a, b = recs[-2], recs[-1]
    Cc = self.in_shape[-1]
    bern = self.observation == 'bernoulli'
    if not (b.kind == 'conv' and b.desc['K'] == 1 and b.desc['stride'] == 1 and b.act == 'linear'
            and b.desc['Cout'] == (Cc if bern else 2 * Cc) and a.kind in ('conv', 'deconv')):
      return
    if not bern and self.fused_tail:
      return
    if bern and self.fused_tail:
      d = a.desc
      mac = self.B * (d['OH'] * d['OW'] if a.kind == 'conv' else d['H'] * d['W']) * d['K'] ** 2 * d['Cin'] * d['Cout']
      if self.tail_keeps_range or 2.0 * mac < 1.2e9:
        return
    self.head_mode = 3 if bern else OBS_MODE[self.observation]
    rows, npart = C.c_int(0), C.c_int(0)
    try:
      self.lib.odin_gaussian_head_fwd_bwd(None, None, None, None, None, None, None, None, C.byref(npart), None,
                                          C.byref(rows), None, None, self.B, self.n_per // Cc, b.desc['Cin'], Cc,
                                          self.head_mode, ACT[a.act], None, None)
    except _lib.OdinError:
      return
    self.gauss_head = True
    self.fused_tail = False
    self.head_rows, self.head_npart = rows.value, npart.value
    cin, co = b.desc['Cin'], b.desc['Cout']
    self.head_slab = torch.empty(rows.value, cin * co + co, **f32)
    self.head_colsum = torch.empty(rows.value, cin, **f32) if a.kind == 'deconv' else None
    self.head_llk_part = torch.empty(self.B * npart.value, **f32)

  def _plan_latent_block(self, f32):
    self.lat_block = self._used_block = False
    recs = self.dec_recs
    if len(recs) < 2 or recs[0].kind != 'dense' or self.enc_recs[-1].kind == 'deconv':
      return
    rows = self.lib.odin_latent_block_rows(self.B, self.hdim, self.D, recs[0].N)
    if rows <= 0:
      return
    self.lat_block, self.lb_rows = True, rows
    D, N0 = self.D, recs[0].N
    self.lb_slab0 = torch.empty(rows, D * N0 + N0, **f32)
    self.lb_slabl = torch.empty(rows, self.hdim * 2 * D + 2 * D, **f32)

  def _plan_neck(self, f32, enabled: bool):
    self.neck = self._used_neck = False
    er, dr = self.enc_recs, self.dec_recs
    if not (enabled and self.lat_block and len(er) >= 3 and len(dr) >= 3):
      return
    c3, d4, d0, t1 = er[-2], er[-1], dr[0], dr[1]
    if not (c3.kind == 'conv' and d4.kind == 'dense' and d0.kind == 'dense' and t1.kind == 'deconv'):
      return
    g = c3.desc
    if not (g['H'] == 8 and g['W'] == 8 and g['Cin'] == 64 and g['Cout'] == 64 and g['K'] == 4 and g['stride'] == 2
            and g['pad_t'] == 1 and g['pad_l'] == 1 and not c3.center and d4.K == 1024):
      return
    t = t1.desc
    if not (t['H'] == 4 and t['W'] == 4 and t['Cout'] == 64 and t['K'] == 4 and t['stride'] == 2 and t['pad_t'] == 1
            and t['pad_l'] == 1 and d0.N == 16 * t['Cin']):
      return
    rows = self.lib.odin_neck_rows(self.B, d4.N, self.D, t['Cin'])
    if rows <= 0:
      return
    if self.params[d4.w_off:].data_ptr() % 16 != 0:
      return
    self.neck, self.nk_rows = True, rows
    ne = len(er)
    self.enc.y_word[ne - 3] = self.enc.aword(ne - 3)
    if self.enc.descs[ne - 3] is not None:
      self.enc.descs[ne - 3].y_amax = self.enc.y_word[ne - 3]
    A = _lib.NeckArgs()
    A.B, A.P, A.D, A.C0 = self.B, d4.N, self.D, t['Cin']
    A.act2, A.act3, A.act4, A.act0, A.act1 = (ACT[er[-3].act], ACT[c3.act], ACT[d4.act], ACT[d0.act], ACT[t1.act])
    A.seed = self.seed
    A.x, A.x_amax = self.enc.outs[ne - 3].data_ptr(), self.enc.y_word[ne - 3]
    A.w3, A.b3, A.y3 = self.enc.w(ne - 2).data_ptr(), self.enc.b(ne - 2).data_ptr(), self.enc.outs[ne - 2].data_ptr()
    A.w4, A.b4, A.y4 = self.enc.w(ne - 1).data_ptr(), self.enc.b(ne - 1).data_ptr(), self.enc.outs[ne - 1].data_ptr()
    A.wl, A.bl = self.params[self.lat_w_off:].data_ptr(), self.params[self.lat_b_off:].data_ptr()
    A.eps = self.eps.data_ptr()
    A.p, A.kl, A.fbmask = self.p.data_ptr(), self.kl.data_ptr(), self.fbmask.data_ptr()
    A.w0, A.b0, A.y0 = self.dec.w(0).data_ptr(), self.dec.b(0).data_ptr(), self.dec.outs[0].data_ptr()
    A.w1, A.b1, A.y1 = self.dec.w(1).data_ptr(), self.dec.b(1).data_ptr(), self.dec.outs[1].data_ptr()
    self._nk = A
    C0 = t['Cin']
    self.nk_slab1 = torch.empty(rows, 16 * 64 * C0, **f32)
    self.nk_slab0 = torch.empty(rows, self.D * 16 * C0 + 16 * C0, **f32)
    self.nk_slabl = torch.empty(rows, d4.N * 2 * self.D + 2 * self.D, **f32)

  def _neck_fwd(self, eps, st, y1_word: bool = True, enc_only: bool = False):
    A = self._nk
    A.y1 = None if enc_only else self.dec.outs[1].data_ptr()
    A.analytic, A.free_bits = int(self.analytic), float(self.free_bits)
    A.step_dev = self.hp(N_HYPER)
    A.eps_in = None if eps is None else self.eps.data_ptr()
    A.z = self.z.data_ptr()
    A.capacity = self.hp(H_CAP) if self.capacity_on else None
    A.y1_amax = self.dec.y_word[1] if y1_word else None
    self.lib.odin_neck_fwd(C.byref(A), st)

  def _dec_first(self) -> int:
    return 2 if self._bwd_neck() else int(self._bwd_block())

  def _neck_bwd(self, dzx, tl, ts, st, jobs):
    lib, A, ne = self.lib, self._nk, len(self.enc_recs)
    c3, d4, d0, t1 = self.enc_recs[-2], self.enc_recs[-1], self.dec_recs[0], self.dec_recs[1]
    A.dy1 = self.dec.gouts[1].data_ptr()
    A.klw = self.hp(H_KLW)
    A.dz_extra, A.dloc_x, A.dscale_x = dzx, tl, ts
    A.dz, A.dp = self.dz.data_ptr(), self.dp.data_ptr()
    A.dh4, A.dy3, A.dx = (self.enc.gouts[ne - 1].data_ptr(), self.enc.gouts[ne - 2].data_ptr(),
                          self.enc.gouts[ne - 3].data_ptr())
    A.dh4_amax, A.dy3_amax, A.dx_amax = self.enc.set_top_word(True), self.enc.word(ne - 2), self.enc.word(ne - 3)
    A.slab1, A.slab0, A.slabl = self.nk_slab1.data_ptr(), self.nk_slab0.data_ptr(), self.nk_slabl.data_ptr()
    lib.odin_neck_bwd(C.byref(A), st)
    for slab, off in ((self.nk_slab1, t1.w_off), (self.nk_slab0, d0.w_off), (self.nk_slabl, self.lat_w_off)):
      jobs.append(self._slab_job(slab, off, self.nk_rows))
    wrows = C.c_int(0)
    lib.odin_wgrad_pair_begin()
    try:
      slab = self.enc.wslabs[ne - 2]
      lib.odin_conv2d_wgrad(self.enc.outs[ne - 3].data_ptr(), self.enc.gouts[ne - 2].data_ptr(), slab.data_ptr(),
                            C.byref(wrows), C.byref(self.enc.descs[ne - 2]), st)
      jobs.append(self._slab_job(slab, c3.w_off, wrows.value))
      slab = self.enc.wslabs[ne - 1]
      lib.odin_dense_bwd_ranged(self.enc.outs[ne - 2].data_ptr(), self.enc.gouts[ne - 1].data_ptr(), None, None, 0, None,
                                None, None, slab.data_ptr(), C.byref(wrows), self.B, d4.K, d4.N, 1, 0,
                                self.enc.dy_word[ne - 1], None, None, st)
    finally:
      lib.odin_wgrad_pair_end()
    jobs.append(self._slab_job(slab, d4.w_off, wrows.value))

  def _bwd_neck(self) -> bool:
    if not (self.neck and self._used_neck) or (self.is_dp and self.dp_buckets >= 2):
      return False
    return self._nk.P == 128 if self._neck_bwd_opt is None else bool(self._neck_bwd_opt)

  def _bwd_block(self) -> bool:
    return self.lat_block and self._used_block and not (self.is_dp and self.dp_buckets >= 2)

  def _slab_job(self, slab, off, rows, n=None) -> ReduceJob:
    return ReduceJob(slab.data_ptr(), self.grads[off:].data_ptr(), slab.shape[1] if n is None else n, rows,
                     slab.shape[1], 0)

  def hp(self, idx):
    return self.hyper.data_ptr() + 4 * idx

  def stream(self):
    if self.device.type == 'cuda':
      return torch.cuda.current_stream(self.device).cuda_stream
    return None

  def param_views(self) -> Dict[tuple, torch.Tensor]:
    return self.layout.views(self.params)

  def grad_views(self) -> Dict[tuple, torch.Tensor]:
    return self.layout.views(self.grads)

  def load_params(self, P: Dict[tuple, np.ndarray]):
    views = self.param_views()
    assert set(P.keys()) == set(views.keys()), (sorted(P.keys()), sorted(views.keys()))
    for k, v in P.items():
      views[k].copy_(torch.as_tensor(np.asarray(v), dtype=torch.float32).to(self.device))

  def set_hyper(self, lr=1e-3, beta=1.0, b1=0.9, b2=0.999, eps=1e-7, grad_scale=1.0,
                t: Optional[int] = None, tc_coef: Optional[float] = None,
                skip_enable: bool = True, extra: Optional[Sequence[float]] = None,
                capacity: Optional[float] = None, reg_coef: Optional[float] = None):
    t = self.step_count if t is None else t
    self._ring_live = False
    self._ring_i = (self._ring_i + 1) % len(self._ring)
    h = self._ring[self._ring_i]
    if self._ring_ev[self._ring_i] is not None:
      self._ring_ev[self._ring_i].synchronize()
    self._fill_row(h, t, lr=lr, beta=beta, b1=b1, b2=b2, eps=eps, grad_scale=grad_scale, tc_coef=tc_coef,
                   skip_enable=skip_enable, extra=extra, capacity=capacity, reg_coef=reg_coef)
    self.hyper.copy_(h, non_blocking=True)
    if self.device.type == 'cuda':
      ev = torch.cuda.Event()
      ev.record(torch.cuda.current_stream(self.device))
      self._ring_ev[self._ring_i] = ev

  def _fill_row(self, h, t, lr=1e-3, beta=1.0, b1=0.9, b2=0.999, eps=1e-7, grad_scale=1.0, tc_coef=None,
                skip_enable=True, extra=None, capacity=None, reg_coef=None):
    tt = max(int(t), 1)
    Bg = self.B * self.world_size
    h[H_ALPHA] = lr * math.sqrt(1.0 - b2 ** tt) / (1.0 - b1 ** tt)
    h[H_B1], h[H_B2], h[H_EPS], h[H_GSCALE] = b1, b2, eps, grad_scale
    h[H_INVB] = 1.0 / Bg
    h[H_KLW] = beta / Bg
    h[H_BETA] = beta
    h[H_TCCOEF] = (beta - 1.0) if self.tc_mode == 'betatc' else 0.0
    h[H_TCGRAD] = (beta - 1.0) if self.tc_mode == 'betatc' else 0.0
    if tc_coef is not None:
      h[H_TCCOEF] = tc_coef
    if self.reg_mode is not None:
      h[H_TCCOEF] = h[H_TCGRAD] = self.reg_coef if reg_coef is None else float(reg_coef)
    if self.vamp_K is not None:
      h[H_TCCOEF] = beta
      h[H_TCGRAD] = beta / Bg
    if self.vq_K is not None:
      h[H_TCCOEF] = self.vq_cw + (0.0 if self.vq_ema else 1.0)
    if extra is not None:
      for i, val in enumerate(extra):
        h[10 + i] = float(val)
    if self.capacity_on:
      assert capacity is not None, 'this engine was built with capacity=True: pass the capacity C(step)'
      h[H_CAP] = float(capacity)
    h[N_HYPER:].view(torch.int32)[0] = int(t)
    h[N_HYPER:].view(torch.int32)[1] = int(skip_enable)

  def _ring_step(self, t: int, args: dict, schedule=None) -> None:
    R = self.ring_rows
    row = self._ring_host[t % R]
    want = torch.zeros(N_HYPER + 4, dtype=torch.float32)
    wa = dict(args)
    if schedule is not None:
      wa.update(schedule(t))
    if 'when_skip_update' in wa:
      wa['skip_enable'] = t >= int(wa.pop('when_skip_update'))
    self._fill_row(want, t, **wa)
    hit = (self._ring_live and self._ring_last_t == t - 1 and self._ring_filled_to >= t and
           torch.equal(want.view(torch.int32), row.view(torch.int32)))
    self._ring_last_t = t
    key = tuple(sorted((k, v if not isinstance(v, (list, tuple)) else tuple(v)) for k, v in args.items()))
    stable = schedule is not None or self._ring_args is None or key == self._ring_args
    self._ring_args = key
    if not hit:
      self.set_hyper(t=t, **wa)
      if not stable:
        return
      self._ring_filled_to = t
    if self._ring_filled_to - t < R // 4:
      lo, hi = self._ring_filled_to + 1, t + R // 2
      for old in self._ring_copy_ev:
        if old is not None:
          old.synchronize()
      self._ring_copy_ev.append(None)
      self._ring_copy_ev.pop(0)
      for u in range(lo, hi + 1):
        a = dict(args)
        if schedule is not None:
          a.update(schedule(u))
        if 'when_skip_update' in a:
          a['skip_enable'] = u >= int(a.pop('when_skip_update'))
        self._fill_row(self._ring_host[u % R], u, **a)
      a0, a1 = lo % R, hi % R
      spans = [(a0, a1 + 1)] if a0 <= a1 else [(a0, R), (0, a1 + 1)]
      for x0, x1 in spans:
        self.hyper_ring[x0:x1].copy_(self._ring_host[x0:x1], non_blocking=True)
      if self.device.type == 'cuda':
        ev = torch.cuda.Event()
        ev.record(torch.cuda.current_stream(self.device))
        self._ring_copy_ev[-1] = ev
      self._ring_filled_to = hi
    self._ring_live = True

  def _clear_stale_act_words(self, st):
    if self._shared_ranges:
      return
    if self._act_words_dirty:
      nl = len(self.enc_recs) + len(self.dec_recs)
      self.lib.odin_range_reset(self.range_words.data_ptr() + 4 * RANGE_WORDS * nl,
                                nl + (1 if self.vq_K is not None else 0), st)
    self._act_words_dirty = True

  def run_encoder(self, x: torch.Tensor, eps: Optional[torch.Tensor] = None, st=None):
    st = self.stream() if st is None else st
    assert x.shape == (self.B,) + self.in_shape and x.is_contiguous()
    self.x = x
    self._clear_stale_act_words(st)
    self._latent_fwd(x, eps, st, self.neck, self.lat_block, for_step=False)
    return (self.enc.outs[-1] if self.vq_K is not None else self.p), self.z

  def _latent_fwd(self, x, eps, st, neck: bool, block: bool, for_step: bool):
    lib, B, D = self.lib, self.B, self.D
    if self.vq_K is not None:
      self._vq_assign(self.enc.forward(x, st), st, count=for_step)
      return self.z, 0
    if eps is not None and eps is not self.eps:
      self.eps.copy_(eps)
    lw, lb = self.params[self.lat_w_off:], self.params[self.lat_b_off:]
    cap = self.hp(H_CAP) if self.capacity_on else None
    if neck:
      self.enc.forward(x, st, upto=len(self.enc_recs) - 2)
      self._neck_fwd(eps, st, y1_word=for_step, enc_only=not for_step)
      return self.dec.outs[1], 2
    if block:
      h_e = self.enc.forward(x, st)
      r0 = self.dec_recs[0]
      lib.odin_latent_block_fwd(h_e.data_ptr(), lw.data_ptr(), lb.data_ptr(),
                                None if eps is None else self.eps.data_ptr(), self.eps.data_ptr(),
                                self.seed, self.hp(N_HYPER), self.p.data_ptr(), self.z.data_ptr(),
                                self.kl.data_ptr(), self.fbmask.data_ptr(), self.dec.w(0).data_ptr(),
                                self.dec.b(0).data_ptr(), self.dec.outs[0].data_ptr(), B, self.hdim, D,
                                r0.N, ACT[r0.act], int(self.analytic), self.free_bits, cap, st)
      return self.dec.outs[0], 1
    if eps is None:
      lib.odin_rng_normal(self.eps.data_ptr(), B * D, self.seed, self.hp(N_HYPER), st)
    h_e = self.enc.forward(x, st)
    lib.odin_dense_fwd(h_e.data_ptr(), lw.data_ptr(), lb.data_ptr(), self.p.data_ptr(), B,
                       self.hdim, 2 * D, 0, st)
    lib.odin_latent_fwd(self.p.data_ptr(), self.eps.data_ptr(), self.z.data_ptr(),
                        self.kl.data_ptr(), self.fbmask.data_ptr(), B, D, int(self.analytic),
                        self.free_bits, cap, st)
    return self.z, 0

  def run_decoder(self, z: torch.Tensor, st=None):
    st = self.stream() if st is None else st
    assert z.shape == (self.B, self.D) and z.is_contiguous()
    self._clear_stale_act_words(st)
    if len(self.dec_recs) > 1:
      self.dec.set_x_word(1, True)
    if self.vq_K is not None and self._vq_zq_word is not None:
      self.lib.odin_absmax(z.data_ptr(), z.numel(), self._vq_zq_word, st)
    return self.dec.forward(z, st)

  def observation_llk(self, h_d: torch.Tensor, x: torch.Tensor, out: torch.Tensor, st=None):
    st = self.stream() if st is None else st
    npart = self._observation_fwd_bwd(h_d.data_ptr(), x.data_ptr(), self.llk_part.data_ptr(),
                                      self.dec.gouts[-1].data_ptr(), None, st)
    self.lib.odin_sum_parts(self.llk_part.data_ptr(), npart, out.data_ptr(), self.B, st)
    return out

  def _observation_fwd_bwd(self, h_d, x, part, dlogits, top_word, st) -> int:
    lib, B, Cc = self.lib, self.B, self.in_shape[-1]
    inv_b = None if h_d is None else self.hp(H_INVB)
    npart = C.c_int(0)
    if self.observation == 'bernoulli':
      lib.odin_elbo_bernoulli_fwd_bwd_ranged(h_d, x, part, dlogits, inv_b, B, self.n_per, C.byref(npart), top_word, st)
    elif self.observation == 'mixqlogistic':
      lib.odin_elbo_mixqlogistic_fwd_bwd(h_d, x, part, dlogits, inv_b, B, self.n_per // Cc, Cc, MIXQL_K,
                                         C.byref(npart), st)
    else:
      lib.odin_elbo_gaussian_fwd_bwd(h_d, x, part, dlogits, inv_b, B, self.n_per // Cc, Cc,
                                     OBS_MODE[self.observation], C.byref(npart), st)
    return npart.value

  def forward(self, x: torch.Tensor, eps: Optional[torch.Tensor] = None, st=None,
              fused: bool = True, tc_ptr: Optional[int] = None, finalize: bool = True,
              tc_split: bool = False, after_latent=None, prior: Optional[torch.Tensor] = None):
    lib, B = self.lib, self.B
    st = self.stream() if st is None else st
    assert x.shape == (B,) + self.in_shape and x.is_contiguous()
    self.x = x
    if self.reg_mode == 'mmd':
      self._prior_explicit = prior is not None
      if prior is not None and prior is not self.reg_y:
        self.reg_y.copy_(prior.reshape(self.reg_y.shape))
    else:
      assert prior is None, 'an explicit prior sample needs latent_reg="mmd"'
    self._used_block = self.lat_block and fused
    self._used_neck = self.neck and fused
    if self.vamp_K is not None:
      self.pseudo_forward(st)
    self._clear_stale_act_words(st)
    if len(self.dec_recs) > 1:
      self.dec.set_x_word(1, not self._used_block)
    dec_in, dec_start = self._latent_fwd(x, eps, st, self._used_neck, self._used_block, for_step=True)
    if after_latent is not None:
      after_latent()
    npart = C.c_int(0)
    if self.fused_tail:
      nd2 = len(self.dec_recs) - 2
      self.dec.descs[nd2].dy_amax = self.dec.word(nd2)
    self._used_head = False
    if self.gauss_head:
      nd2 = len(self.dec_recs) - 2
      self.dec.set_top_word(True, nd2)
    if self.gauss_head and fused:
      nd = len(self.dec_recs)
      hm = self.dec.forward(dec_in, st, upto=nd - 1, start=dec_start)
      a, b = self.dec_recs[-2], self.dec_recs[-1]
      Cc = self.in_shape[-1]
      rows = C.c_int(0)
      lib.odin_gaussian_head_fwd_bwd(
          hm.data_ptr(), self.dec.w(nd - 1).data_ptr(), self.dec.b(nd - 1).data_ptr(), x.data_ptr(),
          self.dec.outs[-1].data_ptr(), None, self.dec.gouts[-2].data_ptr(), self.head_llk_part.data_ptr(),
          C.byref(npart), self.head_slab.data_ptr(), C.byref(rows),
          self.head_colsum.data_ptr() if self.head_colsum is not None else None, self.hp(H_INVB), B,
          self.n_per // Cc, b.desc['Cin'], Cc, self.head_mode, ACT[a.act], self.dec.word(nd - 2), st)
      assert rows.value == self.head_rows and npart.value == self.head_npart
      self._used_fused, self._used_head = False, True
      llk_part = self.head_llk_part
      h_d = self.dec.outs[-1]
    elif self.fused_tail and fused:
      nd = len(self.dec_recs)
      h = self.dec.forward(dec_in, st, upto=nd - 2, start=dec_start)
      a, b = self.dec_recs[-2], self.dec_recs[-1]
      rows = C.c_int(0)
      if self.tail_mode is not None:
        lib.odin_gaussian_tail_fwd_bwd(
            h.data_ptr(), self.dec.w(nd - 2).data_ptr(), self.dec.b(nd - 2).data_ptr(),
            self.dec.w(nd - 1).data_ptr(), self.dec.b(nd - 1).data_ptr(), x.data_ptr(),
            self.dec.outs[-1].data_ptr(), self.dec.gouts[-2].data_ptr(), self.tail_llk_part.data_ptr(),
            C.byref(npart), self.tail_slab.data_ptr(), C.byref(rows), self.hp(H_INVB),
            C.byref(self.dec.descs[-2]), self.in_shape[-1], self.tail_mode, st)
        assert rows.value == self.tail_rows and npart.value == self.tail_npart
      else:
        lib.odin_bernoulli_tail_fwd_bwd(
            int(a.kind == 'deconv'), h.data_ptr(), self.dec.w(nd - 2).data_ptr(),
            self.dec.b(nd - 2).data_ptr(), self.dec.w(nd - 1).data_ptr(),
            self.dec.b(nd - 1).data_ptr(), x.data_ptr(), self.dec.outs[-1].data_ptr(),
            self.dec.gouts[-2].data_ptr(), self.tail_llk_part.data_ptr(), C.byref(npart),
            self.tail_slab.data_ptr(), C.byref(rows), self.hp(H_INVB), C.byref(self.dec.descs[-2]),
            b.desc['Cout'], st)
      self._used_fused = True
      llk_part = self.tail_llk_part
      h_d = self.dec.outs[-1]
    else:
      self._used_fused = False
      llk_part = self.llk_part
      h_d = self.dec.forward(dec_in, st, start=dec_start)
    if not (self._used_fused or self._used_head):
      npart.value = self._observation_fwd_bwd(h_d.data_ptr(), x.data_ptr(), self.llk_part.data_ptr(),
                                              self.dec.gouts[-1].data_ptr(),
                                              self.dec.dy_word[-1] if self._bern_keeps_top else None, st)
    self.n_part = npart.value
    if self.tc_sharded and tc_split:
      self._tc_pack()
      self._llk_part_used = llk_part
      return h_d
    if self.reg_sharded and tc_split:
      if self.reg_mode != 'mmd':
        self._dip_moments(st)
      self._llk_part_used = llk_part
      return h_d
    if self._term.launch is not None:
      self._term.launch(st)
    self._llk_part_used = llk_part
    if finalize:
      lib.odin_elbo_finalize(llk_part.data_ptr(), self.n_part, self.kl.data_ptr(), self.hp(H_BETA),
                             self._term.ptr() if tc_ptr is None else tc_ptr, self.llk.data_ptr(), self.out4.data_ptr(),
                             B, st)
    return h_d

  def _tc_pack(self):
    D = self.D
    self.tc_pz_local[:, :2 * D].copy_(self.p)
    self.tc_pz_local[:, 2 * D:].copy_(self.z)

  def _tc_gather(self):
    self._comm().all_gather(self.tc_pz_all.view(-1), self.tc_pz_local.view(-1))

  def _tc_shard(self, st=None):
    lib, B, D, W = self.lib, self.B, self.D, self.world_size
    st = self.stream() if st is None else st
    self.tc_p_all.copy_(self.tc_pz_all[:, :2 * D])
    dl, ds = self.tc_part_all[0], self.tc_part_all[1]
    lib.odin_total_correlation_shard(self.z.data_ptr(), self.tc_p_all.data_ptr(),
                                     self.tc_ws.data_ptr(), self.tc_dz.data_ptr(), dl.data_ptr(),
                                     ds.data_ptr(), self.hp(H_TCGRAD), B, B * W, D, st)

  def _tc_scatter(self):
    c = self._comm()
    c.reduce_scatter(self.tc_dloc.view(-1), self.tc_part_all[0].view(-1))
    c.reduce_scatter(self.tc_dscale.view(-1), self.tc_part_all[1].view(-1))
    c.all_reduce(self.tc_ws[:1])

  def _prior_ptr(self):
    return self.reg_y.data_ptr() if self._prior_explicit else None

  def _dip_moments(self, st=None):
    st = self.stream() if st is None else st
    self.lib.odin_dip_moments(self.p.data_ptr(), self.dip_block_local.data_ptr(), self.B, self.D, st)

  def _reg_segments(self):
    lib, B, D, W = self.lib, self.B, self.D, self.world_size
    c = self._comm
    if self.reg_mode == 'mmd':
      def shard():
        rank = c().rank
        lib.odin_mmd_shard(self.z.data_ptr(), self.reg_z_all.data_ptr(), self._prior_ptr(), self.reg_ws.data_ptr(),
                           self.reg_dz.data_ptr(), None, self.hp(H_TCGRAD), B, B * W, self.mmd_M, D, self.mmd_kernel,
                           int(rank == 0), self.prior_key, self.hp(N_HYPER), self.stream())
      return [('c', lambda: c().all_gather(self.reg_z_all.view(-1), self.z.view(-1))),
              ('k', shard),
              ('c', lambda: c().all_reduce(self.reg_ws[:1]))]

    def finish():
      lib.odin_dip_finish(self.dip_blocks.data_ptr(), W, self.p.data_ptr(), self.reg_ws.data_ptr(),
                          self.reg_dloc.data_ptr(), self.reg_dscale.data_ptr() if self.dip_type2 else None, None,
                          self.hp(H_TCGRAD), B, D, self.dip_type2, self.dip_lambda[0], self.dip_lambda[1], self.stream())
    return [('c', lambda: c().all_gather(self.dip_blocks, self.dip_block_local)), ('k', finish)]

  def finalize(self, tc_ptr: Optional[int] = None, st=None):
    st = self.stream() if st is None else st
    self.lib.odin_elbo_finalize(self._llk_part_used.data_ptr(), self.n_part, self.kl.data_ptr(),
                                self.hp(H_BETA), tc_ptr, self.llk.data_ptr(),
                                self.out4.data_ptr(), self.B, st)

  def _fork(self):
    if self.side_stream is None or not (self.overlap_wgrad or self.early_reduce):
      return None, (lambda: None)
    cur = torch.cuda.current_stream(self.device)
    sides = self.side_streams
    nxt = [0]

    def fork(i):
      side = sides[nxt[0] % len(sides)]
      nxt[0] += 1
      ev = torch.cuda.Event()
      ev.record(cur)
      side.wait_event(ev)
      return side.cuda_stream

    small_on = self.overlap_wgrad == 'small'
    fork.wants = lambda small: small_on and bool(small)

    def join():
      for side in sides[:max(1, min(nxt[0], len(sides)))]:
        cur.wait_stream(side)

    return fork, join

  def backward(self, st=None, extra_dz: Optional[torch.Tensor] = None, phase: Optional[str] = None):
    lib = self.lib
    st = self.stream() if st is None else st
    if phase == 'dec':
      jobs, _, _ = self._backward_dec(st, None)
      arr = (ReduceJob * len(jobs))(*jobs)
      self._jobs_keepalive0 = arr
      lib.odin_slab_reduce(arr, len(jobs), st)
      return
    fork, join = self._fork() if phase is None else (None, (lambda: None))
    if phase is None and fork is None and self.defer_wgrad:
      lib.odin_wgrad_planes_defer_begin()
    try:
      jobs, late_jobs, early = ([], [], False) if phase == 'enc' else self._backward_dec(st, fork)
      self._backward_enc(st, extra_dz, fork, jobs, late_jobs)
      join()
    finally:
      lib.odin_wgrad_planes_defer_end(st)
    self._reduce_slabs(jobs, early, st)

  def _backward_dec(self, st, fork):
    lib, B, D = self.lib, self.B, self.D
    late_jobs: list = []
    early = fork is not None and self.early_reduce
    if self._used_fused:
      nd = len(self.dec_recs)
      a, b = self.dec_recs[-2], self.dec_recs[-1]
      co, c1 = a.desc['Cout'], b.desc['Cout']
      jobs = self.dec.backward(self.z, self.dec.gouts[-2], st, dx_out=self.dz, last=nd - 2,
                               skip_bias_of_last=True, fork=fork,
                               side_jobs=late_jobs if early else None, first=self._dec_first())
      ts = self.tail_slab
      jobs.append(self._slab_job(ts, b.w_off, self.tail_rows, n=co * c1 + c1))
      jobs.append(ReduceJob(ts[:, co * c1 + c1:].data_ptr(), self.grads[a.b_off:].data_ptr(), co,
                            self.tail_rows, ts.shape[1], 0))
    elif self._used_head:
      nd = len(self.dec_recs)
      a, b = self.dec_recs[-2], self.dec_recs[-1]
      jobs = self.dec.backward(self.z, self.dec.gouts[-2], st, dx_out=self.dz, last=nd - 2, fork=fork,
                               side_jobs=late_jobs if early else None, first=self._dec_first())
      jobs.append(self._slab_job(self.head_slab, b.w_off, self.head_rows))
      if self.head_colsum is not None:
        jobs.append(self._slab_job(self.head_colsum, a.b_off, self.head_rows, n=a.b_n))
    else:
      jobs = self.dec.backward(self.z, self.dec.gouts[-1], st, dx_out=self.dz, fork=fork,
                               side_jobs=late_jobs if early else None, first=self._dec_first())
    if early and jobs:
      arr0 = (ReduceJob * len(jobs))(*jobs)
      self._jobs_keepalive0 = arr0
      lib.odin_slab_reduce(arr0, len(jobs), fork(-3))
      jobs = []
    return jobs, late_jobs, early

  def _backward_enc(self, st, extra_dz, fork, jobs, late_jobs):
    lib, B, D = self.lib, self.B, self.D
    T = self._term
    assert extra_dz is None or (T.dz is None and self.vq_K is None)
    dzx, tl, ts = (None if t is None else t.data_ptr()
                   for t in (T.dz if extra_dz is None else extra_dz, T.dloc, T.dscale))
    h_e = self.enc.outs[-1]
    last = self.enc_recs[-1]
    aux_act = ACT[last.act]
    lw = self.params[self.lat_w_off:]
    if self.vq_K is not None:
      self._vq_bwd(st, jobs)
    elif self._bwd_neck():
      ne = len(self.enc_recs)
      self._neck_bwd(dzx, tl, ts, st, jobs)
      jobs += self.enc.backward(self.x, self.enc.gouts[ne - 3], st, fork=fork, last=ne - 3,
                                fuse_first=self._fuse_first_now())
    elif self._bwd_block():
      r0 = self.dec_recs[0]
      lib.odin_latent_block_bwd(self.dec.gouts[0].data_ptr(), self.dec.w(0).data_ptr(), self.z.data_ptr(),
                                self.p.data_ptr(), self.eps.data_ptr(), self.fbmask.data_ptr(),
                                self.hp(H_KLW), dzx, tl, ts, lw.data_ptr(), h_e.data_ptr(), aux_act,
                                self.dz.data_ptr(), self.dp.data_ptr(), self.enc.gouts[-1].data_ptr(),
                                self.lb_slab0.data_ptr(), self.lb_slabl.data_ptr(), B, self.hdim, D, r0.N,
                                int(self.analytic), self.enc.set_top_word(True), st)
      jobs.append(self._slab_job(self.lb_slab0, r0.w_off, self.lb_rows))
      jobs.append(self._slab_job(self.lb_slabl, self.lat_w_off, self.lb_rows))
    else:
      lib.odin_latent_bwd(self.p.data_ptr(), self.eps.data_ptr(), self.z.data_ptr(),
                          self.dz.data_ptr(), dzx, self.fbmask.data_ptr(), self.hp(H_KLW), tl, ts,
                          self.dp.data_ptr(), B, D, int(self.analytic), st)
      rows = C.c_int(0)
      lib.odin_dense_wgrad(h_e.data_ptr(), self.dp.data_ptr(), self.lat_slab.data_ptr(),
                           C.byref(rows), B, self.hdim, 2 * D,
                           st if (fork is None or not fork.wants(True)) else fork(-1))
      jobs.append(self._slab_job(self.lat_slab, self.lat_w_off, rows.value))
      auxp = h_e.data_ptr() if aux_act != 0 else None
      bslab = self.enc.bslabs[-1]
      top = self.enc.set_top_word(True)
      lib.odin_dense_bwd(None, self.dp.data_ptr(), lw.data_ptr(), auxp, aux_act, self.enc.gouts[-1].data_ptr(),
                         bslab.data_ptr() if bslab is not None else None, C.byref(rows), None, None, B,
                         self.hdim, 2 * D, 0, 1, None, top, st)
      if bslab is not None:
        jobs.append(self._slab_job(bslab, last.b_off, rows.value))
    if not self._bwd_neck():
      jobs += self.enc.backward(self.x, self.enc.gouts[-1], st, fork=fork, fuse_first=self._fuse_first_now())
    if self.vamp_K is not None:
      self._backward_pseudo(st, jobs, late_jobs)
    jobs += late_jobs
    rw = self.range_words
    jobs.append(ReduceJob(rw.data_ptr(), rw.data_ptr(), rw.numel(), 0, rw.numel(), 0))
    self._act_words_dirty = False

  def _fuse_first_now(self) -> bool:
    return not self.defer_wgrad and not self.debug_check_ranges

  def _reduce_slabs(self, jobs, early, st):
    lib = self.lib
    arr = (ReduceJob * len(jobs))(*jobs)
    self._jobs_keepalive = arr
    if callable(self.debug_check_ranges):
      self.debug_check_ranges(self)
    elif self.debug_check_ranges:
      self.dec.check_range_words(upto=len(self.dec_recs) - 1 if (self._used_fused or self._used_head) else None,
                                 first=self._dec_first() - 1 if self._bwd_neck() else 0)
      self.enc.check_range_words()
    self._norm_parts = 0
    if getattr(self, '_fuse_norm_now', False) and not early:
      nparts = C.c_int(0)
      sig = tuple((jb.dst, jb.n) for jb in jobs)
      ok = self._jobs_cover_ok.get(sig)
      if ok is None:
        ok = self._jobs_cover(jobs)
        if ok:
          lib.odin_slab_reduce_sumsq(arr, len(jobs), self.grads.data_ptr(), self.grads.numel(), None, C.byref(nparts),
                                     None, None, 0, st)
          ok = 0 < nparts.value <= 2048
        self._jobs_cover_ok[sig] = ok
      if not ok:
        lib.odin_slab_reduce(arr, len(jobs), st)
        return
      lib.odin_slab_reduce_sumsq(arr, len(jobs), self.grads.data_ptr(), self.grads.numel(), self.ws.data_ptr(),
                                 C.byref(nparts), self.hyper.data_ptr(), self.hyper_staged.data_ptr(), N_HYPER + 4, st)
      assert 0 < nparts.value <= self.ws.numel(), (nparts.value, self.ws.numel())
      self._norm_parts = nparts.value
      return
    lib.odin_slab_reduce(arr, len(jobs), st)

  def _jobs_cover(self, jobs) -> bool:
    g0, n = self.grads.data_ptr(), self.grads.numel()
    cover = np.zeros(n, dtype=np.int32)
    for jb in jobs:
      off = (jb.dst - g0) // 4 if jb.dst is not None else -1
      if 0 <= off < n:
# ... 218 lines not shown
```

Before: 557,300 images/sec.

## Fuse first encoder conv into second conv's planes kernel

Adds a fused forward kernel that computes the first 4x4 stride-2 conv with ELU (1->32 channels) on the fly from an LDS-staged image, then feeds it straight into the FCONV_PLANES second-layer kernel. Layer-0 outputs are still written for backward, but the separate launch and the layer-1 reread of y0 from global memory go away. The range bound for the first layer comes from an analytic bound (|w| sum times the image bound) when the observation is bernoulli. This costs extra LDS for double-buffered image planes, fewer tiles per workgroup, and more complex in-loop staging.

```diff
diff --git a/include/odin_hip.h b/include/odin_hip.h
--- a/include/odin_hip.h
+++ b/include/odin_hip.h
@@ -60,6 +60,9 @@
 int odin_deconv2d_bwd(const float* x, const float* dy, const float* w, const float* aux, int aux_act, float* dx,
                       float* colsum_slab, int* colsum_rows_out, float* wslab, int* wslab_rows_out,
                       const odin_conv_desc* d, void* stream);
+int odin_conv2d_fwd_first(const float* x, const float* w0, const float* b0, float* y0, const float* w1, const float* b1,
+                          float* y1, const odin_conv_desc* d0, const odin_conv_desc* d1, float x_bound, int* rows_out,
+                          void* stream);
 int odin_conv2d_dgrad_first(const float* dy, const float* w, const float* aux, int aux_act, float* dx,
                             float* colsum_slab, int* colsum_rows_out, const odin_conv_desc* d, const float* x0,
                             float* wslab0, int* wslab0_rows_out, const odin_conv_desc* d0, void* stream);
diff --git a/odin_ai_amd/_lib.py b/odin_ai_amd/_lib.py
--- a/odin_ai_amd/_lib.py
+++ b/odin_ai_amd/_lib.py
@@ -56,6 +56,7 @@
     'odin_conv2d_bwd': [P, P, P, P, I, P, P, IP, P, IP, DP, P],
     'odin_deconv2d_bwd': [P, P, P, P, I, P, P, IP, P, IP, DP, P],
     'odin_conv2d_dgrad_first': [P, P, P, I, P, P, IP, DP, P, P, IP, DP, P],
+    'odin_conv2d_fwd_first': [P, P, P, P, P, P, P, DP, DP, F, IP, P],
     'odin_dense_bwd': [P, P, P, P, I, P, P, IP, P, IP, I, I, I, I, I, P, P, P],
     'odin_dense_bwd_ranged': [P, P, P, P, I, P, P, IP, P, IP, I, I, I, I, I, P, P, P, P],
     'odin_dense_dgrad_keeps_range': [I, I, I],
diff --git a/odin_ai_amd/csrc/dispatch.hip b/odin_ai_amd/csrc/dispatch.hip
--- a/odin_ai_amd/csrc/dispatch.hip
+++ b/odin_ai_amd/csrc/dispatch.hip
@@ -10,6 +10,7 @@
   WGRAD_PLANES, WGRAD5_BLK, WGRAD_BLK, IGEMM_H_WGRAD, IGEMM_WGRAD,
   BWD_PLANES, BWD_BLK,
   TCONV_PLANES_FIRST,
+  FCONV_PLANES_FIRST,
   NOT_SERVED,
   BWD_PAIR,
   TINY_DENSE, THIN_DENSE, DENSE_H, DENSE_GEMM
@@ -22,6 +23,7 @@
     case SMALLDECONV: case IGEMM: case THIN_DENSE: return FOLDS_Y | FOLDS_DX;
     case FCONV_PLANES: case FCONV_BLK: case CONV5_BLK: case TCONV_PLANES: case TCONV_BLK: case IGEMM_H: case DENSE_H:
       return FOLDS_Y | FOLDS_DX | READS_X;
+    case FCONV_PLANES_FIRST: return FOLDS_Y;
     case WGRAD_PLANES: case WGRAD5_BLK: case WGRAD_BLK: case IGEMM_H_WGRAD: return READS_X;
     case BWD_PLANES: case BWD_BLK: case DENSE_GEMM: case TCONV_PLANES_FIRST: return FOLDS_DX;
     default: return 0;
@@ -50,6 +52,12 @@
   if (odin_igemm_h_applicable(0, g)) return IGEMM_H;
   if (odin_igemm_applicable(0, g)) return IGEMM;
   return GENERIC;
+}
+
+Family select_conv2d_fwd_first(const odin_geom& l0, const odin_geom& l1, bool bias, int act0, int act1) {
+  if (act0 != ODIN_ACT_ELU || select_conv2d_fwd(l0, bias, act0) != SMALLC) return NOT_SERVED;
+  if (select_conv2d_fwd(l1, bias, act1) != FCONV_PLANES) return NOT_SERVED;
+  return odin_fconv_planes_first_applicable(l0, l1) ? FCONV_PLANES_FIRST : NOT_SERVED;
 }
 
 bool igemm_dgrad(int tmode, const odin_geom& g, bool slab, bool dry) {
@@ -285,6 +293,19 @@
   return conv_fwd(select_conv2d_fwd(g, bias != nullptr, d->act), 0, 0, g, x, w, bias, y, d, stream);
 }
 
+extern "C" int odin_conv2d_fwd_first(const float* x, const float* w0, const float* b0, float* y0, const float* w1,
+                                     const float* b1, float* y1, const odin_conv_desc* d0, const odin_conv_desc* d1,
+                                     float x_bound, int* rows_out, void* stream) {
+  const bool dry = y1 == nullptr;
+  const Family f = select_conv2d_fwd_first(odin_geom_fwd(d0), odin_geom_fwd(d1), dry || (b0 != nullptr && b1 != nullptr),
+                                           d0->act, d1->act);
+  if (f != FCONV_PLANES_FIRST) return odin_fail(-2, "conv2d_fwd_first: shapes outside the kernel");
+  if (!dry && (x == nullptr || w0 == nullptr || w1 == nullptr)) return odin_fail(-2, "conv2d_fwd_first: null argument");
+  if (!dry && !(x_bound > 0.f) && d0->x_amax == nullptr) return odin_fail(-2, "conv2d_fwd_first: no bound for the image");
+  return odin_fconv_planes_first_launch(x, w0, b0, d0->center, x_bound, d0->x_amax, y0, d0->y_amax, w1, b1, y1, d1->y_amax,
+                                        rows_out, d0->B, stream);
+}
+
 extern "C" int odin_conv2d_dgrad(const float* dy, const float* w, const float* aux, int aux_act, float* dx,
                                  float* colsum_slab, int* slab_rows_out, const odin_conv_desc* d, void* stream) {
   const odin_geom g = odin_geom_dgrad(d);
diff --git a/odin_ai_amd/csrc/fconv_planes.hip b/odin_ai_amd/csrc/fconv_planes.hip
--- a/odin_ai_amd/csrc/fconv_planes.hip
+++ b/odin_ai_amd/csrc/fconv_planes.hip
@@ -1,5 +1,6 @@
 #include "odin_device.h"
 #include "odin_internal.h"
+#include "first_rows.h"
 #include <cstdlib>
 
 namespace {
@@ -17,6 +18,13 @@
   const unsigned* in_amax;
   unsigned* out_amax;
   long long* stamps;
+  const float* img;
+  const float* w0;
+  const float* b0;
+  float* y0;
+  unsigned* y0_amax;
+  float x_bound;
+  int center0;
 };
 
 #if defined(ODIN_SIM) || !defined(ODIN_DIAG)
@@ -40,8 +48,9 @@
 
 constexpr int FP_MAXU = 4;
 
-template <int EPI, int OW, bool ACC, int SCM>
+template <int EPI, int OW, bool ACC, int SCM, bool FR = false>
 __device__ __forceinline__ void fp_body(const FPParams& p) {
+  static_assert(!FR || (EPI == 1 && OW == 16 && !ACC && SCM == 2), "FR: the second layer of the dSprites encoders");
   constexpr int NPL = 2;
   constexpr int TC = 32 / OW;
   constexpr int WU = 2 * OW;
@@ -74,6 +83,12 @@
   FP_STAMP(1);
 
   const OdinRangeReq in_rq = odin_range_issue(SCM != 0 ? p.in_amax : nullptr, lane);
+  FrLane frl;
+  FrStage frs;
+  if (FR) {
+    fr_lane_init(frl, p.w0, p.b0, lane);
+    fr_stage_load(frs, p.img, T0 >> 3, tid);
+  }
   const int kh = wave >> 1, kw0 = 2 * (wave & 1);
   float wv[2][2][8];
 #pragma unroll
@@ -97,7 +112,7 @@
   const int u_lds = (pcw & 1) * PARB + (pcw >> 1) * 64 + (((ch4 >> 1) ^ (((pcw >> 1) >> 2) & 3)) << 4) + (ch4 & 1) * 8;
   const unsigned u_g = (unsigned)(((8 * cblk + pxl) * p.CS + p.ci_off + 4 * ch4) * 4);
   FpItem iuA[FP_MAXU], iuB[FP_MAXU], iuC[FP_MAXU];
-  {
+  if (!FR) {
     const int tpi = p.tiles_per_img;
     const int b0 = odin_div_small(T0, tpi), t0 = T0 - b0 * tpi;
     const int start = HPU * b0 + 2 * TC * t0;
@@ -129,6 +144,7 @@
   const int NF = p.tiles_per_wg + 4;
   FpEnt* tt = reinterpret_cast<FpEnt*>(red + 2 * RED);
   FpEnt* tr = tt + NF;
+  float* imgs = reinterpret_cast<float*>(tr + NF * RPF);
   {
     const int tpi = p.tiles_per_img;
     for (int e = tid; e < NF; e += 512) {
@@ -149,15 +165,31 @@
       const bool valid = T < T1 && G < end;
       const int b = odin_div_small(G, HPU), gi = G - b * HPU;
       const bool real = valid && gi != 0 && b < p.B;
-      tr[e] = FpEnt{valid ? (G - odin_div_small(G, NSU) * NSU) * RBU : DST_NONE,
-                        real ? (int)((unsigned)(G - b - 1) * u_rowbytes) : (int)OFF_NONE};
+      int goff = real ? (int)((unsigned)(G - b - 1) * u_rowbytes) : (int)OFF_NONE;
+      if (FR && real && f == 0 && r < 2 && t1 > 0) goff |= 1;
+      tr[e] = FpEnt{valid ? (G - odin_div_small(G, NSU) * NSU) * RBU : DST_NONE, goff};
+    }
+  }
+  if (FR) {
+    fr_zero_guards(imgs, tid, 512);
+    fr_zero_guards(imgs + FR_IMG_FLOATS, tid, 512);
+    fr_stage_store(frs, imgs + ((T0 >> 3) & 1) * FR_IMG_FLOATS, p.center0, tid);
+    if (((T0 + 1) & 7) == 0 && T0 + 1 < T1) {
+      fr_stage_load(frs, p.img, (T0 + 1) >> 3, tid);
+      fr_stage_store(frs, imgs + (((T0 + 1) >> 3) & 1) * FR_IMG_FLOATS, p.center0, tid);
     }
   }
   auto fill_entries = [&](FpEnt (&en)[FP_MAXU], int f) {
+    if (FR) { en[0] = tr[f * RPF + wave]; return; }
 #pragma unroll
     for (int j = 0; j < FP_MAXU; ++j) en[j] = tr[f * RPF + r0w + RJ * j];
   };
   auto fill_loads = [&](FpItem (&iu)[FP_MAXU], const FpEnt (&en)[FP_MAXU]) {
+    if (FR) {
+      iu[0].dst = en[0].x;
+      iu[0].v.x = odin_bitsf((unsigned)en[0].y);
+      return;
+    }
 #pragma unroll
     for (int j = 0; j < FP_MAXU; ++j) {
       iu[j].dst = en[j].x + u_lds;
@@ -178,6 +210,51 @@
     *reinterpret_cast<u32x2*>(d + PBU) = l;
   };
 
+  float amx0 = 0.f;
+  float frb[8];
+  f32x16 fro;
+  auto fr_item = [&](const FpItem& it, int stage) {
+#ifdef ODIN_SIM
+    const int dst = it.dst, goff = (int)odin_fbits(it.v.x);
+#else
+    const int dst = __builtin_amdgcn_readfirstlane(it.dst);
+    const int goff = __builtin_amdgcn_readfirstlane((int)odin_fbits(it.v.x));
+#endif
+    if (dst < 0) return;
+    const bool zero = goff == (int)OFF_NONE;
+    if (stage == 0) {
+      const int grow = goff >> 12;
+      if (!zero) fr_row_taps(frb, imgs + ((grow >> 5) & 1) * FR_IMG_FLOATS, grow & 31, lane);
+      return;
+    }
+    if (stage == 1) {
+      if (!zero) fro = fr_row_mfma(frl, frb);
+      else fro = f32x16_zero();
+      return;
+    }
+    const int pc = l31 + 1, slot = pc >> 1;
+    char* d0 = ring + dst + (pc & 1) * PARB + slot * 64 + half * 8;
+    float* yp = p.y0 + ((goff & ~1) >> 2) + l31 * 32 + 4 * half;
+    const bool keep = p.y0 != nullptr && !zero && (goff & 1) == 0;
+#pragma unroll
+    for (int qq = 0; qq < 2; ++qq) {
+      const int q = 2 * (stage - 2) + qq;
+      float4 o = make_float4(fro[4 * q], fro[4 * q + 1], fro[4 * q + 2], fro[4 * q + 3]);
+      if (!zero) {
+        o = make_float4(fr_act(o.x + frl.bias[4 * q]), fr_act(o.y + frl.bias[4 * q + 1]),
+                        fr_act(o.z + frl.bias[4 * q + 2]), fr_act(o.w + frl.bias[4 * q + 3]));
+        amx0 = odin_amax3(odin_amax3(amx0, o.x, o.y), o.z, o.w);
+        if (keep) *reinterpret_cast<float4*>(yp + 8 * q) = o;
+      }
+      u32x2 h, l;
+      if (sc) odin_split_h4<true>(o, in_s, in_s2k, h, l);
+      else odin_split_h4<false>(o, 1.f, ODIN_LO_SCALE, h, l);
+      char* d = d0 + ((q ^ ((slot >> 2) & 3)) << 4);
+      *reinterpret_cast<u32x2*>(d) = h;
+      *reinterpret_cast<u32x2*>(d + PBU) = l;
+    }
+  };
+
   const int orow = (OW == 32) ? 0 : (OW == 16) ? (l31 >> 4) : (l31 >> 3);
   const int ocol = (OW == 32) ? l31 : (OW == 16) ? (l31 & 15) : (l31 & 7);
   int boff[2][2];
@@ -209,14 +286,30 @@
     }
 
   if (SCM != 0) {
-    const unsigned in_mb = odin_range_finish(in_rq);
+    unsigned in_mb = odin_range_finish(in_rq);
+    if (FR) {
+      float X = p.x_bound;
+      if (!(X > 0.f)) { X = odin_bitsf(in_mb); X = p.center0 ? 2.f * X + 1.f : X; }
+      in_mb = odin_fbits(fr_bound(frl, p.b0, X, lane));
+#ifndef ODIN_SIM
+      in_mb = __builtin_amdgcn_readfirstlane(in_mb);
+#endif
+    }
     sc = SCM == 1 || odin_act_needs_scale(in_mb);
     const int gk = sc ? odin_range_shift(in_mb) : 0;
     in_s = odin_pow2(gk); in_s2k = odin_pow2(gk + 11); out_s = odin_pow2(-gk);
   }
   FP_STAMP(8);
-#pragma unroll
-  for (int j = 0; j < FP_MAXU; ++j) store_item(iuA[j]);
+  if (FR) {
+    __syncthreads();
+    fill_entries(en, 0);
+    fill_loads(iuA, en);
+#pragma unroll
+    for (int st = 0; st < 4; ++st) fr_item(iuA[0], st);
+  } else {
+#pragma unroll
+    for (int j = 0; j < FP_MAXU; ++j) store_item(iuA[j]);
+  }
   FP_STAMP(9);
   __syncthreads();
   FP_STAMP(7);
@@ -282,6 +375,7 @@
     float2 auxN = make_float2(0.f, 0.f), pvN = make_float2(0.f, 0.f);
     float2 q8[8];
     f32x16 acc = f32x16_zero(), acx = f32x16_zero();
+    const bool stage_img = FR && ((T + 2) & 7) == 0 && T + 2 < T1;
 #pragma unroll
     for (int m = 0; m < 12; ++m) {
       const int t = (m >> 1) & 1, kk = m & 1, pp = m >> 2;
@@ -291,6 +385,7 @@
       if (m == 0) FP_STAMP(3);
       if (m == 11) FP_STAMP(4);
       if (m == 0) {
+        if (FR && stage_img) fr_stage_load(frs, p.img, (T + 2) >> 3, tid);
         fill_loads(ldu, en);
         if (EPI == 2) auxN = odin_run_load2(RX, ooff);
         if (ACC) pvN = odin_run_load2(RO, ooff);
@@ -299,7 +394,10 @@
         fill_entries(en, T - T0 + 4);
         thN = tt[T - T0 + 1];
       }
-      if ((m & 1) == 1 && (m >> 1) < FP_MAXU) store_item(stu[m >> 1]);
+      if ((m & 1) == 1 && (m >> 1) < FP_MAXU) {
+        if (FR) fr_item(stu[0], m >> 1);
+        else store_item(stu[m >> 1]);
+      }
       if (m == 8) finish_load((T - 1) & 1, q8);
       if (m == 9) finish_done(q8);
       ODIN_SCHED_FENCE();
@@ -311,6 +409,7 @@
     for (int pr = 0; pr < 8; ++pr)
       *reinterpret_cast<float2*>(d + pr * (8 * 64 * 8)) = make_float2(acc[2 * pr], acc[2 * pr + 1]);
     FP_STAMP(5);
+    if (FR && stage_img) fr_stage_store(frs, imgs + (((T + 2) >> 3) & 1) * FR_IMG_FLOATS, p.center0, tid);
     ooffP = ooff;
     auxP = auxN;
     pvP = pvN;
@@ -331,6 +430,7 @@
   if (EPI == 2 || EPI == 1) {
     __syncthreads();
     odin_amax_commit_wg(p.out_amax, amx, tid, 512, reinterpret_cast<float*>(red), blockIdx.x + gridDim.x * blockIdx.y);
+    if (FR) odin_amax_commit_wg(p.y0_amax, amx0, tid, 512, reinterpret_cast<float*>(red) + 16, blockIdx.x);
   }
   if (EPI == 2 && p.colsum != nullptr) {
 #pragma unroll
@@ -346,6 +446,10 @@
 template <int EPI, int OW, bool ACC, int SCM>
 __global__ __launch_bounds__(512) void fconv_planes_kernel(FPParams p) {
   fp_body<EPI, OW, ACC, SCM>(p);
+}
+
+__global__ __launch_bounds__(512) void fconv_planes_first_kernel(FPParams p) {
+  fp_body<1, 16, false, 2, true>(p);
 }
 
 template <int EPI, int OW, int SCM>
@@ -372,12 +476,12 @@
   const int ipu = 2 * OW / 8, rj = 8 / ipu > 0 ? 8 / ipu : 1;
   return 8 * (1 + FP_MAXU * rj);
 }
-int fp_tiles_per_wg(int OW, int n_tiles, int gy) {
+int fp_tiles_per_wg(int OW, int n_tiles, int gy, int extra_lds = 0) {
   int cap = odin_num_cus() / gy;
   if (cap < 1) cap = 1;
   if (cap > ODIN_MAX_COLSUM_BLOCKS) cap = ODIN_MAX_COLSUM_BLOCKS;
   int tpw = (n_tiles + cap - 1) / cap;
-  const int limit = (FP_LDS_MAX - fp_ring_bytes(OW)) / fp_fill_bytes(OW) - 4;
+  const int limit = (FP_LDS_MAX - extra_lds - fp_ring_bytes(OW)) / fp_fill_bytes(OW) - 4;
   if (tpw > limit) tpw = limit;
   if ((n_tiles + tpw - 1) / tpw > ODIN_MAX_COLSUM_BLOCKS) return -1;
   return tpw;
@@ -488,3 +592,41 @@
   if (epi == 1) return aw ? fp_launch_w<1, false, 2>(p, OW, grid, stream) : fp_launch_w<1, false, 0>(p, OW, grid, stream);
   return fp_launch_w<2, false, 1>(p, OW, grid, stream);
 }
+
+bool odin_fconv_planes_first_applicable(const odin_geom& l0, const odin_geom& l1) {
+  return odin_fconv_planes_applicable(l1) && l1.B == l0.B && l1.H == 32 && l1.W == 32 && l1.CI == 32 && l1.CO == 32 &&
+         l0.H == 64 && l0.W == 64 && l0.CI == 1 && l0.OH == 32 && l0.OW == 32 && l0.CO == 32 && l0.KH == 4 && l0.KW == 4 &&
+         l0.S == 2 && l0.pt == 1 && l0.pl == 1 && fp_tiles_per_wg(16, l0.B * 8, 1, 2 * FR_IMG_BYTES) > 0;
+}
+
+int odin_fconv_planes_first_launch(const float* img, const float* w0, const float* b0, int center0, float x_bound,
+                                   const uint32_t* x_amax, float* y0, uint32_t* y0_amax, const float* w1, const float* b1,
+                                   float* y1, uint32_t* y1_amax, int* rows_out, int B, void* stream) {
+  FPParams p;
+  memset(&p, 0, sizeof(p));
+  p.w = w1; p.bias = b1; p.out = y1;
+  p.B = B; p.OH = 16; p.CO = 32; p.CS = 32; p.ci_off = 0;
+  p.tiles_per_img = 8;
+  p.n_tiles = B * 8;
+  p.tiles_per_wg = fp_tiles_per_wg(16, p.n_tiles, 1, 2 * FR_IMG_BYTES);
+  if (p.tiles_per_wg <= 0) return odin_fail(-2, "fconv_planes(first): too many tiles for the fill tables");
+  const int gx = (p.n_tiles + p.tiles_per_wg - 1) / p.tiles_per_wg;
+  if (rows_out) *rows_out = gx;
+  if (y1 == nullptr) return 0;
+  if (!(x_bound > 0.f) && x_amax == nullptr) return odin_fail(-2, "fconv_planes(first): no bound for the image");
+  p.img = img; p.w0 = w0; p.b0 = b0; p.y0 = y0; p.y0_amax = y0_amax; p.x_bound = x_bound; p.center0 = center0;
+  p.in_amax = x_bound > 0.f ? nullptr : x_amax;
+  p.out_amax = y1_amax;
+  const size_t lds = (size_t)fp_ring_bytes(16) + (size_t)(p.tiles_per_wg + 4) * fp_fill_bytes(16) + 2 * FR_IMG_BYTES;
+#ifndef ODIN_SIM
+  static bool attr_done = false;
+  if (!attr_done) {
+    if (hipFuncSetAttribute(reinterpret_cast<const void*>(&fconv_planes_first_kernel),
+                            hipFuncAttributeMaxDynamicSharedMemorySize, FP_LDS_MAX) != hipSuccess)
+      (void)hipGetLastError();
+    attr_done = true;
+  }
+#endif
+  ODIN_LAUNCH(fconv_planes_first_kernel, dim3(gx, 1, 1), dim3(512), lds, stream, p);
+  return odin_check_launch("smallc_fwd+fconv_planes(f16x2)");
+}
diff --git a/odin_ai_amd/csrc/first_rows.h b/odin_ai_amd/csrc/first_rows.h
--- /dev/null
+++ b/odin_ai_amd/csrc/first_rows.h
@@ -0,0 +1,71 @@
+#pragma once
+#include "odin_device.h"
+
+constexpr int FR_PITCH = 66;
+constexpr int FR_IMG_FLOATS = 66 * FR_PITCH;
+constexpr int FR_IMG_BYTES = FR_IMG_FLOATS * 4;
+
+struct FrLane {
+  float a[8];
+  float bias[16];
+};
+
+__device__ __forceinline__ void fr_lane_init(FrLane& f, const float* w0, const float* b0, int lane) {
+  const int l31 = lane & 31, h = lane >> 5;
+#pragma unroll
+  for (int u = 0; u < 8; ++u) f.a[u] = w0[(2 * u + h) * 32 + l31];
+#pragma unroll
+  for (int i = 0; i < 16; ++i) f.bias[i] = b0[8 * (i >> 2) + 4 * h + (i & 3)];
+}
+
+__device__ __forceinline__ float fr_bound(const FrLane& f, const float* b0, float X, int lane) {
+  float s = 0.f;
+#pragma unroll
+  for (int u = 0; u < 8; ++u) s += fabsf(f.a[u]);
+  s += __shfl_xor(s, 32);
+  float v = fmaf(s, X, fabsf(b0[lane & 31])) * 1.0009765625f;
+#pragma unroll
+  for (int m = 16; m >= 1; m >>= 1) v = fmaxf(v, __shfl_xor(v, m));
+  return v;
+}
+
+__device__ __forceinline__ void fr_zero_guards(float* img, int tid, int nthreads) {
+  for (int e = tid; e < 4 * 66; e += nthreads) {
+    const int side = e / 66, i = e - side * 66;
+    const int idx = side == 0 ? i : side == 1 ? 65 * FR_PITCH + i : side == 2 ? i * FR_PITCH : i * FR_PITCH + 65;
+    img[idx] = 0.f;
+  }
+}
+
+struct FrStage { float4 v[2]; };
+__device__ __forceinline__ void fr_stage_load(FrStage& s, const float* x, int b, int tid) {
+  const float4* src = reinterpret_cast<const float4*>(x + (size_t)b * 4096);
+  s.v[0] = src[tid];
+  s.v[1] = src[tid + 512];
+}
+__device__ __forceinline__ void fr_stage_store(const FrStage& s, float* img, int center, int tid) {
+#pragma unroll
+  for (int u = 0; u < 2; ++u) {
+    const int e = tid + 512 * u, r = e >> 4, c4 = e & 15;
+    float4 t = s.v[u];
+    if (center) { t.x = 2.f * t.x - 1.f; t.y = 2.f * t.y - 1.f; t.z = 2.f * t.z - 1.f; t.w = 2.f * t.w - 1.f; }
+    float* d = img + (r + 1) * FR_PITCH + 1 + 4 * c4;
+    d[0] = t.x; d[1] = t.y; d[2] = t.z; d[3] = t.w;
+  }
+}
+
+__device__ __forceinline__ void fr_row_taps(float (&b)[8], const float* img, int row, int lane) {
+  const float* p = img + (2 * row) * FR_PITCH + 2 * (lane & 31) + (lane >> 5);
+#pragma unroll
+  for (int u = 0; u < 8; ++u) b[u] = p[(u >> 1) * FR_PITCH + 2 * (u & 1)];
+}
+__device__ __forceinline__ f32x16 fr_row_mfma(const FrLane& f, const float (&b)[8]) {
+  f32x16 acc = f32x16_zero();
+#pragma unroll
+  for (int u = 0; u < 8; ++u) acc = mfma32(f.a[u], b[u], acc);
+  return acc;
+}
+__device__ __forceinline__ float fr_act(float v) {
+  const float em1 = odin_exp2(v * 1.44269504088896341f) - 1.f;
+  return v > 0.f ? v : em1;
+}
diff --git a/odin_ai_amd/csrc/odin_internal.h b/odin_ai_amd/csrc/odin_internal.h
--- a/odin_ai_amd/csrc/odin_internal.h
+++ b/odin_ai_amd/csrc/odin_internal.h
@@ -153,6 +153,10 @@
 
 bool odin_fconv_planes_applicable(const odin_geom& g);
 void odin_fconv_planes_set_stamps(void* buf);
+bool odin_fconv_planes_first_applicable(const odin_geom& l0, const odin_geom& l1);
+int odin_fconv_planes_first_launch(const float* img, const float* w0, const float* b0, int center0, float x_bound,
+                                   const uint32_t* x_amax, float* y0, uint32_t* y0_amax, const float* w1, const float* b1,
+                                   float* y1, uint32_t* y1_amax, int* rows_out, int B, void* stream);
 int odin_fconv_planes_launch(const float* in, const float* w, const float* bias, const float* aux,
                              float* out, float* colsum, int* rows_out, int B, int OH, int OW, int CI, int CO,
                              int epi, const uint32_t* in_amax, uint32_t* out_amax, void* stream);
diff --git a/odin_ai_amd/engine.py b/odin_ai_amd/engine.py
--- a/odin_ai_amd/engine.py
+++ b/odin_ai_amd/engine.py
@@ -110,7 +110,8 @@
   def __init__(self, lib, recs: List[LayerRec], B: int, device, params: torch.Tensor,
                grads: torch.Tensor, max_rows: int, range_words: Optional[torch.Tensor] = None,
                act_words: Optional[torch.Tensor] = None, use_act_words: bool = True, small_wgrad_gf: float = 0.8,
-               direct_wgrad: bool = False, fuse_first_wgrad: bool = False):
+               direct_wgrad: bool = False, fuse_first_wgrad: bool = False, fuse_first_fwd: bool = False,
+               x_bound: float = 0.0):
     self.lib, self.recs, self.B, self.device = lib, recs, B, device
     self.fuse_first = bool(fuse_first_wgrad) and self._first_pair_qualifies()
     self.params, self.grads = params, grads
@@ -148,6 +149,15 @@
     for i, cd in enumerate(self.descs):
       if cd is not None:
         cd.x_amax, cd.y_amax = self.x_word[i], self.y_word[i]
+    self.x_bound = float(x_bound)
+    self.fuse_first_fwd = (bool(fuse_first_fwd) and self._first_pair_qualifies() and
+                           (self.x_bound > 0.0 or self.x_word[0] is not None))
+    if self.fuse_first_fwd:
+      try:
+        lib.odin_conv2d_fwd_first(None, None, None, None, None, None, None, C.byref(self.descs[0]),
+                                  C.byref(self.descs[1]), self.x_bound, None, None)
+      except _lib.OdinError:
+        self.fuse_first_fwd = False
     self.wslabs: List[Optional[torch.Tensor]] = [None] * len(recs)
     self.direct_wgrad = bool(direct_wgrad)
     self.wdirect = [False] * len(recs)
@@ -269,9 +279,18 @@
     r = self.recs[i]
     return self.params[r.b_off:r.b_off + r.b_n]
 
-  def forward(self, x: torch.Tensor, st, upto: Optional[int] = None, start: int = 0):
+  def forward(self, x: torch.Tensor, st, upto: Optional[int] = None, start: int = 0, fuse_first: bool = False):
     lib, B = self.lib, self.B
     h = x
+    end = len(self.recs) if upto is None else upto
+    if fuse_first and self.fuse_first_fwd and start == 0 and end >= 2:
+      try:
+        lib.odin_conv2d_fwd_first(x.data_ptr(), self.w(0).data_ptr(), self.b(0).data_ptr(), self.outs[0].data_ptr(),
+                                  self.w(1).data_ptr(), self.b(1).data_ptr(), self.outs[1].data_ptr(),
+                                  C.byref(self.descs[0]), C.byref(self.descs[1]), self.x_bound, None, st)
+        h, start = self.outs[1], 2
+      except _lib.OdinError:
+        pass
     for i in range(start, len(self.recs) if upto is None else upto):
       r = self.recs[i]
       y = self.outs[i]
@@ -419,7 +438,7 @@
                range_words: Optional[torch.Tensor] = None, *,
                act_words: bool = True, hyper_ring: bool = True, hyper_ring_rows: int = 128, fuse_norm: bool = True,
                overlap_wgrad: Optional[str] = None, early_reduce: bool = False, defer_wgrad: bool = False,
-               fuse_first_wgrad: bool = True, side_streams: int = 2, small_wgrad_gf: float = 0.8, dp_buckets: Optional[int] = None,
+               fuse_first_wgrad: bool = True, fuse_first_fwd: bool = True, side_streams: int = 2, small_wgrad_gf: float = 0.8, dp_buckets: Optional[int] = None,
                neck: bool = True, neck_bwd: Optional[bool] = None, static_top_word: bool = True,
                latent_reg: Optional[str] = None, reg_coef: float = 1.0, mmd_kernel: str = 'gaussian',
                mmd_prior_samples: int = 100, dip_lambda: Tuple[float, float] = (1.0, 2.0), prior_seed: int = 0,
@@ -502,7 +521,9 @@
     gw, aw = self.range_words[:nl * RANGE_WORDS], self.range_words[nl * RANGE_WORDS:2 * nl * RANGE_WORDS]
     self.enc = NetProgram(self.lib, self.enc_recs, B, self.device, self.params, self.grads, mr,
                           range_words=gw[:ne * RANGE_WORDS], act_words=aw[:ne * RANGE_WORDS],
-                          use_act_words=act_words, small_wgrad_gf=small_wgrad_gf, fuse_first_wgrad=fuse_first_wgrad)
+                          use_act_words=act_words, small_wgrad_gf=small_wgrad_gf, fuse_first_wgrad=fuse_first_wgrad,
+                          fuse_first_fwd=fuse_first_fwd,
+                          x_bound=1.0 if (observation == 'bernoulli' and bool(static_top_word)) else 0.0)
     self.dec = NetProgram(self.lib, self.dec_recs, B, self.device, self.params, self.grads, mr,
                           range_words=gw[ne * RANGE_WORDS:], act_words=aw[ne * RANGE_WORDS:],
                           use_act_words=act_words, small_wgrad_gf=small_wgrad_gf)
@@ -1252,7 +1273,7 @@
     self._latent_fwd(x, eps, st, self.neck, self.lat_block, for_step=False)
     return (self.enc.outs[-1] if self.vq_K is not None else self.p), self.z
 
-  def _latent_fwd(self, x, eps, st, neck: bool, block: bool, for_step: bool):
+  def _latent_fwd(self, x, eps, st, neck: bool, block: bool, for_step: bool, fuse_first: bool = False):
     lib, B, D = self.lib, self.B, self.D
     if self.vq_K is not None:
       self._vq_assign(self.enc.forward(x, st), st, count=for_step)
@@ -1262,11 +1283,11 @@
     lw, lb = self.params[self.lat_w_off:], self.params[self.lat_b_off:]
     cap = self.hp(H_CAP) if self.capacity_on else None
     if neck:
-      self.enc.forward(x, st, upto=len(self.enc_recs) - 2)
+      self.enc.forward(x, st, upto=len(self.enc_recs) - 2, fuse_first=fuse_first)
       self._neck_fwd(eps, st, y1_word=for_step, enc_only=not for_step)
       return self.dec.outs[1], 2
     if block:
-      h_e = self.enc.forward(x, st)
+      h_e = self.enc.forward(x, st, fuse_first=fuse_first)
       r0 = self.dec_recs[0]
       lib.odin_latent_block_fwd(h_e.data_ptr(), lw.data_ptr(), lb.data_ptr(),
                                 None if eps is None else self.eps.data_ptr(), self.eps.data_ptr(),
@@ -1277,7 +1298,7 @@
       return self.dec.outs[0], 1
     if eps is None:
       lib.odin_rng_normal(self.eps.data_ptr(), B * D, self.seed, self.hp(N_HYPER), st)
-    h_e = self.enc.forward(x, st)
+    h_e = self.enc.forward(x, st, fuse_first=fuse_first)
     lib.odin_dense_fwd(h_e.data_ptr(), lw.data_ptr(), lb.data_ptr(), self.p.data_ptr(), B,
                        self.hdim, 2 * D, 0, st)
     lib.odin_latent_fwd(self.p.data_ptr(), self.eps.data_ptr(), self.z.data_ptr(),
@@ -1336,7 +1357,8 @@
     self._clear_stale_act_words(st)
     if len(self.dec_recs) > 1:
       self.dec.set_x_word(1, not self._used_block)
-    dec_in, dec_start = self._latent_fwd(x, eps, st, self._used_neck, self._used_block, for_step=True)
+    dec_in, dec_start = self._latent_fwd(x, eps, st, self._used_neck, self._used_block, for_step=True,
+                                         fuse_first=fused and not self.debug_check_ranges)
     if after_latent is not None:
       after_latent()
     npart = C.c_int(0)
```

Measured after the change: 563,900 images/sec, median of 6. 1.2% higher.
